# actuday6418/ray-tracer-s8

Hardware: AMD Instinct MI355X
Metric: Mrays/sec @ 4K/8spp 1024-sphere (higher is better)
Workload: dtype f32

## Files before the change

ray_tracer_s8_amd/csrc/rt_api.hip:

```cpp
#include <hip/hip_runtime.h>
#include <dlfcn.h>

#include <algorithm>
#include <chrono>
#include <cmath>
#include <cstdarg>
#include <cstdio>
#include <cstdlib>
#include <cstring>
#include <atomic>
#include <climits>
#include <condition_variable>
#include <mutex>
#include <new>
#include <stdexcept>
#include <string>
#include <thread>
#include <vector>

#include "rt_assign.h"
#include "rt_bvh.h"
#include "rt_kernel.hip.h"
#include "rt_plan.h"
#include "rt_query.hip.h"
#include "rt_scene_host.h"
#include "rt_trace.hip.h"
#include "rt_bounce.hip.h"
#include "rt_direct.hip.h"
#include "rt_nee.hip.h"
#include "rt_aov.hip.h"
#include "rt_camera.hip.h"
#include "rt_denoise.hip.h"
#include "rt_tile.h"
#ifdef RT_DEBUG_HOOKS
#include "rt_unit.hip.h"
#endif

namespace {

thread_local std::string g_err;

int fail(int code, const std::string& msg) {
    g_err = msg;
    return code;
}

void set_err_noexcept(const char* what) noexcept {
    try {
        g_err = what;
    } catch (...) {
    }
}
template <class F>
int guarded(F&& body) noexcept {
    try {
        return body();
    } catch (const std::bad_alloc&) {
        set_err_noexcept("host allocation failed");
        return RT_ERR_OOM;
    } catch (const std::exception& e) {
        set_err_noexcept(e.what());
        return RT_ERR_HIP;
    } catch (...) {
        set_err_noexcept("internal error");
        return RT_ERR_HIP;
    }
}

#define HIPCHK(expr)                                                                                  \
    do {                                                                                              \
        hipError_t _e = (expr);                                                                       \
        if (_e != hipSuccess)                                                                         \
            return fail(RT_ERR_HIP, std::string(#expr) + ": " + hipGetErrorString(_e) + " (" __FILE__ \
                                                                                        ":" +         \
                                        std::to_string(__LINE__) + ")");                              \
    } while (0)

struct DevBuf {
    char* d = nullptr;
    size_t cap = 0;
    int reserve(size_t bytes, const char* what) {
        if (cap >= bytes) return RT_OK;
        release();
        if (hipMalloc(&d, bytes) != hipSuccess) {
            d = nullptr;
            (void)hipGetLastError();
            return fail(RT_ERR_OOM, std::string("hipMalloc(") + what + ") failed");
        }
        cap = bytes;
        return RT_OK;
    }
    void release() {
        (void)hipFree(d);
        d = nullptr;
        cap = 0;
    }
};

struct DeviceCtx {
    int dev = -1;
    hipStream_t stream = nullptr;
    hipStream_t copy_stream = nullptr;
    int n_cu = 0;
    std::mutex mu;
};

enum DebugKnob {
    DBG_LDS_TREE = 0,
    DBG_CULL_WALK,
    DBG_NO_STAGE,
    DBG_SLOTS,
    DBG_FORCE_CAPPED,
    DBG_STACK_LDS,
    DBG_COMPACT,
    DBG_REFILL_EIGHTHS,
    DBG_COMMIT_SLOTS,
    DBG_VERBOSE,
    DBG_REORDER,
    DBG_TAIL_TILES,
    DBG_STRIP_COST,
    DBG_DENOISE_LDS_STEP,
    DBG_N
};
std::atomic<int> g_dbg[DBG_N];
const struct { const char* env; int def; } g_dbg_spec[DBG_N] = {
    {"RT_LDS_TREE", 1}, {"RT_CULL_WALK", -1}, {"RT_NO_STAGE", 0}, {"RT_SLOTS", 0}, {"RT_FORCE_CAPPED", 0},
    {"RT_STACK_LDS", 0}, {"RT_COMPACT", 1}, {"RT_REFILL_EIGHTHS", 0}, {"RT_COMMIT_SLOTS", 0}, {"RT_VERBOSE", 0}, {"RT_REORDER", 1}, {"RT_TAIL_TILES", -1}, {"RT_STRIP_COST", 1},
    {"RT_DENOISE_LDS_STEP", -1}};
std::once_flag g_dbg_once;
void dbg_load_env() {
    std::call_once(g_dbg_once, [] {
        for (int k = 0; k < DBG_N; k++) {
            const char* e = getenv(g_dbg_spec[k].env);
            int v = g_dbg_spec[k].def;
            if (e) v = k == DBG_VERBOSE ? 1 : atoi(e);
            g_dbg[k].store(v, std::memory_order_relaxed);
        }
    });
}
inline int dbg(DebugKnob k) { return g_dbg[k].load(std::memory_order_relaxed); }

std::mutex g_mu;
bool g_init = false;
std::vector<DeviceCtx*> g_ctx;
std::atomic<int> g_live_scenes{0};

rtplan::Knobs plan_knobs() {
    rtplan::Knobs k;
    k.lds_tree = dbg(DBG_LDS_TREE);
    k.cull_walk = dbg(DBG_CULL_WALK);
    k.no_stage = dbg(DBG_NO_STAGE);
    k.slots = dbg(DBG_SLOTS);
    k.commit_slots = dbg(DBG_COMMIT_SLOTS);
    k.force_capped = dbg(DBG_FORCE_CAPPED);
    k.stack_lds = dbg(DBG_STACK_LDS);
    k.compact = dbg(DBG_COMPACT);
    k.refill_eighths = dbg(DBG_REFILL_EIGHTHS);
    k.tail_tiles = dbg(DBG_TAIL_TILES);
    return k;
}

}

struct rt_scene {
    DeviceCtx* ctx = nullptr;
    rtplan::SceneShape shape;
    uint32_t n_lights = 0;
    uint32_t* d_lights = nullptr;
    rtplan::Pose pose;
    bool has_pose = false;
    float4* d_geom = nullptr;
    float4* d_geom_pk = nullptr;
    float4* d_geom_px = nullptr;
    float4* d_mat = nullptr;
    float* d_emis = nullptr;
    float* d_tri = nullptr;
    float4* d_tri_box = nullptr;
    float4* d_bvh = nullptr;
    float4* d_trav = nullptr;
    uint32_t* d_stack_ovf = nullptr;
    size_t stack_ovf_words = 0;
    hipEvent_t ovf_done = nullptr;
    uint4* d_travq = nullptr;
    float4* d_geom_r = nullptr;
    uint32_t* d_big = nullptr;
    uint32_t n_big = 0;
    float tri_k = 0.f, tri_diag = 0.f, tri_es = 0.f, tri_e = 0.f;
    rtbvh::QGrid grid;
    uint32_t* d_leaf_of = nullptr;
    uint32_t* d_world_rank = nullptr;
    bool has_order = false;
    float bvh_build_ms = 0.f;
    unsigned long long* d_counters = nullptr;
    struct Ring {
        float* d = nullptr;
        size_t bytes = 0;
        hipStream_t last = nullptr;
        hipEvent_t done = nullptr;
        uint64_t stamp = 0;
    };
    Ring rings[4];
    uint64_t ring_clock = 0;
    DevBuf d_out, d_outf, d_acc, d_cost, d_aov, d_dn, d_cam;
    DevBuf d_caller;
    std::vector<std::pair<hipEvent_t, hipEvent_t>> pending, free_ev;
    uint64_t primary_rays = 0;
    float h2d_ms = 0.f;
    uint32_t last_engine = 0, last_form = 0;
    std::mutex mu;
};

namespace {

int check_request(const rt_tile_request* rq) {
    if (!rq) return fail(RT_ERR_BAD_ARG, "request is NULL");
    if (rq->width == 0 || rq->height == 0 || rq->divisions == 0 || rq->spp == 0)
        return fail(RT_ERR_BAD_ARG, "width, height, divisions and spp must be non-zero");
    if (rq->division_no >= rq->divisions) return fail(RT_ERR_BAD_ARG, "division_no >= divisions");
    if (rq->height / rq->divisions == 0) return fail(RT_ERR_BAD_ARG, "height / divisions == 0 rows");
    if (rq->max_bounces > RT_MAX_BOUNCES) return fail(RT_ERR_LIMIT, "max_bounces > RT_MAX_BOUNCES");
    if (rq->spp > RT_MAX_SPP) return fail(RT_ERR_LIMIT, "spp > RT_MAX_SPP");
    if (rq->reserved != 0) return fail(RT_ERR_BAD_ARG, "reserved must be 0");
    if ((uint64_t)rq->width * rq->height > 0x7fffffffull) return fail(RT_ERR_LIMIT, "image too large");
    return RT_OK;
}

struct EvPair {
    hipEvent_t a, b;
};

int get_events(rt_scene* sc, EvPair& ev) {
    if (!sc->free_ev.empty()) {
        ev.a = sc->free_ev.back().first;
        ev.b = sc->free_ev.back().second;
        sc->free_ev.pop_back();
        return RT_OK;
    }
    HIPCHK(hipEventCreate(&ev.a));
    HIPCHK(hipEventCreate(&ev.b));
    return RT_OK;
}

constexpr uint32_t QUEUE_SLOTS = 16384;
#ifdef RT_PROFILE_TIME
constexpr uint32_t COUNTER_WORDS = 4 + QUEUE_SLOTS + 16 * 8192;
#else
constexpr uint32_t COUNTER_WORDS = 4 + QUEUE_SLOTS;
#endif

int check_slot(const rt_scene* sc) {
    if (sc->pending.size() >= QUEUE_SLOTS) return fail(RT_ERR_LIMIT, "too many uncollected launches: call rt_scene_collect()");
    return RT_OK;
}

template <class P>
int enqueue(rt_scene* sc, hipStream_t stream, void (*kern)(const P), uint32_t blocks, uint32_t block, size_t lds, const P& p) {
    EvPair ev;
    int rc;
    if ((rc = check_slot(sc)) || (rc = get_events(sc, ev))) return rc;
    HIPCHK(hipEventRecord(ev.a, stream));
    hipLaunchKernelGGL(kern, dim3(blocks), dim3(block), lds, stream, p);
    HIPCHK(hipGetLastError());
    HIPCHK(hipEventRecord(ev.b, stream));
    sc->pending.push_back({ev.a, ev.b});
    return RT_OK;
}

struct Grid {
    uint32_t blocks = 0;
    int per_cu = 0;
};
template <class P>
int persistent_blocks(const rt_scene* sc, void (*kern)(const P), uint32_t block, size_t lds, uint64_t items, Grid& g) {
    HIPCHK(hipOccupancyMaxActiveBlocksPerMultiprocessor(&g.per_cu, kern, (int)block, lds));
    if (g.per_cu < 1) g.per_cu = 1;
    g.blocks = (uint32_t)std::min<uint64_t>((items + block - 1) / block, (uint64_t)sc->ctx->n_cu * (uint32_t)g.per_cu);
    return RT_OK;
}

void scene_refs(const rt_scene* sc, bool full_chain, rtk::SceneRefs& r) {
    r.n_sph = sc->shape.n_sph;
    r.n_tri = sc->shape.n_tri;
    r.root_ref = sc->shape.root_ref;
    r.full_chain = full_chain ? 1u : 0u;
    r.trav = sc->d_trav;
    r.bvh_nodes = sc->d_bvh;
    r.leaf_of = sc->d_leaf_of;
    r.world_rank = sc->has_order ? sc->d_world_rank : nullptr;
    r.geom_r = sc->d_geom_r;
    r.tri = sc->d_tri;
    r.counters = sc->d_counters;
}

bool same_frame(const rt_tile_request& a, const rt_tile_request& b) {
    return a.width == b.width && a.height == b.height && a.divisions == b.divisions && a.spp == b.spp &&
           a.max_bounces == b.max_bounces && a.aperture == b.aperture && a.focus_distance == b.focus_distance &&
           a.fov == b.fov && a.focal_length == b.focal_length && a.t_min == b.t_min && a.t_max == b.t_max &&
           a.flags == b.flags;
}

struct Pass {
    uint32_t begin, end;
    void* const* d_acc;
};
int acquire_stack_ovf(rt_scene* sc, size_t words) {
    if (words > sc->stack_ovf_words) {
        if (sc->d_stack_ovf) {
            if (sc->ovf_done) HIPCHK(hipEventSynchronize(sc->ovf_done));
            (void)hipFree(sc->d_stack_ovf);
            sc->d_stack_ovf = nullptr;
            sc->stack_ovf_words = 0;
        }
        HIPCHK(hipMalloc(&sc->d_stack_ovf, words * sizeof(uint32_t)));
        sc->stack_ovf_words = words;
    }
    return RT_OK;
}

int acquire_ring(rt_scene* sc, hipStream_t stream, size_t bytes, rt_scene::Ring*& rg) {
    rg = nullptr;
    for (auto& r : sc->rings)
        if (r.d && r.last == stream) { rg = &r; break; }
    if (!rg)
        for (auto& r : sc->rings)
            if (!r.d) { rg = &r; break; }
    if (!rg) {
        rg = &sc->rings[0];
        for (auto& r : sc->rings)
            if (r.stamp < rg->stamp) rg = &r;
    }
    if (rg->bytes < bytes) {
        if (rg->d) {
            if (rg->done) HIPCHK(hipEventSynchronize(rg->done));
            (void)hipFree(rg->d);
            rg->d = nullptr;
            rg->bytes = 0;
        }
        HIPCHK(hipMalloc(&rg->d, bytes));
        rg->bytes = bytes;
    }
    if (!rg->done) HIPCHK(hipEventCreateWithFlags(&rg->done, hipEventDisableTiming));
    else if (rg->last != stream) HIPCHK(hipStreamWaitEvent(stream, rg->done, 0));
    rg->last = stream;
    rg->stamp = ++sc->ring_clock;
    return RT_OK;
}

int launch_batch(rt_scene* sc, const rt_tile_request* rqs, uint32_t n, void* const* d_rgb, void* const* d_f32,
                 hipStream_t stream, unsigned long long* d_strip_cost = nullptr, const Pass* pass = nullptr) {
    const rtplan::Knobs kn = plan_knobs();
    const rtplan::SceneShape& sh = sc->shape;
    rtk::KParams p;
    std::memset(&p, 0, sizeof p);
    const rtplan::SampleRange smp = pass ? rtplan::SampleRange{pass->begin, pass->end, true} : rtplan::SampleRange{0u, rqs[0].spp, false};
    rtplan::Plan pl = rtplan::plan_launch(sh, rqs[0], n, smp, kn, p, sc->has_pose ? &sc->pose : nullptr);
    if (pl.status != RT_OK) return fail(pl.status, pl.error);
    p.geom_pk = sc->d_geom_pk;
    p.geom_px = sc->d_geom_px;
    p.geom = sc->d_geom;
    p.mat = sc->d_mat;
    p.emis = sc->d_emis;
    p.tri = sc->d_tri;
    p.tri_box = sc->d_tri_box;
    p.bvh_nodes = sc->d_bvh;
    p.trav = sc->d_trav;
    p.travq = sc->d_travq;
    p.geom_r = sc->d_geom_r;
    for (int i = 0; i < 3; i++) {
        p.q_base[i] = sc->grid.base[i];
        p.q_step[i] = sc->grid.step[i];
        p.q_rstep[i] = 1.0f / sc->grid.step[i];
    }
    p.leaf_of = sc->d_leaf_of;
    p.world_rank = sc->has_order ? sc->d_world_rank : nullptr;
    p.big = sc->d_big;
    p.n_big = sc->n_big;
    p.r_slack = sh.r_slack;
    p.tri_k = sc->tri_k;
    p.tri_diag = sc->tri_diag;
    p.tri_es = sc->tri_es;
    p.tri_e = sc->tri_e;
    for (uint32_t i = 0; i < n; i++) {
        p.strips[i].seed = rqs[i].seed;
        p.strips[i].rgb = (uint8_t*)d_rgb[i];
        p.strips[i].f32 = d_f32 ? (float*)d_f32[i] : nullptr;
        p.strips[i].acc = pass ? (float*)pass->d_acc[i] : nullptr;
        p.strips[i].y0 = p.Hs * rqs[i].division_no;
    }
    int rc = check_slot(sc);
    if (rc) return rc;
    p.counters = sc->d_counters;
    p.queue = sc->d_counters + 4 + sc->pending.size();
    p.strip_cost = dbg(DBG_STRIP_COST) ? d_strip_cost : nullptr;

    const rtk::KernelFn kern = pl.isect < 2 ? rtk::kernel_linear(pl.isect, pl.expanded) : rtk::kernel_traverse(pl.isect, pl.count_steps);
    int per_cu = 0;
    HIPCHK(hipOccupancyMaxActiveBlocksPerMultiprocessor(&per_cu, kern, pl.block, pl.lds));
    if (per_cu < 1) per_cu = 1;
    if (dbg(DBG_VERBOSE))
        fprintf(stderr, "[rt] engine %d%s  lds %zu B  workgroups/CU %d  leaf slots %u  bvh depth %u  leaf density %.3f  prims %u\n",
                pl.engine, pl.capped ? " (capped stack)" : "", pl.lds, per_cu, pl.maxl_l2, sh.bvh_depth, sh.leaf_density, sh.n_sph + sh.n_tri);
    rtplan::plan_queue(pl, (uint32_t)sc->ctx->n_cu * (uint32_t)per_cu, kn, p);
    p.stack_ovf = nullptr;
    if (pl.capped) {
        if ((rc = acquire_stack_ovf(sc, pl.ovf_words))) return rc;
        p.stack_ovf = sc->d_stack_ovf;
    }
    if (dbg(DBG_VERBOSE))
        fprintf(stderr, "[rt] sample-unit ring %zu B: %u units per pixel, %u slots of %u records per wave\n", pl.ring_bytes, p.upp, p.n_slots,
                p.slot_stride);
    rt_scene::Ring* rg = nullptr;
    if ((rc = acquire_ring(sc, stream, pl.ring_bytes, rg))) return rc;
    p.ring = rg->d;
    if (p.stack_ovf) {
        if (sc->ovf_done) HIPCHK(hipStreamWaitEvent(stream, sc->ovf_done, 0));
        else HIPCHK(hipEventCreateWithFlags(&sc->ovf_done, hipEventDisableTiming));
    }
    HIPCHK(hipMemsetAsync(p.queue, 0, sizeof(unsigned long long), stream));
    sc->last_engine = (uint32_t)pl.engine;
    sc->last_form = pl.expanded ? 1u : 0u;
    if ((rc = enqueue(sc, stream, kern, pl.blocks, pl.block, pl.lds, p))) return rc;
    HIPCHK(hipEventRecord(rg->done, stream));
    if (p.stack_ovf) HIPCHK(hipEventRecord(sc->ovf_done, stream));
    sc->primary_rays += (uint64_t)p.Hs * p.W * p.upp * n;
    return RT_OK;
}

int collect_locked(rt_scene* sc, rt_tile_stats* st) {
    float ms = 0.f;
    uint32_t n = 0;
    for (auto& pr : sc->pending) {
        HIPCHK(hipEventSynchronize(pr.second));
        float t = 0.f;
        HIPCHK(hipEventElapsedTime(&t, pr.first, pr.second));
        ms += t;
        n++;
        sc->free_ev.push_back(pr);
    }
    sc->pending.clear();
    unsigned long long c[4] = {0, 0, 0, 0};
    HIPCHK(hipMemcpy(c, sc->d_counters, sizeof c, hipMemcpyDeviceToHost));
    HIPCHK(hipMemset(sc->d_counters, 0, sizeof c));
    if (st) {
        st->ray_segments = c[0];
        st->broad_candidates = c[1];
        st->exact_fallbacks = c[2];
        st->primary_rays = sc->primary_rays;
        st->kernel_ms = ms;
        st->n_launches = n;
        st->h2d_ms = sc->h2d_ms;
        st->d2h_ms = 0.f;
        st->engine = sc->last_engine;
        st->broad_form = sc->last_form;
        st->node_steps = c[3];
    }
    sc->primary_rays = 0;
    sc->h2d_ms = 0.f;
    return RT_OK;
}

struct StagedCall {
    rt_scene* const sc;
    const hipStream_t st;
    const float scene_h2d_ms;
    EvPair up{nullptr, nullptr}, down{nullptr, nullptr};
    bool finished = false;
    explicit StagedCall(rt_scene* s) : sc(s), st(s->ctx->stream), scene_h2d_ms(s->h2d_ms) {}
    StagedCall(const StagedCall&) = delete;
    ~StagedCall() {
        if (!finished) (void)hipStreamSynchronize(st);
        if (up.b) sc->free_ev.push_back({up.a, up.b});
        if (down.b) sc->free_ev.push_back({down.a, down.b});
        sc->h2d_ms = scene_h2d_ms;
    }
    int begin() {
        int rc;
        if ((rc = collect_locked(sc, nullptr)) || (rc = get_events(sc, up)) || (rc = get_events(sc, down))) return rc;
        HIPCHK(hipEventRecord(up.a, st));
        return RT_OK;
    }
    int uploads_done() {
        HIPCHK(hipEventRecord(up.b, st));
        return RT_OK;
    }
    int kernels_done() {
        HIPCHK(hipEventRecord(down.a, st));
        return RT_OK;
    }
    int finish(rt_tile_stats* stats) {
        HIPCHK(hipEventRecord(down.b, st));
        HIPCHK(hipEventSynchronize(down.b));
        finished = true;
        rt_tile_stats s;
        float h2d = 0.f, d2h = 0.f;
        HIPCHK(hipEventElapsedTime(&h2d, up.a, up.b));
        HIPCHK(hipEventElapsedTime(&d2h, down.a, down.b));
        int rc = collect_locked(sc, &s);
        if (rc) return rc;
        s.h2d_ms = h2d;
        s.d2h_ms = d2h;
        if (stats) *stats = s;
        return RT_OK;
    }
};

__attribute__((format(printf, 1, 2))) std::string vtext(const char* fmt, ...) {
    if (!dbg(DBG_VERBOSE)) return {};
    char buf[256];
    va_list ap;
    va_start(ap, fmt);
    vsnprintf(buf, sizeof buf, fmt, ap);
    va_end(ap);
    return buf;
}

template <class P>
void material_refs(const rt_scene* sc, P& p) {
    p.mat = sc->d_mat;
    p.emis = sc->d_emis;
}
template <class P>
void light_refs(const rt_scene* sc, P& p) {
    p.lights = sc->d_lights;
    p.n_lights = sc->n_lights;
}

template <class P>
int launch_rays(rt_scene* sc, const rtplan::QueryPlan& qp, uint32_t block, void (*kern)(const P), const char* what, P& p, uint64_t items,
                const std::string& head, const std::string& tail, uint64_t primary, hipStream_t stream, void* d_zero = nullptr) {
    if (!kern) return fail(RT_ERR_HIP, std::string("no ") + what + " kernel for this plan");
    scene_refs(sc, qp.full_chain, p);
    Grid g;
    int rc = persistent_blocks(sc, kern, block, qp.lds, items, g);
    if (rc || (d_zero && (rc = check_slot(sc)))) return rc;
    if (dbg(DBG_VERBOSE)) fprintf(stderr, "[rt] %s  workgroups/CU %d  %s\n", head.c_str(), g.per_cu, tail.c_str());
    if (d_zero) HIPCHK(hipMemsetAsync(d_zero, 0, sizeof(uint32_t), stream));
    if ((rc = enqueue(sc, stream, kern, g.blocks, block, qp.lds, p))) return rc;
    sc->primary_rays += primary;
    sc->last_engine = (uint32_t)qp.engine;
    sc->last_form = 0;
    return RT_OK;
}

template <class L>
int device_form(rt_scene* sc, void* hip_stream, L&& launch) {
    std::lock_guard<std::mutex> lk(sc->mu);
    HIPCHK(hipSetDevice(sc->ctx->dev));
    return launch(hip_stream ? (hipStream_t)hip_stream : sc->ctx->stream);
}

struct HostForm {
    rt_scene* const sc;
    std::lock_guard<std::mutex> dl, lk;
    explicit HostForm(rt_scene* s) : sc(s), dl(s->ctx->mu), lk(s->mu) {}
    int device() const {
        HIPCHK(hipSetDevice(sc->ctx->dev));
        return RT_OK;
    }
};

struct Staging {
    enum : unsigned { UP = 1, DOWN = 2 };
    struct Entry {
        const void* host;
        size_t bytes;
        unsigned copy;
        size_t off;
    };
    DevBuf& buf;
    std::vector<Entry> e;
    size_t total = 0;
    Staging(rt_scene* sc, std::initializer_list<Entry> entries) : buf(sc->d_caller), e(entries) {
        for (Entry& x : e) {
            x.off = total;
            total += x.bytes;
        }
    }
    int reserve(const char* what) { return buf.reserve(total, what); }
    char* dev(int k) const { return e[k].host ? buf.d + e[k].off : nullptr; }
    int upload(StagedCall& call) const {
        for (int k = 0; k < (int)e.size(); k++)
            if (e[k].host && e[k].bytes && (e[k].copy & UP)) HIPCHK(hipMemcpyAsync(dev(k), e[k].host, e[k].bytes, hipMemcpyHostToDevice, call.st));
        return call.uploads_done();
    }
    int download(StagedCall& call) const {
        int rc = call.kernels_done();
        if (rc) return rc;
        for (int k = 0; k < (int)e.size(); k++)
            if (e[k].host && e[k].bytes && (e[k].copy & DOWN))
                HIPCHK(hipMemcpyAsync(const_cast<void*>(e[k].host), dev(k), e[k].bytes, hipMemcpyDeviceToHost, call.st));
        return RT_OK;
    }
};

int check_active_list(const uint32_t* active, uint32_t n_active, uint32_t n) {
    if (!active) return RT_OK;
    if (n_active > n) return fail(RT_ERR_BAD_ARG, "n_active > n");
    for (uint32_t k = 0; k < n_active; k++)
        if (active[k] >= n) return fail(RT_ERR_BAD_ARG, "active[" + std::to_string(k) + "] >= n");
    return RT_OK;
}

}

extern "C" {

RT_API uint32_t rt_abi_version(void) { return RT_ABI_VERSION; }

RT_API const char* rt_strerror(int status) {
    switch (status) {
        case RT_OK: return "ok";
        case RT_ERR_BAD_ARG: return "bad argument";
        case RT_ERR_NOT_INITIALIZED: return "rt_init() has not succeeded";
        case RT_ERR_NO_DEVICE: return "no HIP device (this library has no CPU fallback)";
        case RT_ERR_BAD_DEVICE: return "device ordinal out of range";
        case RT_ERR_BUFFER_TOO_SMALL: return "output buffer smaller than (height/divisions)*width*3";
        case RT_ERR_FRAME_SIZE: return "height is not a multiple of divisions";
        case RT_ERR_HIP: return "HIP runtime error";
        case RT_ERR_LIMIT: return "limit exceeded";
        case RT_ERR_OOM: return "out of memory";
        default: return "unknown status";
    }
}

RT_API const char* rt_last_error(void) { return g_err.c_str(); }

RT_API void rt_tile_request_defaults(rt_tile_request* rq) {
    if (!rq) return;
    std::memset(rq, 0, sizeof *rq);
    rq->width = 1920;
    rq->height = 1080;
    rq->divisions = 20;
    rq->division_no = 0;
    rq->spp = 100;
    rq->max_bounces = 10;
    rq->aperture = 0.1f;
    rq->focus_distance = 1.0f;
    rq->fov = 3.14159265358979323846f / 2.0f;
    rq->focal_length = 1.0f;
    rq->t_min = 0.001f;
    rq->t_max = 1000.0f;
    rq->seed = 0;
    rq->flags = RT_FLAG_NONE;
}

RT_API size_t rt_tile_bytes(const rt_tile_request* rq) {
    if (!rq || rq->divisions == 0) return 0;
    return (size_t)(rq->height / rq->divisions) * rq->width * 3;
}

static int rt_init_impl(int* n_devices) {
    dbg_load_env();
    std::lock_guard<std::mutex> lk(g_mu);
    if (g_init) {
        if (n_devices) *n_devices = (int)g_ctx.size();
        return RT_OK;
    }
    int n = 0;
    hipError_t e = hipGetDeviceCount(&n);
    if (e != hipSuccess || n <= 0) {
        if (n_devices) *n_devices = 0;
        return fail(RT_ERR_NO_DEVICE, std::string("hipGetDeviceCount: ") +
                                          (e != hipSuccess ? hipGetErrorString(e) : "0 devices"));
    }
    for (int d = 0; d < n; d++) {
        DeviceCtx* c = new DeviceCtx;
        c->dev = d;
        g_ctx.push_back(c);
    }
    g_init = true;
    if (n_devices) *n_devices = n;
    return RT_OK;
}

static int ensure_ctx(DeviceCtx* c) {
    std::lock_guard<std::mutex> lk(c->mu);
    if (c->stream) return RT_OK;
    HIPCHK(hipSetDevice(c->dev));
    HIPCHK(hipDeviceGetAttribute(&c->n_cu, hipDeviceAttributeMultiprocessorCount, c->dev));
    for (int isect = 0; isect < rtplan::N_ISECT; isect++)
        for (int alt = 0; alt < 2; alt++)
            HIPCHK(hipFuncSetAttribute((const void*)(isect < 2 ? rtk::kernel_linear(isect, alt != 0) : rtk::kernel_traverse(isect, alt != 0)),
                                       hipFuncAttributeMaxDynamicSharedMemorySize, (int)rtplan::LDS_LIMIT));
    hipStream_t st = nullptr, cs = nullptr;
    HIPCHK(hipStreamCreateWithFlags(&st, hipStreamNonBlocking));
    HIPCHK(hipStreamCreateWithFlags(&cs, hipStreamNonBlocking));
    c->copy_stream = cs;
    c->stream = st;
    return RT_OK;
}

static int rt_shutdown_impl(void) {
    std::lock_guard<std::mutex> lk(g_mu);
    if (g_live_scenes.load() > 0)
        return fail(RT_ERR_BAD_ARG, "rt_shutdown() refused: destroy every rt_scene first (their device contexts stay valid)");
    for (DeviceCtx* c : g_ctx) {
        (void)hipSetDevice(c->dev);
        if (c->stream) (void)hipStreamDestroy(c->stream);
        if (c->copy_stream) (void)hipStreamDestroy(c->copy_stream);
        delete c;
    }
    g_ctx.clear();
    g_init = false;
    return RT_OK;
}

static int rt_scene_destroy_impl(rt_scene* sc);

using rtscene::HostScene;
static_assert(sizeof(rtscene::F4) == sizeof(float4) && alignof(rtscene::F4) == alignof(float4), "HostScene's records are the device's float4");

static int check_world(const rt_sphere* sp, uint32_t ns, const rt_triangle* tr, uint32_t nt, const uint32_t* world_index) {
    if ((ns && !sp) || (nt && !tr)) return fail(RT_ERR_BAD_ARG, "primitive pointer is NULL");
    if ((uint64_t)ns + nt > RT_MAX_PRIMITIVES) return fail(RT_ERR_LIMIT, "too many primitives (RT_MAX_PRIMITIVES)");
    if (world_index && !rtscene::world_is_permutation(world_index, ns + nt))
        return fail(RT_ERR_BAD_ARG, "world_index is not a permutation of 0 .. n_spheres + n_triangles - 1");
    return RT_OK;
}

static int upload_scene(int device, const HostScene& hs, rt_scene** out) {
    const auto t_create0 = std::chrono::steady_clock::now();
    if (!g_init) return fail(RT_ERR_NOT_INITIALIZED, "call rt_init() first");
    if (device < 0 || device >= (int)g_ctx.size()) return fail(RT_ERR_BAD_DEVICE, "bad device ordinal");
    DeviceCtx* ctx = g_ctx[device];
    {
        int rc0 = ensure_ctx(ctx);
        if (rc0) return rc0;
    }
    HIPCHK(hipSetDevice(ctx->dev));
    rt_scene* sc = new (std::nothrow) rt_scene;
    if (!sc) return fail(RT_ERR_OOM, "host allocation failed");
    g_live_scenes.fetch_add(1);
    struct SceneGuard {
        rt_scene* sc;
        ~SceneGuard() {
            if (sc) rt_scene_destroy_impl(sc);
        }
    } guard{sc};
    const rtbvh::FlatBVH& bvh = hs.bvh;
    sc->ctx = ctx;
    sc->shape = hs.shape;
    sc->bvh_build_ms = hs.bvh_build_ms;
    sc->grid = bvh.grid;
    hipEvent_t e0, e1;
    if (hipEventCreate(&e0) != hipSuccess) return fail(RT_ERR_HIP, "hipEventCreate failed");
    if (hipEventCreate(&e1) != hipSuccess) {
        (void)hipEventDestroy(e0);
        return fail(RT_ERR_HIP, "hipEventCreate failed");
    }
#define SC_CHK(expr)                                                                      \
    do {                                                                                  \
        hipError_t _e = (expr);                                                           \
        if (_e != hipSuccess) {                                                           \
            (void)hipEventDestroy(e0);                                                    \
            (void)hipEventDestroy(e1);                                                    \
            return fail(_e == hipErrorOutOfMemory ? RT_ERR_OOM : RT_ERR_HIP,              \
                        std::string(#expr) + ": " + hipGetErrorString(_e));               \
        }                                                                                 \
    } while (0)
#define SC_UP(dst, vec)                                                                                       \
    do {                                                                                                      \
        SC_CHK(hipMalloc(&sc->dst, (vec).size() * sizeof((vec)[0])));                                         \
        SC_CHK(hipMemcpyAsync(sc->dst, (vec).data(), (vec).size() * sizeof((vec)[0]), hipMemcpyHostToDevice,  \
                              ctx->stream));                                                                  \
    } while (0)
    SC_CHK(hipEventRecord(e0, ctx->stream));
    SC_UP(d_geom, hs.geom);
    SC_UP(d_geom_pk, hs.geom_pk);
    SC_UP(d_geom_px, hs.geom_px);
    SC_UP(d_mat, hs.mat);
    SC_UP(d_emis, hs.emis);
    SC_UP(d_tri, hs.tri);
    SC_UP(d_tri_box, hs.tri_box);
    SC_UP(d_bvh, bvh.nodes);
    SC_UP(d_leaf_of, bvh.leaf_of);
    SC_UP(d_world_rank, hs.world_rank);
    sc->has_order = hs.has_order;
    SC_UP(d_trav, bvh.trav);
    SC_UP(d_travq, bvh.travq);
    SC_UP(d_geom_r, hs.geom_r);
    SC_UP(d_big, hs.big);
    SC_UP(d_lights, hs.lights);
    sc->n_lights = hs.n_lights;
    sc->n_big = hs.n_big;
    sc->tri_k = hs.tri_k;
    sc->tri_diag = hs.tri_diag;
    sc->tri_es = hs.tri_es;
    sc->tri_e = hs.tri_e;
    SC_CHK(hipMalloc(&sc->d_counters, COUNTER_WORDS * sizeof(unsigned long long)));
    SC_CHK(hipMemsetAsync(sc->d_counters, 0, COUNTER_WORDS * sizeof(unsigned long long), ctx->stream));
    SC_CHK(hipEventRecord(e1, ctx->stream));
    SC_CHK(hipEventSynchronize(e1));
    SC_CHK(hipEventElapsedTime(&sc->h2d_ms, e0, e1));
#undef SC_UP
#undef SC_CHK
    (void)hipEventDestroy(e0);
    (void)hipEventDestroy(e1);
    if (dbg(DBG_VERBOSE))
        fprintf(stderr, "[rt] scene: %u prims  culled walk: %u big spheres, slack radius %g, box density %.3f -> %s  bvh build %.2f ms (host)  uploads %.2f ms  upload total %.2f ms\n",
                hs.shape.n_sph + hs.shape.n_tri, hs.n_big, hs.shape.r_slack, hs.shape.cull_density, hs.shape.cull_pays ? "default" : "off", sc->bvh_build_ms, sc->h2d_ms,
                std::chrono::duration<float, std::milli>(std::chrono::steady_clock::now() - t_create0).count());
    guard.sc = nullptr;
    *out = sc;
    return RT_OK;
}

static int rt_scene_create_impl(int device, const rt_sphere* sp, uint32_t ns, const rt_triangle* tr, uint32_t nt,
                                const uint32_t* world_index, rt_scene** out) {
    if (!out) return fail(RT_ERR_BAD_ARG, "out_scene is NULL");
    *out = nullptr;
    int rc = check_world(sp, ns, tr, nt, world_index);
    if (rc) return rc;
    if (!g_init) return fail(RT_ERR_NOT_INITIALIZED, "call rt_init() first");
    if (device < 0 || device >= (int)g_ctx.size()) return fail(RT_ERR_BAD_DEVICE, "bad device ordinal");
    HostScene hs;
    rtscene::build_host_scene(sp, ns, tr, nt, world_index, dbg(DBG_REORDER) != 0, hs);
    return upload_scene(device, hs, out);
}

static int rt_scene_destroy_impl(rt_scene* sc) {
    if (!sc) return RT_OK;
    if (sc->ctx) (void)hipSetDevice(sc->ctx->dev);
    for (auto& pr : sc->pending) {
        (void)hipEventSynchronize(pr.second);
        (void)hipEventDestroy(pr.first);
        (void)hipEventDestroy(pr.second);
    }
    for (auto& pr : sc->free_ev) {
        (void)hipEventDestroy(pr.first);
        (void)hipEventDestroy(pr.second);
    }
    (void)hipFree(sc->d_geom);
    (void)hipFree(sc->d_geom_pk);
    (void)hipFree(sc->d_geom_px);
    (void)hipFree(sc->d_mat);
    (void)hipFree(sc->d_emis);
    (void)hipFree(sc->d_tri);
    (void)hipFree(sc->d_tri_box);
    (void)hipFree(sc->d_bvh);
    (void)hipFree(sc->d_trav);
    (void)hipFree(sc->d_travq);
    (void)hipFree(sc->d_stack_ovf);
    if (sc->ovf_done) (void)hipEventDestroy(sc->ovf_done);
    for (auto& r : sc->rings) {
        (void)hipFree(r.d);
        if (r.done) (void)hipEventDestroy(r.done);
    }
    (void)hipFree(sc->d_geom_r);
    (void)hipFree(sc->d_big);
    (void)hipFree(sc->d_lights);
    (void)hipFree(sc->d_leaf_of);
    (void)hipFree(sc->d_world_rank);
    (void)hipFree(sc->d_counters);
    for (DevBuf* b : {&sc->d_out, &sc->d_outf, &sc->d_acc, &sc->d_cost, &sc->d_aov, &sc->d_dn, &sc->d_cam, &sc->d_caller}) b->release();
    delete sc;
    g_live_scenes.fetch_sub(1);
    return RT_OK;
}

static int check_batch(const rt_tile_request* rqs, uint32_t n) {
    if (!rqs || n == 0) return fail(RT_ERR_BAD_ARG, "empty request batch");
    for (uint32_t i = 0; i < n; i++) {
        int rc = check_request(&rqs[i]);
        if (rc) return rc;
        if (!same_frame(rqs[0], rqs[i]))
            return fail(RT_ERR_BAD_ARG, "batched requests must agree on every field but division_no and seed");
    }
    return RT_OK;
}

static int check_samples(uint32_t begin, uint32_t end, uint32_t spp) {
    if (begin >= end) return fail(RT_ERR_BAD_ARG, "sample_begin >= sample_end");
    if (end > spp) return fail(RT_ERR_BAD_ARG, "sample_end > spp");
    return RT_OK;
}

static int check_array(const void* const* a, uint32_t n, const char* what) {
    if (!a) return fail(RT_ERR_BAD_ARG, std::string(what) + " is NULL");
    for (uint32_t i = 0; i < n; i++)
        if (!a[i]) return fail(RT_ERR_BAD_ARG, std::string(what) + "[i] is NULL");
    return RT_OK;
}

static int check_pass(const rt_tile_request* rqs, uint32_t n, const Pass& pass) {
    int rc = check_samples(pass.begin, pass.end, rqs[0].spp);
    return rc ? rc : check_array(pass.d_acc, n, "accum");
}

static int rt_scene_render_tiles_device_impl(rt_scene* sc, const rt_tile_request* rqs, uint32_t n,
                                        void* const* d_out_rgb, size_t out_len_each, void* const* d_out_f32,
                                        void* hip_stream, const Pass* pass = nullptr) {
    if (!sc) return fail(RT_ERR_BAD_ARG, "scene is NULL");
    int rc = check_batch(rqs, n);
    if (rc) return rc;
    if ((rc = check_array(d_out_rgb, n, "d_out_rgb"))) return rc;
    if (out_len_each < rt_tile_bytes(&rqs[0])) return fail(RT_ERR_BUFFER_TOO_SMALL, "out_len < (H/div)*W*3");
    if (pass && (rc = check_pass(rqs, n, *pass))) return rc;
    std::lock_guard<std::mutex> lk(sc->mu);
    HIPCHK(hipSetDevice(sc->ctx->dev));
    hipStream_t st = hip_stream ? (hipStream_t)hip_stream : sc->ctx->stream;
    for (uint32_t i0 = 0; i0 < n; i0 += rtk::MAX_BATCH) {
        uint32_t m = std::min<uint32_t>(rtk::MAX_BATCH, n - i0);
        Pass part = {};
        if (pass) part = {pass->begin, pass->end, pass->d_acc + i0};
        rc = launch_batch(sc, rqs + i0, m, d_out_rgb + i0, d_out_f32 ? d_out_f32 + i0 : nullptr, st, nullptr, pass ? &part : nullptr);
        if (rc) return rc;
    }
    return RT_OK;
}

static int rt_scene_render_tile_device_impl(rt_scene* sc, const rt_tile_request* rq, void* d_out_rgb, size_t out_len,
                                       void* d_out_f32, void* hip_stream) {
    void* rgb[1] = {d_out_rgb};
    void* f32[1] = {d_out_f32};
    return rt_scene_render_tiles_device_impl(sc, rq, 1, rgb, out_len, d_out_f32 ? f32 : nullptr, hip_stream);
}

static int rt_scene_collect_impl(rt_scene* sc, rt_tile_stats* st) {
    if (!sc) return fail(RT_ERR_BAD_ARG, "scene is NULL");
    std::lock_guard<std::mutex> lk(sc->mu);
    HIPCHK(hipSetDevice(sc->ctx->dev));
    return collect_locked(sc, st);
}

static int rt_scene_render_tiles_impl(rt_scene* sc, const rt_tile_request* rqs, uint32_t n, uint8_t* const* out_rgb,
                                 size_t out_len_each, float* const* out_f32, rt_tile_stats* stats,
                                 unsigned long long* strip_cost_out = nullptr, const Pass* pass = nullptr) {
    if (!sc) return fail(RT_ERR_BAD_ARG, "scene is NULL");
    int rc = check_batch(rqs, n);
    if (rc) return rc;
    if ((rc = check_array((const void* const*)out_rgb, n, "out_rgb"))) return rc;
    const size_t need = rt_tile_bytes(&rqs[0]);
    if (out_len_each < need) return fail(RT_ERR_BUFFER_TOO_SMALL, "out_len < (H/div)*W*3");
    if (pass && (rc = check_pass(rqs, n, *pass))) return rc;
    bool want_f32 = false;
    if (out_f32)
        for (uint32_t i = 0; i < n; i++) want_f32 |= out_f32[i] != nullptr;
    std::lock_guard<std::mutex> dl(sc->ctx->mu);
    std::lock_guard<std::mutex> lk(sc->mu);
    HIPCHK(hipSetDevice(sc->ctx->dev));
    hipStream_t st = sc->ctx->stream;
    if ((rc = sc->d_out.reserve(need * n, "strips")) || (want_f32 && (rc = sc->d_outf.reserve(need * n * sizeof(float), "strips f32"))) ||
        (pass && (rc = sc->d_acc.reserve(need * n * sizeof(float), "running sums"))))
        return rc;
    constexpr size_t COST_BLOCK = (size_t)rtk::COST_COPIES * rtk::MAX_BATCH;
    const size_t cost_blocks = strip_cost_out ? (n + rtk::MAX_BATCH - 1) / rtk::MAX_BATCH + 1 : 0;
    unsigned long long* d_cost = nullptr;
    if (strip_cost_out) {
        const size_t cost_b = cost_blocks * COST_BLOCK * sizeof(unsigned long long);
        if ((rc = sc->d_cost.reserve(cost_b, "strip costs"))) return rc;
        d_cost = (unsigned long long*)sc->d_cost.d;
        HIPCHK(hipMemsetAsync(d_cost, 0, cost_b, st));
    }
    rt_tile_stats prev;
    rc = collect_locked(sc, &prev);
    if (rc) return rc;
    sc->h2d_ms = prev.h2d_ms;
    std::vector<void*> drgb(n), df32(n), dacc(pass ? n : 0);
    for (uint32_t i = 0; i < n; i++) {
        drgb[i] = sc->d_out.d + need * i;
        df32[i] = (want_f32 && out_f32[i]) ? sc->d_outf.d + need * i * sizeof(float) : nullptr;
        if (pass) dacc[i] = sc->d_acc.d + need * i * sizeof(float);
    }
    std::vector<std::pair<uint32_t, uint32_t>> groups;
    {
        const uint32_t tail = (n >= 4 && (uint64_t)need * n > (64ull << 20)) ? std::max<uint32_t>(1, n / 4) : 0;
        for (uint32_t i0 = 0; i0 < n - tail; i0 += rtk::MAX_BATCH)
            groups.emplace_back(i0, std::min<uint32_t>(rtk::MAX_BATCH, n - tail - i0));
        for (uint32_t i0 = n - tail; i0 < n; i0 += rtk::MAX_BATCH)
            groups.emplace_back(i0, std::min<uint32_t>(rtk::MAX_BATCH, n - i0));
    }
    hipStream_t cs = sc->ctx->copy_stream;
    std::vector<EvPair> gev;
    gev.reserve(groups.size());
    struct EvReturn {
        rt_scene* sc;
        std::vector<EvPair>& v;
        hipStream_t a, b;
        bool ok = false;
        ~EvReturn() {
            if (!ok) {
                (void)hipStreamSynchronize(a);
                (void)hipStreamSynchronize(b);
            }
            for (auto& e : v) sc->free_ev.push_back({e.a, e.b});
        }
// ... 1538 lines not shown
```

ray_tracer_s8_amd/csrc/rt_consts.h:

```cpp
#pragma once
#include <stdint.h>

#if defined(__HIPCC__)
#define RT_HOST_DEVICE __host__ __device__ inline
#else
#define RT_HOST_DEVICE inline
#endif

#ifndef RT_MAXC
#define RT_MAXC 16
#endif
#ifndef RT_MAXL
#define RT_MAXL 8
#endif
#ifndef RT_MINL
#define RT_MINL 4
#endif
#ifndef RT_MAXL_LTREE
#define RT_MAXL_LTREE 12
#endif

namespace rtk {

constexpr int BLOCK = 256;
constexpr int LTREE_BLOCK = 1024;
constexpr int UNROLL = 8;
constexpr int MAXC = RT_MAXC;
constexpr int CHUNK = 2048;
constexpr int MAX_BATCH = 64;
constexpr int TRAV_STACK = 64;
constexpr int MAXL = RT_MAXL;
constexpr int MINL = RT_MINL;
constexpr int MAXL_EXACT = 7;
constexpr int LNODE_DW = 19;
RT_HOST_DEVICE uint32_t lt_r0(uint32_t n_internal) { return 0x8000u - (n_internal + 1u) * (uint32_t)LNODE_DW; }
constexpr int MAXL_LTREE = RT_MAXL_LTREE;
constexpr int MAXL_LTREE_MAX = 16;
constexpr uint32_t LEAF_BIT = 0x80000000u;
constexpr uint32_t STAGE_TILE_BYTES = 192;
constexpr uint32_t STAGE_TILES = 3;
constexpr uint32_t SLOTS_MAX = 32;
constexpr uint32_t COST_COPIES = 16;

}
```

ray_tracer_s8_amd/csrc/rt_kernel.hip.h:

```cpp
#pragma once
#include <hip/hip_runtime.h>
#include <type_traits>
#include <stdint.h>

#include "rt_consts.h"
#include "rt_cull.h"

namespace rtk {

#ifndef RT_MINWAVES
#define RT_MINWAVES 4
#endif
#ifndef RT_MINWAVES_TRAV
#define RT_MINWAVES_TRAV 4
#endif
#ifndef RT_MINWAVES_LTREE
#define RT_MINWAVES_LTREE 4
#endif
#ifndef RT_MINWAVES_CULL
#define RT_MINWAVES_CULL 5
#endif
#ifndef RT_STEPS_PER_CHECK_X
#define RT_STEPS_PER_CHECK_X 16
#endif
#ifndef RT_QUEUE_TAKE_MIN
#define RT_QUEUE_TAKE_MIN 4
#endif
#ifndef RT_BF2
#define RT_BF2 1
#endif
#ifndef RT_CULL_FLUSH_MIN
#define RT_CULL_FLUSH_MIN 1
#endif
#ifndef RT_MINWAVES_QTRAV
#define RT_MINWAVES_QTRAV 5
#endif
#ifndef RT_STEPS_PER_CHECK
#define RT_STEPS_PER_CHECK 8
#endif
#ifndef RT_STEPS_PER_CHECK_LTREE
#define RT_STEPS_PER_CHECK_LTREE 8
#endif
#ifndef RT_STEPS_PER_CHECK_Q
#define RT_STEPS_PER_CHECK_Q 16
#endif
#ifndef RT_LT_PARTIAL
#define RT_LT_PARTIAL 40
#endif
#ifndef RT_LT_EAGER
#define RT_LT_EAGER 12
#endif

constexpr uint32_t SLOT_FREE = 0x80000000u;
struct WaveQ {
    uint32_t cnt[SLOTS_MAX];
    uint32_t cost_acc[2];
    uint32_t cost_strip[2];
};
static_assert(sizeof(WaveQ) == 144, "WaveQ layout (rt_plan.h: LDS_LIMIT leaves 3 KiB of static LDS)");
constexpr uint32_t SLOT_UNIT_BITS = 13;
struct WaveStage {
    int left[STAGE_TILES + 1];
    uint32_t dst_lo[STAGE_TILES + 1], dst_hi[STAGE_TILES + 1];
};

struct StripDesc {
    uint64_t seed;
    uint8_t* rgb;
    float* f32;
    float* acc;
    uint32_t y0;
    uint32_t pad;
};

struct KParams {
    uint32_t W, H, Hs;
    uint32_t upp, depth;
    uint32_t spp_all, s_begin, gap;
    uint32_t acc_out;
    uint32_t n_sph, n_sph_pad;
    uint32_t n_tri;
    uint32_t chunk;
    uint32_t n_chunks;
    uint32_t flags;
    uint32_t path32;
    uint32_t lds_cand_off;
    uint32_t lds_path_off;
    uint32_t lds_rr_off;
    uint32_t lds_stack_off;
    uint32_t lds_cmp_off;
    uint32_t lds_stage_off;
    uint32_t n_strips;
    uint32_t tiles_x, tiles_per_strip;
    uint32_t tiles_total;
    uint32_t tiles_big;
    uint32_t sub_shift;
    uint32_t n_tiles;
    uint32_t n_slots;
    uint32_t grp;
    uint32_t grp_magic;
    uint32_t slot_stride;
    uint32_t commit_slots;
    uint32_t spp_magic;
    uint32_t slotu_magic;
    float* ring;
    float org[3], llc[3], hor[3], ver[3];
    float lens_radius, focus_distance;
    float lens_u[3], lens_v[3];
    float u_den, v_den;
    float t_min, t_max;
    float spp_f;
    float spp_rcp;
    const float4* geom_pk;
    const float4* geom_px;
    const float4* geom;
    const float4* mat;
    const float* emis;
    const float* tri;
    const float4* tri_box;
    const float4* trav;
    const uint4* travq;
    const float4* geom_r;
    float q_base[3], q_step[3], q_rstep[3];
    uint32_t root_ref;
    uint32_t maxl;
    uint32_t list16;
    uint32_t stack_lds;
    uint32_t ovf_stride;
    uint32_t* stack_ovf;
    const uint32_t* big;
    uint32_t n_big;
    float r_slack;
    float tri_k, tri_diag, tri_es, tri_e;
    uint32_t refill_eighths;
    uint32_t n_internal;
    uint32_t lds_node_off;
    const float4* bvh_nodes;
    const uint32_t* leaf_of;
    const uint32_t* world_rank;
    unsigned long long* strip_cost;
    unsigned long long* counters;
    unsigned long long* queue;
    StripDesc strips[MAX_BATCH];
};

struct V3 {
    float x, y, z;
};
__device__ __forceinline__ V3 mk(float x, float y, float z) { return V3{x, y, z}; }
__device__ __forceinline__ V3 operator+(V3 a, V3 b) { return {a.x + b.x, a.y + b.y, a.z + b.z}; }
__device__ __forceinline__ V3 operator-(V3 a, V3 b) { return {a.x - b.x, a.y - b.y, a.z - b.z}; }
__device__ __forceinline__ V3 operator*(float s, V3 a) { return {s * a.x, s * a.y, s * a.z}; }
__device__ __forceinline__ V3 operator*(V3 a, float s) { return {a.x * s, a.y * s, a.z * s}; }
template <class P>
__device__ __forceinline__ V3 lens_offset(const P& p, float x1, float x2) {
    return mk(x1 * p.lens_u[0] + x2 * p.lens_v[0], x1 * p.lens_u[1] + x2 * p.lens_v[1], x1 * p.lens_u[2] + x2 * p.lens_v[2]);
}
template <bool NEG_OK = false>
__device__ __forceinline__ float sqrt_rn(float x) {
#ifdef RT_IEEE_SQRT_PLAIN
    return __builtin_sqrtf(x);
#else
    const float r = __builtin_amdgcn_rsqf(x);
    float g = x * r, h = 0.5f * r;
    const float e = __builtin_fmaf(-h, g, 0.5f);
    g = __builtin_fmaf(g, e, g);
    h = __builtin_fmaf(h, e, h);
    const float dd = __builtin_fmaf(-g, g, x);
    float y = __builtin_fmaf(dd, h, g);
    const bool odd = ((__float_as_uint(x) & (NEG_OK ? 0x7fffffffu : 0xffffffffu)) - 0x0f800000u) >= (0x7f800000u - 0x0f800000u);
    if (__ballot(odd)) {
        if (odd) {
            asm volatile("" : "+v"(x));
            y = __builtin_sqrtf(x);
        }
    }
    return y;
#endif
}
#define RT_SQRT(x_) sqrt_rn(x_)
#define RT_SQRT_NEG_OK(x_) sqrt_rn<true>(x_)
#define RT_DIV(a_, b_) ((a_) / (b_))
#define RT_HOOK_LT_STEP_LOADS(nd_, ni_, lnodes_)
#define RT_HOOK_LT_STEP_ALU(p0_, p1_, p2_, p3_, oy_)
#define RT_HOOK_LT_STEP_END
#define RT_HOOK_Q_GATHER(t_ref_, cl_, travq_, n_internal_)
#ifdef RT_PROBES
#include "rt_probes.h"
#endif
__device__ __forceinline__ V3 operator/(V3 a, float s) { return {RT_DIV(a.x, s), RT_DIV(a.y, s), RT_DIV(a.z, s)}; }
__device__ __forceinline__ float dot(V3 a, V3 b) { return (a.x * b.x + a.y * b.y) + a.z * b.z; }
__device__ __forceinline__ float vlength(V3 a) { return RT_SQRT(dot(a, a)); }
__device__ __forceinline__ V3 normalize(V3 a) { return a / vlength(a); }
__device__ __forceinline__ bool try_normalize(V3 a, V3& out) {
    float rcp = RT_DIV(1.0f, RT_SQRT(dot(a, a)));
    if (rcp > 0.0f && rcp < __builtin_inff()) {
        out = a * rcp;
        return true;
    }
    return false;
}
__device__ __forceinline__ V3 normalize_or_zero(V3 a) {
    V3 r;
    return try_normalize(a, r) ? r : mk(0.f, 0.f, 0.f);
}
__device__ __forceinline__ V3 cross(V3 a, V3 b) {
    return {a.y * b.z - a.z * b.y, a.z * b.x - a.x * b.z, a.x * b.y - a.y * b.x};
}

struct Rng {
    uint64_t s0, s1, s2, s3;
};
__device__ __forceinline__ uint64_t rotl64(uint64_t x, int k) { return (x << k) | (x >> (64 - k)); }
__device__ __forceinline__ uint32_t next_u32(Rng& r) {
    uint64_t result = rotl64(r.s0 + r.s3, 23) + r.s0;
    uint64_t t = r.s1 << 17;
    r.s2 ^= r.s0;
    r.s3 ^= r.s1;
    r.s1 ^= r.s2;
    r.s0 ^= r.s3;
    r.s2 ^= t;
    r.s3 = rotl64(r.s3, 45);
    return (uint32_t)(result >> 32);
}
__device__ __forceinline__ uint64_t splitmix_mix(uint64_t z) {
    z = (z ^ (z >> 30)) * 0xbf58476d1ce4e5b9ull;
    z = (z ^ (z >> 27)) * 0x94d049bb133111ebull;
    return z ^ (z >> 31);
}
constexpr uint64_t PHI = 0x9e3779b97f4a7c15ull;
__device__ __forceinline__ Rng seed_state(uint64_t st) {
    Rng r;
    st += PHI; r.s0 = splitmix_mix(st);
    st += PHI; r.s1 = splitmix_mix(st);
    st += PHI; r.s2 = splitmix_mix(st);
    st += PHI; r.s3 = splitmix_mix(st);
    return r;
}
__device__ __forceinline__ float u01(Rng& r) {
    return __uint_as_float((next_u32(r) >> 9) | 0x3f800000u) - 1.0f;
}
__device__ __forceinline__ float gen_range_01(Rng& r) { return u01(r) * 1.0f + 0.0f; }
__device__ __forceinline__ float uniform_m1_1(Rng& r) { return u01(r) * 2.0f + -1.0f; }

__device__ __forceinline__ bool exact_sphere(V3 o, V3 td, V3 cen, float rr, float t_min, float t_max,
                                             float& t_out) {
    const V3 oc = o - cen;
    const float b = dot(td, oc);
    const float len = RT_SQRT(dot(oc, oc));
    const float c = len * len - rr;
    const float disc = b * b - 4.0f * c;
    const float sq = RT_SQRT_NEG_OK(disc);
    const bool bneg = b < 0.0f;
    const float same_sign = bneg ? -b + sq : -b - sq;
    const float diff_sign = bneg ? -b - sq : -b + sq;
    const float a0x2 = 2.0f * c;
    const bool big_s = __builtin_fabsf(same_sign) > 2.0f, big_d = __builtin_fabsf(diff_sign) > 2.0f;
    const float q1 = RT_DIV(a0x2, same_sign), q2 = RT_DIV(a0x2, diff_sign), hs = same_sign / 2.0f, hd = diff_sign / 2.0f;
    const float x1 = big_s ? q1 : hd;
    const float x2 = big_s ? (big_d ? q2 : hs) : hs;
    const bool one = disc == 0.0f;
    const float r1 = -b / 2.0f;
    const float x = one ? r1 : (x1 < x2 ? x1 : x2);
    const float y = one ? r1 : (x1 < x2 ? x2 : x1);
    const bool xin = (x >= t_min) && (x < t_max);
    const bool yin = (y >= t_min) && (y < t_max);
    t_out = (xin && yin) ? (x < y ? x : y) : (xin ? x : y);
    return !(disc < 0.0f) && (xin || yin);
}

__device__ __forceinline__ bool exact_triangle(V3 o, V3 d, const float* __restrict__ tv, float t_min, float t_max,
                                               float& t_out) {
    const float EPSILON = 0.00001f;
    V3 A = mk(tv[0], tv[1], tv[2]), B = mk(tv[3], tv[4], tv[5]), C = mk(tv[6], tv[7], tv[8]);
    V3 a_to_b = B - A;
    V3 a_to_c = C - A;
    V3 u_vec = cross(d, a_to_c);
    float det = dot(a_to_b, u_vec);
    if (det < EPSILON && det > -EPSILON) return false;
    float inv_det = 1.0f / det;
    V3 a_to_origin = o - A;
    float u = dot(a_to_origin, u_vec) * inv_det;
    if (!(u >= 0.0f && u <= 1.0f)) return false;
    V3 v_vec = cross(a_to_origin, a_to_b);
    float v = dot(d, v_vec) * inv_det;
    if (v < 0.0f || u + v > 1.0f) return false;
    float dist = dot(a_to_c, v_vec) * inv_det;
    if (!(dist > EPSILON)) return false;
    t_out = dist;
    return (dist >= t_min) && (dist < t_max);
}

struct RayAux {
    V3 inv;
    bool sx, sy, sz;
    bool full_chain;
    bool finite;
};
__device__ __forceinline__ RayAux ray_aux(V3 d, bool full_chain) {
    RayAux a;
    a.full_chain = full_chain;
    a.inv = mk(RT_DIV(1.0f, d.x), RT_DIV(1.0f, d.y), RT_DIV(1.0f, d.z));
    a.sx = d.x < 0.0f;
    a.sy = d.y < 0.0f;
    a.sz = d.z < 0.0f;
    const float big = __builtin_inff();
    a.finite = !full_chain && __builtin_fabsf(a.inv.x) < big && __builtin_fabsf(a.inv.y) < big &&
               __builtin_fabsf(a.inv.z) < big;
    return a;
}
__device__ __forceinline__ float rmin(float x, float y) { return x < y ? x : y; }
__device__ __forceinline__ float rmax(float x, float y) { return x > y ? x : y; }
__device__ __forceinline__ bool intersects_aabb(V3 o, const RayAux& a, float4 lo, float4 hi) {
    float ray_min = ((a.sx ? hi.x : lo.x) - o.x) * a.inv.x;
    float ray_max = ((a.sx ? lo.x : hi.x) - o.x) * a.inv.x;
    float y_min = ((a.sy ? hi.y : lo.y) - o.y) * a.inv.y;
    float y_max = ((a.sy ? lo.y : hi.y) - o.y) * a.inv.y;
    ray_min = rmax(ray_min, y_min);
    ray_max = rmin(ray_max, y_max);
    float z_min = ((a.sz ? hi.z : lo.z) - o.z) * a.inv.z;
    float z_max = ((a.sz ? lo.z : hi.z) - o.z) * a.inv.z;
    ray_min = rmax(ray_min, z_min);
    ray_max = rmin(ray_max, z_max);
    return rmax(ray_min, 0.0f) <= ray_max;
}
__device__ __forceinline__ bool intersects_aabb_finite(V3 o, const RayAux& a, float4 lo, float4 hi) {
    const float x0 = (lo.x - o.x) * a.inv.x, x1 = (hi.x - o.x) * a.inv.x;
    const float y0 = (lo.y - o.y) * a.inv.y, y1 = (hi.y - o.y) * a.inv.y;
    const float z0 = (lo.z - o.z) * a.inv.z, z1 = (hi.z - o.z) * a.inv.z;
    const float ray_min = __builtin_fmaxf(__builtin_fmaxf(__builtin_fminf(x0, x1), __builtin_fminf(y0, y1)),
                                          __builtin_fminf(z0, z1));
    const float ray_max = __builtin_fminf(__builtin_fminf(__builtin_fmaxf(x0, x1), __builtin_fmaxf(y0, y1)),
                                          __builtin_fmaxf(z0, z1));
    return __builtin_fmaxf(ray_min, 0.0f) <= ray_max;
}
__device__ __forceinline__ void slabs_finite(V3 o, const RayAux& a, float4 lo, float4 hi, float& ray_min, float& ray_max) {
    const float x0 = (lo.x - o.x) * a.inv.x, x1 = (hi.x - o.x) * a.inv.x;
    const float y0 = (lo.y - o.y) * a.inv.y, y1 = (hi.y - o.y) * a.inv.y;
    const float z0 = (lo.z - o.z) * a.inv.z, z1 = (hi.z - o.z) * a.inv.z;
    ray_min = __builtin_fmaxf(__builtin_fmaxf(__builtin_fminf(x0, x1), __builtin_fminf(y0, y1)), __builtin_fminf(z0, z1));
    ray_max = __builtin_fminf(__builtin_fminf(__builtin_fmaxf(x0, x1), __builtin_fmaxf(y0, y1)), __builtin_fmaxf(z0, z1));
}
__device__ __forceinline__ bool bvh_reaches(const float4* __restrict__ nodes, uint32_t node, V3 o, const RayAux& a) {
    const bool finite_inv = a.finite;
    for (;;) {
        const float4 lo = nodes[2 * (size_t)node];
        const uint32_t parent = __float_as_uint(lo.w);
        if (parent == 0xffffffffu) return true;
        const float4 hi = nodes[2 * (size_t)node + 1];
        if (!intersects_aabb(o, a, lo, hi)) return false;
        if (finite_inv) return true;
        node = parent;
    }
}

struct Hit {
    int idx;
    float dist;
    float t;
};
template <int MODE>
__device__ __forceinline__ void consider(Hit& h, int idx, V3 o, V3 d, float t, const RayAux& a,
                                         const float4* __restrict__ nodes, const uint32_t* __restrict__ leaf_of) {
    V3 p = o + t * d;
    float dist = vlength(p - o);
    const bool better = h.idx < 0 || h.dist > dist;
    const bool tie = h.idx >= 0 && h.dist == dist;
    if (!(better || tie)) return;
    if (MODE == 0) {
        if (!better) return;
    } else if (MODE == 1) {
        if (!better && leaf_of[idx] > leaf_of[h.idx]) return;
    } else {
        const uint32_t rank = leaf_of[idx];
        if (!better && rank > leaf_of[h.idx]) return;
        if (!bvh_reaches(nodes, rank, o, a)) return;
    }
    h.idx = idx;
    h.dist = dist;
    h.t = t;
}

template <bool RANKED = false, class Pred>
__device__ __forceinline__ void consider_if(Hit& h, int idx, V3 o, V3 d, float t, Pred admitted, const uint32_t* __restrict__ leaf_of = nullptr) {
    V3 p = o + t * d;
    float dist = vlength(p - o);
    if (!(h.idx < 0 || h.dist > dist)) {
        if (!(RANKED && h.dist == dist && leaf_of[idx] < leaf_of[h.idx])) return;
    }
    if (!admitted()) return;
    h.idx = idx;
    h.dist = dist;
    h.t = t;
}

__device__ __forceinline__ unsigned long long wave_sum(unsigned long long v) {
    for (int off = 32; off > 0; off >>= 1) v += __shfl_xor(v, off, 64);
    return v;
}

__device__ __forceinline__ uint8_t f32_as_u8(float v) {
    if (!(v == v)) return 0;
    if (v <= 0.0f) return 0;
    if (v >= 255.0f) return 255;
    return (uint8_t)(int)v;
}

#ifdef RT_PROFILE_PHASES
#define WCOUNT(slot)                                                                         \
    do {                                                                                     \
        unsigned long long _m = __ballot(1);                                                 \
        if ((int)(threadIdx.x & 63) == (int)__builtin_ctzll(_m)) atomicAdd(&p.counters[4 + 8192 + (slot)], 1ull); \
    } while (0)
#define LCOUNT(slot)                                                                         \
    do {                                                                                     \
        unsigned long long _m = __ballot(1);                                                 \
        if ((int)(threadIdx.x & 63) == (int)__builtin_ctzll(_m)) {                           \
            atomicAdd(&p.counters[4 + 8192 + 32 + (slot)], (unsigned long long)__builtin_popcountll(_m)); \
            atomicAdd(&p.counters[4 + 8192 + 64 + (slot)], 1ull);                            \
        }                                                                                    \
    } while (0)
#else
#define WCOUNT(slot) do { } while (0)
#define LCOUNT(slot) do { } while (0)
#endif
#ifdef RT_PROFILE_TIME
#define TDECL unsigned long long _tacc[8] = {0, 0, 0, 0, 0, 0, 0, 0}; unsigned long long _tlast = __builtin_amdgcn_s_memtime(); const unsigned long long _t0 = __builtin_amdgcn_s_memrealtime(); unsigned long long _tq = 0, _nq = 0
#define TDRAINED do { _tq = __builtin_amdgcn_s_memrealtime(); } while (0)
#define TROUND do { if (_tq) { const uint32_t _w = blockIdx.x * (blockDim.x >> 6) + (threadIdx.x >> 6); const unsigned long long _lv = __builtin_popcountll(__ballot(have_unit)); \
    if ((threadIdx.x & 63) == 0 && _w % 20u == 0u && _w / 20u < 215u && _nq < 16ull) p.counters[4 + 8192 + 4400 + (_w / 20u) * 16u + _nq] = (__builtin_amdgcn_s_memrealtime() & 0xfffffffull) | (_lv << 28); \
    _nq++; } } while (0)
#define TSTAMP(ph) do { const unsigned long long _n = __builtin_amdgcn_s_memtime(); _tacc[ph] += _n - _tlast; _tlast = _n; } while (0)
#define TFLUSH do { if ((threadIdx.x & 63) == 0) { const uint32_t _w = blockIdx.x * (blockDim.x >> 6) + (threadIdx.x >> 6); \
    if (_w < 8192u) { unsigned long long* _b = p.counters + 4 + 16384 + 16u * _w; for (int _i = 0; _i < 8; _i++) _b[_i] = _tacc[_i]; \
    _b[8] = __builtin_amdgcn_s_memrealtime(); _b[9] = _t0; _b[10] = _tq; _b[11] = _nq; } } } while (0)
#else
#define TDECL do { } while (0)
#define TDRAINED do { } while (0)
#define TROUND do { } while (0)
#define TSTAMP(ph) do { } while (0)
#define TFLUSH do { } while (0)
#endif

#ifndef RT_GEOM_RR
#define RT_SPHERE_REC(p_, prim_) ([&]() { const float4 r_ = at32((p_).geom_r, (prim_)); return make_float4(r_.x, r_.y, r_.z, r_.w * r_.w); }())
#else
#define RT_SPHERE_REC(p_, prim_) at32((p_).geom, (prim_))
#endif

typedef float v2f __attribute__((ext_vector_type(2)));
__device__ __forceinline__ v2f pk_fma(v2f a, v2f b, v2f c) { return __builtin_elementwise_fma(a, b, c); }

template <class T>
__device__ __forceinline__ const T& at32(const T* __restrict__ base, uint32_t i) {
    return *reinterpret_cast<const T*>(reinterpret_cast<const char*>(base) + i * (uint32_t)sizeof(T));
}

template <bool ON>
__device__ __forceinline__ int cold(int v) {
    if (ON) asm volatile("" : "+v"(v));
    return v;
}
#ifndef RT_COMMIT_BATCH
#define RT_COMMIT_BATCH 8
#endif
#ifndef RT_COMMIT_AGENT_LOADS
#define RT_COMMIT_AGENT_LOADS 0
#endif
template <class T>
__device__ __forceinline__ T ring_load(const T* q) {
#if RT_COMMIT_AGENT_LOADS
    return __hip_atomic_load(q, __ATOMIC_RELAXED, __HIP_MEMORY_SCOPE_AGENT);
#else
    return *q;
#endif
}
__device__ __forceinline__ uint32_t uni(uint32_t v) { return (uint32_t)__builtin_amdgcn_readfirstlane((int)v); }

__device__ __forceinline__ void qslabs(const uint4 qa, const uint4 qb, V3 ig, V3 cq, float& lmin, float& lmax, float& rmin_, float& rmax_) {
#define RT_Q(word, hi16) ((float)((hi16) ? ((word) >> 16) : ((word) & 0xffffu)))
    const float ax = __builtin_fabsf(ig.x), ay = __builtin_fabsf(ig.y), az = __builtin_fabsf(ig.z);
    const float lcx = __builtin_fmaf(RT_Q(qa.x, 0), ig.x, cq.x), lcy = __builtin_fmaf(RT_Q(qa.x, 1), ig.y, cq.y), lcz = __builtin_fmaf(RT_Q(qa.y, 0), ig.z, cq.z);
    const float lhx = RT_Q(qa.y, 1), lhy = RT_Q(qa.z, 0), lhz = RT_Q(qa.z, 1);
    const float rcx = __builtin_fmaf(RT_Q(qa.w, 0), ig.x, cq.x), rcy = __builtin_fmaf(RT_Q(qa.w, 1), ig.y, cq.y), rcz = __builtin_fmaf(RT_Q(qb.x, 0), ig.z, cq.z);
    const float rhx = RT_Q(qb.x, 1), rhy = RT_Q(qb.y, 0), rhz = RT_Q(qb.y, 1);
#undef RT_Q
    lmin = __builtin_fmaxf(__builtin_fmaxf(__builtin_fmaf(-lhx, ax, lcx), __builtin_fmaf(-lhy, ay, lcy)), __builtin_fmaf(-lhz, az, lcz));
    lmax = __builtin_fminf(__builtin_fminf(__builtin_fmaf(lhx, ax, lcx), __builtin_fmaf(lhy, ay, lcy)), __builtin_fmaf(lhz, az, lcz));
    rmin_ = __builtin_fmaxf(__builtin_fmaxf(__builtin_fmaf(-rhx, ax, rcx), __builtin_fmaf(-rhy, ay, rcy)), __builtin_fmaf(-rhz, az, rcz));
    rmax_ = __builtin_fminf(__builtin_fminf(__builtin_fmaf(rhx, ax, rcx), __builtin_fmaf(rhy, ay, rcy)), __builtin_fmaf(rhz, az, rcz));
}

__device__ __forceinline__ float cull_bound(float best, V3 o, float r_slack) { return cull_bound(best, o.x, o.y, o.z, r_slack); }
__device__ __forceinline__ float cull_bound_tri(float best, V3 o, float k, float diag, float es, float e) {
    return cull_bound_tri(best, o.x, o.y, o.z, k, diag, es, e);
}

template <int ISECT, bool EXPANDED, int BS = BLOCK, bool STATS = false>
__global__ __launch_bounds__(BS, (ISECT == 5 || ISECT == 6) ? RT_MINWAVES_LTREE : ISECT == 9 ? RT_MINWAVES_TRAV : ISECT >= 7 ? RT_MINWAVES_CULL : ISECT >= 3 ? RT_MINWAVES_QTRAV : ISECT == 2 ? RT_MINWAVES_TRAV : RT_MINWAVES) void rt_tile_kernel(const KParams p) {
    constexpr int BLOCK = BS;
    constexpr bool STREAMED = (ISECT == 1);
    constexpr bool TRAVERSE = (ISECT >= 2);
    constexpr bool QNODES = (ISECT == 3 || ISECT == 4 || ISECT == 7 || ISECT == 8);
    constexpr bool CULL = (ISECT == 6 || ISECT == 7 || ISECT == 8 || ISECT == 9);
    constexpr bool XNODES = (ISECT == 2 || ISECT == 9);
    constexpr bool CAPPED = (ISECT == 4 || ISECT == 8);
    constexpr bool LTREE = (ISECT == 5 || ISECT == 6);
    constexpr uint32_t LB = LTREE ? 0x8000u : LEAF_BIT;
    constexpr bool BFSTEP = LTREE;
    const uint32_t ML = QNODES ? p.maxl : (uint32_t)MAXL_EXACT;
    extern __shared__ __attribute__((aligned(16))) unsigned char lds_raw[];
    __shared__ unsigned long long wg_tiles;
    __shared__ unsigned int wg_lock, wg_drained;
    __shared__ WaveQ wave_q[BS / 64];
    constexpr bool CAN_STAGE = (ISECT >= 1 && ISECT <= 4) || ISECT >= 7;
    __shared__ WaveStage wave_st[CAN_STAGE ? BS / 64 : 1];
    {
        uint32_t* z = reinterpret_cast<uint32_t*>(&wave_q[threadIdx.x >> 6]);
        if ((threadIdx.x & 63u) < SLOTS_MAX) wave_q[threadIdx.x >> 6].cnt[threadIdx.x & 63u] = SLOT_FREE;
        if ((threadIdx.x & 63u) == 0u) {
            wave_q[threadIdx.x >> 6].cost_acc[0] = wave_q[threadIdx.x >> 6].cost_acc[1] = 0u;
            wave_q[threadIdx.x >> 6].cost_strip[0] = wave_q[threadIdx.x >> 6].cost_strip[1] = 0xffffffffu;
        }
        (void)z;
        if (CAN_STAGE && (threadIdx.x & 63u) <= STAGE_TILES) wave_st[threadIdx.x >> 6].left[threadIdx.x & 63u] = -1;
    }
    if (threadIdx.x == 0) {
        wg_tiles = 0ull;
        wg_lock = 0u;
        wg_drained = 0u;
    }
    __syncthreads();
    float4* lgeom = reinterpret_cast<float4*>(lds_raw);
    const float* lgeomf = reinterpret_cast<const float*>(lds_raw);
    float* lrr = reinterpret_cast<float*>(lds_raw + p.lds_rr_off);
    const float4* __restrict__ gsrc = EXPANDED ? p.geom_px : p.geom_pk;
    uint16_t* lcand = reinterpret_cast<uint16_t*>(lds_raw + p.lds_cand_off);
    unsigned char* lpath = lds_raw + p.lds_path_off;

    const int tid = threadIdx.x;
    const int lane = tid & 63;
    const int tid16 = (tid & ~63) | ((tid & 31) << 1) | ((tid >> 5) & 1);

    if (ISECT == 0) {
        for (uint32_t i = tid; i < p.n_sph_pad; i += BLOCK) lgeom[i] = gsrc[i];
        if (EXPANDED)
            for (uint32_t i = tid; i < p.n_sph_pad; i += BLOCK) lrr[i] = p.geom[i].w;
        __syncthreads();
    }

    if (LTREE) {
        float* ln = reinterpret_cast<float*>(lds_raw + p.lds_node_off);
        const uint32_t r0 = lt_r0(p.n_internal);
        for (uint32_t n = tid; n <= p.n_internal; n += BLOCK) {
            float* q = ln + LNODE_DW * n;
            if (n < p.n_internal) {
                const float4 a0 = p.trav[4u * n], a1 = p.trav[4u * n + 1], a2 = p.trav[4u * n + 2], a3 = p.trav[4u * n + 3];
                auto ref16 = [r0](uint32_t r) { return (r & LEAF_BIT) ? (0x8000u | (r & 0x7fffu)) : r0 + r * (uint32_t)LNODE_DW; };
                q[0] = a0.x; q[1] = a1.x; q[2] = a0.x;   q[3] = a2.x; q[4] = a3.x; q[5] = a2.x;
                q[6] = a0.y; q[7] = a1.y; q[8] = a0.y;   q[9] = a2.y; q[10] = a3.y; q[11] = a2.y;
                q[12] = a0.z; q[13] = a1.z; q[14] = a0.z; q[15] = a2.z; q[16] = a3.z; q[17] = a2.z;
                q[18] = __uint_as_float(ref16(__float_as_uint(a0.w)) | (ref16(__float_as_uint(a1.w)) << 16));
            } else {
                const float qn = __builtin_nanf(""), inf = __builtin_inff();
                for (int i = 0; i < 18; i++) q[i] = qn;
                for (int a = 0; a < 3; a++) { q[6 * a] = -inf; q[6 * a + 1] = inf; q[6 * a + 2] = -inf; }
                q[18] = __uint_as_float((r0 + p.n_internal * (uint32_t)LNODE_DW) * 0x10001u);
            }
        }
        float* nanf_ = ln + LNODE_DW * (p.n_internal + 1u);
        for (uint32_t i = tid; i < p.n_sph + p.n_tri + (uint32_t)LNODE_DW; i += BLOCK) nanf_[i] = __builtin_nanf("");
        __syncthreads();
    }
    const float* const lnodes = reinterpret_cast<const float*>(lds_raw + p.lds_node_off) - (LTREE ? (int)lt_r0(p.n_internal) : 0);
    const V3 corg = mk(p.org[0], p.org[1], p.org[2]);
    const V3 llc = mk(p.llc[0], p.llc[1], p.llc[2]);
    const V3 hor = mk(p.hor[0], p.hor[1], p.hor[2]);
    const V3 ver = mk(p.ver[0], p.ver[1], p.ver[2]);
    const bool exact_scan = (p.flags & 1u) != 0;
    const bool use_bvh = (p.flags & 2u) == 0;
    const float KMf = 1.0f - 0x1p-17f;
    const v2f NKM = {-KMf, -KMf};

    const uint32_t wave = (uint32_t)tid >> 6;
#define wq wave_q[wave]
#define wst wave_st[CAN_STAGE ? wave : 0u]
    float* const ring = p.ring + (size_t)(blockIdx.x * (uint32_t)(BLOCK / 64) + wave) * ((size_t)p.n_slots * p.slot_stride * 3u);
    const uint32_t all_free = p.n_slots >= 32u ? 0xffffffffu : (1u << p.n_slots) - 1u;
    uint32_t freem = all_free;
    uint32_t cur_slot = 0;
    uint32_t tile_u = 0, tile_units = 0;
    uint32_t tile_x0 = 0, tile_row = 0, tile_yg = 0;
    uint32_t tile_meta = STAGE_TILES << 16;
    uint64_t tile_seed = 0;
    bool q_drained = false;
    bool have_unit = false, need_ray = false;
    uint32_t useq = 0;
    Rng rng = {0, 0, 0, 0};
    uint32_t depth_left = 0, k = 0;
    V3 o = mk(0, 0, 0), d = mk(0, 0, 0);
    bool bounce = false;
    V3 bn = mk(0, 0, 0);
    float brough = 0.f;
    using Cnt = typename std::conditional<(ISECT >= 2), uint32_t, unsigned long long>::type;
    Cnt n_seg = 0, n_cand = 0, n_fall = 0;
    Cnt n_int = 0;
    Hit h;
    h.idx = -1;
    h.dist = 0.f;
    h.t = 0.f;
    RayAux aux = ray_aux(mk(1.f, 1.f, 1.f), false);
    auto AUX = [&]() -> RayAux { return QNODES ? ray_aux(d, (p.flags & 8u) != 0) : aux; };
    auto far_bound = [&](float best) -> float {
        float b = cull_bound(best, o, p.r_slack);
        if ((ISECT == 9 || ISECT == 6) && p.n_tri) b = __builtin_fmaxf(b, cull_bound_tri(best, o, p.tri_k, p.tri_diag, p.tri_es, p.tri_e));
        return b;
    };
    V3 td = mk(0, 0, 0);
    bool in_trav = false;
    uint32_t t_ref = 0, t_sp = 0, t_cnt = 0;
    uint32_t t_head = 0;
    V3 ig = mk(0, 0, 0), cq = mk(0, 0, 0);
    bool qfin = false;
    float t_far = __builtin_inff();
    uint32_t* lc32 = reinterpret_cast<uint32_t*>(lds_raw + p.lds_cand_off);
    uint32_t* lstack = reinterpret_cast<uint32_t*>(lds_raw + p.lds_stack_off);
    uint32_t sgx = 0, sgy = 0, sgz = 0;
    uint16_t* lc16 = reinterpret_cast<uint16_t*>(lds_raw + p.lds_cand_off);
    uint16_t* lstack16 = reinterpret_cast<uint16_t*>(lds_raw + p.lds_stack_off);

    if (BFSTEP) lstack16[tid16] = (uint16_t)(lt_r0(p.n_internal) + p.n_internal * (uint32_t)LNODE_DW);

    auto drain_counters = [&]() {
        const unsigned long long ws = wave_sum(n_seg), wc = wave_sum(n_cand), wf = wave_sum(n_fall);
        const unsigned long long wi = STATS ? wave_sum(n_int) : 0ull;
        if (lane == (int)__builtin_ctzll(__ballot(true))) {
            atomicAdd(&p.counters[0], ws);
            atomicAdd(&p.counters[1], wc);
            atomicAdd(&p.counters[2], wf);
            if (STATS) atomicAdd(&p.counters[3], wi);
        }
        n_seg = n_cand = n_fall = 0;
        n_int = 0;
    };
    const bool staging = CAN_STAGE && p.lds_stage_off != 0xffffffffu;
    unsigned char* const stage_base = lds_raw + (staging ? p.lds_stage_off + wave * (STAGE_TILES * STAGE_TILE_BYTES) : 0u);
    auto decode_tile = [&](uint32_t t, uint32_t& st, uint32_t& x0, uint32_t& row) {
        st = t / p.tiles_per_strip;
        const uint32_t rem = t - st * p.tiles_per_strip;
        row = rem / p.tiles_x;
        x0 = (rem - row * p.tiles_x) << 6;
    };
    auto div_spp = [&](uint32_t q) -> uint32_t { return p.spp_magic ? __umulhi(q, p.spp_magic) : q; };

    TDECL;
    for (;;) {
        WCOUNT(0);
        TSTAMP(5);
        TROUND;
        uint32_t px = 0, pyg = 0;
        if (freem != all_free) {
            __builtin_amdgcn_fence(__ATOMIC_ACQ_REL, "wavefront");
            const bool slot_done = (uint32_t)lane < SLOTS_MAX && (wq.cnt[cold<QNODES>(lane) & (int)(SLOTS_MAX - 1u)] & (SLOT_FREE | ((1u << SLOT_UNIT_BITS) - 1u))) == 0u;
            const uint32_t complete = (uint32_t)__ballot(slot_done);
            const uint32_t n_complete = (uint32_t)__builtin_popcount(complete);
            const bool issue_over = q_drained && tile_u == tile_units;
            if (n_complete >= p.commit_slots || (n_complete != 0u && ((uint32_t)__builtin_popcount(freem) < 2u || issue_over))) {
                WCOUNT(14);
                asm volatile("s_waitcnt vmcnt(0)" ::: "memory");
                const uint32_t n_lanes = p.n_slots * p.grp;
                for (uint32_t l0 = 0; l0 < n_lanes; l0 += 64u) {
                    const uint32_t L = l0 + (uint32_t)lane;
                    const uint32_t slot = p.grp == 1u ? L : __umulhi(L, p.grp_magic), g = L - slot * p.grp;
                    const bool mine = slot < p.n_slots && ((complete >> (slot & 31u)) & 1u) != 0u;
                    if (__ballot(mine) == 0ull) continue;
                    uint32_t stg = STAGE_TILES, cstrip = 0;
                    bool fin = false;
                    uint32_t pin = 0;
                    if (mine) {
                        const float* sb = ring + __umul24(slot, p.slot_stride) * 3u;
                        const uint32_t hx = ring_load(reinterpret_cast<const uint32_t*>(sb) + 0);
                        const uint32_t hrow = ring_load(reinterpret_cast<const uint32_t*>(sb) + 1);
                        const uint32_t hmeta = ring_load(reinterpret_cast<const uint32_t*>(sb) + 2);
                        const float* r = sb + 3u + g * p.upp * 3u;
                        float sum_r = 0.f, sum_g = 0.f, sum_b = 0.f;
                        cstrip = hmeta & 0xffu;
                        if (p.s_begin != 0u && g < ((hmeta >> 8) & 0xffu)) {
                            const float* a = p.strips[cstrip].acc + ((size_t)hrow * p.W + hx + g) * 3;
                            sum_r = a[0];
                            sum_g = a[1];
                            sum_b = a[2];
                        }
                        {
                            uint32_t i = 0;
                            auto batch = [&](auto cb_tag) {
                                constexpr int CB = decltype(cb_tag)::value;
#pragma clang loop unroll(disable)
                                for (; i + (uint32_t)CB <= p.upp; i += (uint32_t)CB) {
                                    LCOUNT(12);
                                    float c[3 * CB];
#pragma unroll
                                    for (int e = 0; e < 3 * CB; e++) c[e] = ring_load(r + e);
#pragma unroll
                                    for (int e = 0; e < CB; e++) {
                                        sum_r = sum_r + c[3 * e + 0];
                                        sum_g = sum_g + c[3 * e + 1];
                                        sum_b = sum_b + c[3 * e + 2];
                                    }
                                    r += 3 * CB;
                                }
                            };
                            if (RT_COMMIT_BATCH > 4 && !QNODES) batch(std::integral_constant<int, RT_COMMIT_BATCH>{});
                            batch(std::integral_constant<int, 4>{});
#pragma clang loop unroll(disable)
                            for (; i < p.upp; i++) {
                                LCOUNT(12);
                                const float cr = ring_load(r + 0);
                                const float cg = ring_load(r + 1);
                                const float cb = ring_load(r + 2);
                                sum_r = sum_r + cr;
                                sum_g = sum_g + cg;
                                sum_b = sum_b + cb;
                                r += 3;
                            }
                        }
                        if (g < ((hmeta >> 8) & 0xffu)) {
                            float cr_, cg_, cb_;
                            if (p.spp_rcp != 0.0f) {
                                cr_ = __builtin_sqrtf(sum_r * p.spp_rcp);
                                cg_ = __builtin_sqrtf(sum_g * p.spp_rcp);
                                cb_ = __builtin_sqrtf(sum_b * p.spp_rcp);
                            } else {
                                cr_ = __builtin_sqrtf(sum_r / p.spp_f);
                                cg_ = __builtin_sqrtf(sum_g / p.spp_f);
                                cb_ = __builtin_sqrtf(sum_b / p.spp_f);
                            }
                            const uint32_t sidx = hmeta & 0xffu;
                            stg = (hmeta >> 16) & 0xffu;
                            const size_t oidx = ((size_t)hrow * p.W + hx + g) * 3;
                            if (p.acc_out) {
                                float* a = p.strips[sidx].acc;
                                a[oidx + 0] = sum_r;
                                a[oidx + 1] = sum_g;
                                a[oidx + 2] = sum_b;
                            }
                            if (!CAN_STAGE || stg == STAGE_TILES) {
                                uint8_t* orgb = p.strips[sidx].rgb;
                                orgb[oidx + 0] = f32_as_u8(cr_ * 255.999f);
                                orgb[oidx + 1] = f32_as_u8(cg_ * 255.999f);
                                orgb[oidx + 2] = f32_as_u8(cb_ * 255.999f);
                            } else {
                                uint8_t* sd = stage_base + stg * STAGE_TILE_BYTES + ((hx + g) & 63u) * 3u;
                                sd[0] = f32_as_u8(cr_ * 255.999f);
                                sd[1] = f32_as_u8(cg_ * 255.999f);
                                sd[2] = f32_as_u8(cb_ * 255.999f);
                                fin = true;
                            }
                            float* of = p.strips[sidx].f32;
                            if (of) {
                                of[oidx + 0] = cr_;
                                of[oidx + 1] = cg_;
                                of[oidx + 2] = cb_;
                            }
                            (void)pin;
                        }
                    }
                    if (p.strip_cost && mine && g == 0u) {
                        const uint32_t sg = wq.cnt[slot & (SLOTS_MAX - 1u)] >> SLOT_UNIT_BITS;
                        if (cstrip == wq.cost_strip[0]) (void)__hip_atomic_fetch_add(&wq.cost_acc[0], sg, __ATOMIC_RELAXED, __HIP_MEMORY_SCOPE_WAVEFRONT);
                        else if (cstrip == wq.cost_strip[1]) (void)__hip_atomic_fetch_add(&wq.cost_acc[1], sg, __ATOMIC_RELAXED, __HIP_MEMORY_SCOPE_WAVEFRONT);
                        else if (sg) atomicAdd(&p.strip_cost[(blockIdx.x % COST_COPIES) * MAX_BATCH + cstrip], (unsigned long long)sg);
                    }
                    if (CAN_STAGE && __ballot(fin)) {
                        __builtin_amdgcn_fence(__ATOMIC_ACQ_REL, "wavefront");
#pragma unroll
                        for (uint32_t k = 0; k < STAGE_TILES; k++) {
                            const unsigned long long mk = __ballot(fin && stg == k);
                            if (mk == 0ull) continue;
                            const int left = (int)uni((uint32_t)wst.left[k]) - (int)__builtin_popcountll(mk);
                            if (left == 0) {
                                if (lane < (int)(STAGE_TILE_BYTES / 4)) {
                                    uint32_t* d32 = reinterpret_cast<uint32_t*>(((uintptr_t)uni(wst.dst_hi[k]) << 32) | uni(wst.dst_lo[k]));
                                    d32[lane] = reinterpret_cast<const uint32_t*>(stage_base + k * STAGE_TILE_BYTES)[lane];
                                }
                            }
                            if (lane == 0) wst.left[k] = left == 0 ? -1 : left;
                        }
                        __builtin_amdgcn_fence(__ATOMIC_ACQ_REL, "wavefront");
                    }
                }
                if (slot_done) wq.cnt[cold<QNODES>(lane)] = SLOT_FREE;
                freem = uni(freem | complete);
                __builtin_amdgcn_fence(__ATOMIC_ACQ_REL, "wavefront");
            }
        }
        TSTAMP(6);
        if (TRAVERSE && __ballot(((n_seg | n_cand | n_fall | n_int) & 0x80000000u) != 0)) drain_counters();
        {
            bool need = !have_unit;
            for (;;) {
                if (__ballot(need) == 0ull) break;
                if (tile_u == tile_units) {
                    if (q_drained) break;
                    uint32_t t = 0xffffffffu;
                    if (lane == 0) {
                        constexpr uint32_t WGC = (uint32_t)(BLOCK / 64) < (uint32_t)RT_QUEUE_TAKE_MIN ? (uint32_t)RT_QUEUE_TAKE_MIN : (uint32_t)(BLOCK / 64);
                        for (;;) {
                            const unsigned long long old = __hip_atomic_fetch_add(&wg_tiles, 1ull, __ATOMIC_RELAXED, __HIP_MEMORY_SCOPE_WORKGROUP);
                            if ((uint32_t)old < (uint32_t)(old >> 32)) {
                                t = (uint32_t)old;
                                break;
                            }
                            if (__hip_atomic_load(&wg_drained, __ATOMIC_RELAXED, __HIP_MEMORY_SCOPE_WORKGROUP)) break;
                            if (__hip_atomic_exchange(&wg_lock, 1u, __ATOMIC_ACQUIRE, __HIP_MEMORY_SCOPE_WORKGROUP) == 0u) {
                                const unsigned long long cur = __hip_atomic_load(&wg_tiles, __ATOMIC_RELAXED, __HIP_MEMORY_SCOPE_WORKGROUP);
                                bool done = false;
                                if ((uint32_t)cur >= (uint32_t)(cur >> 32)) {
                                    const uint32_t g = (uint32_t)atomicAdd(p.queue, (unsigned long long)WGC);
                                    if (g >= p.n_tiles) {
                                        __hip_atomic_store(&wg_drained, 1u, __ATOMIC_RELAXED, __HIP_MEMORY_SCOPE_WORKGROUP);
                                    } else {
                                        t = g;
                                        const uint32_t ge = min(g + WGC, p.n_tiles);
                                        __hip_atomic_store(&wg_tiles, (unsigned long long)(g + 1u) | ((unsigned long long)ge << 32),
                                                           __ATOMIC_RELAXED, __HIP_MEMORY_SCOPE_WORKGROUP);
                                    }
                                    done = true;
                                }
                                __hip_atomic_store(&wg_lock, 0u, __ATOMIC_RELEASE, __HIP_MEMORY_SCOPE_WORKGROUP);
                                if (done) break;
                            } else {
                                __builtin_amdgcn_s_sleep(2);
                            }
                        }
                    }
                    t = (uint32_t)__builtin_amdgcn_readfirstlane((int)t);
                    if (t == 0xffffffffu) {
                        q_drained = true;
                        TDRAINED;
                        break;
                    }
                    uint32_t sub = 0u, tw = 64u;
                    if (t >= p.tiles_big) {
                        const uint32_t e = t - p.tiles_big;
                        t = p.tiles_big + (e >> p.sub_shift);
                        tw = 64u >> p.sub_shift;
                        sub = (e & ((1u << p.sub_shift) - 1u)) * tw;
                    }
#ifndef RT_TILES_TOP_DOWN
                    t = p.tiles_total - 1u - t;
#endif
                    uint32_t tstrip;
                    decode_tile(t, tstrip, tile_x0, tile_row);
                    if (p.strip_cost && lane == 0 && (wq.cost_strip[0] != tstrip || wq.cost_acc[0] >= 0x80000000u)) {
                        if (wq.cost_acc[1]) atomicAdd(&p.strip_cost[(blockIdx.x % COST_COPIES) * MAX_BATCH + wq.cost_strip[1]], (unsigned long long)wq.cost_acc[1]);
                        wq.cost_acc[1] = wq.cost_acc[0];
                        wq.cost_strip[1] = wq.cost_strip[0];
                        wq.cost_acc[0] = 0u;
                        wq.cost_strip[0] = tstrip;
                    }
                    tile_x0 = uni(tile_x0 + sub);
                    tile_row = uni(tile_row);
                    if (tile_x0 >= p.W) continue;
                    tile_yg = uni(p.strips[tstrip].y0 + tile_row);
                    tile_seed = p.strips[tstrip].seed + (((uint64_t)tile_yg * p.W + tile_x0) * p.spp_all + p.s_begin) * (4ull * PHI);
                    tile_seed = (uint64_t)uni((uint32_t)tile_seed) | ((uint64_t)uni((uint32_t)(tile_seed >> 32)) << 32);
                    const uint32_t npix = min(tw, p.W - tile_x0);
                    tile_units = uni(npix * p.upp);
                    tile_u = 0u;
                    uint32_t tstage = STAGE_TILES;
                    if (staging && npix == 64u) {
                        uint8_t* dst = p.strips[tstrip].rgb + ((size_t)tile_row * p.W + tile_x0) * 3;
                        if ((reinterpret_cast<uintptr_t>(dst) & 3u) == 0) {
                            __builtin_amdgcn_fence(__ATOMIC_ACQ_REL, "wavefront");
                            for (uint32_t k = 0; k < STAGE_TILES; k++)
                                if ((int)uni((uint32_t)wst.left[k]) < 0) {
                                    tstage = k;
                                    break;
                                }
                            if (tstage < STAGE_TILES && lane == 0) {
                                wst.left[tstage] = 64;
                                wst.dst_lo[tstage] = (uint32_t)reinterpret_cast<uintptr_t>(dst);
                                wst.dst_hi[tstage] = (uint32_t)(reinterpret_cast<uintptr_t>(dst) >> 32);
                            }
                            __builtin_amdgcn_fence(__ATOMIC_ACQ_REL, "wavefront");
                        }
                    }
                    tile_meta = uni(tstrip | (tstage << 16));
                }
                bool got = false;
                uint32_t tv = 0;
                bool stall = false;
                {
                    const unsigned long long mask = __ballot(need);
                    const uint32_t want = (uint32_t)__builtin_popcountll(mask);
                    const uint32_t U = p.slot_stride - 1u;
                    const uint32_t k_open = __umulhi(tile_u + U - 1u, p.slotu_magic);
                    const uint32_t n_free = (uint32_t)__builtin_popcount(freem);
                    const uint32_t slot_room = (k_open + n_free) * U - tile_u;
                    const uint32_t take = min(want, min(tile_units - tile_u, slot_room));
                    stall = take < want && take == slot_room;
                    const uint32_t n_new = __umulhi(tile_u + take + U - 1u, p.slotu_magic) - k_open;
                    const uint32_t rank = __builtin_amdgcn_mbcnt_hi((uint32_t)(mask >> 32), __builtin_amdgcn_mbcnt_lo((uint32_t)mask, 0u));
                    got = need && rank < take;
                    tv = tile_u + rank;
                    const uint32_t k = __umulhi(tv, p.slotu_magic);
                    const uint32_t unit = tv - __umul24(k, U);
                    uint32_t m = freem;
                    for (uint32_t i = 0; i + 1u < n_new; i++) m = k > k_open + i ? (m & (m - 1u)) : m;
                    const uint32_t slot = k >= k_open ? (uint32_t)__builtin_ctz(m | 0x80000000u) : cur_slot;
                    if (got) {
                        useq = (slot << 24) | unit;
                        if (unit == 0u) {
                            const uint32_t un = min(U, tile_units - tv);
                            wq.cnt[slot] = un;
                            uint32_t* hdr = reinterpret_cast<uint32_t*>(ring + __umul24(slot, p.slot_stride) * 3u);
                            hdr[0] = tile_x0 + __umul24(k, p.grp);
                            hdr[1] = tile_row;
                            hdr[2] = (tile_meta & 0xffu) | (div_spp(un) << 8) | (tile_meta & 0xff0000u);
                        }
                    }
                    tile_u = uni(tile_u + take);
                    if (n_new) {
                        uint32_t fm = freem;
                        for (uint32_t i = 0; i + 1u < n_new; i++) fm &= fm - 1u;
                        cur_slot = uni((uint32_t)__builtin_ctz(fm));
                        freem = uni(fm & (fm - 1u));
                    }
                }
                TSTAMP(7);
                if (got) {
                    WCOUNT(1);
                    LCOUNT(0);
                    const uint32_t j = div_spp(tv);
                    px = tile_x0 + j;
                    pyg = tile_yg;
                    rng = seed_state(tile_seed + (uint64_t)(tv + __umul24(j, p.gap)) * (4ull * PHI));
                    have_unit = true;
                    need_ray = true;
                    bounce = false;
                    need = false;
                }
                if (stall) { LCOUNT(14); break; }
            }
        }
        const bool active = have_unit;
        if (!active) { LCOUNT(13); }
        TSTAMP(0);
        if (active && need_ray) {
            float x1, x2, sm;
            WCOUNT(2);
            for (;;) {
                WCOUNT(3);
                LCOUNT(1);
                x1 = uniform_m1_1(rng);
                x2 = uniform_m1_1(rng);
                sm = x1 * x1 + x2 * x2;
                if (bounce ? !(sm >= 1.0f) : (sm <= 1.0f)) break;
            }
            V3 xdir, pre, fallback;
            LCOUNT(2);
            if (bounce) {
                LCOUNT(3);
                const float factor = 2.0f * RT_SQRT(1.0f - sm);
                const V3 us = mk(x1 * factor, x2 * factor, 1.0f - 2.0f * sm);
                const V3 diffuse_dir = us + bn;
                const V3 glossy_dir = d - (2.0f * dot(d, bn)) * bn;
                pre = diffuse_dir + brough * (glossy_dir - diffuse_dir);
                fallback = bn;
            } else {
                LCOUNT(4);
                const V3 offset = lens_offset(p, x1, x2);
                const float u = ((float)px + gen_range_01(rng)) / p.u_den;
                const float v = ((float)(p.H - pyg - 1) + gen_range_01(rng)) / p.v_den;
                const V3 dir0 = normalize_or_zero(llc + u * hor + v * ver - corg);
                const V3 d1 = normalize(dir0);
                const V3 focal_point = corg + p.focus_distance * d1;
                o = corg + offset;
                pre = focal_point - o;
                fallback = mk(0.f, 0.f, 0.f);
                depth_left = p.depth;
                k = 0;
            }
            if (!try_normalize(pre, xdir)) xdir = fallback;
            d = normalize(xdir);
            need_ray = false;
            bounce = false;
        }
        TSTAMP(1);
        const bool wave_busy = __ballot(active) != 0ull || freem != all_free || !q_drained || tile_u != tile_units;
        if (STREAMED) {
            if (!__syncthreads_or(wave_busy ? 1 : 0)) break;
        } else {
            if (!wave_busy) break;
        }

        if (active && !in_trav) {
            h.idx = -1;
            aux = ray_aux(d, (p.flags & 8u) != 0);
            if (!TRAVERSE) td = 2.0f * d;
            n_seg++;
            if (QNODES) {
                const V3 og = mk((o.x - p.q_base[0]) * p.q_rstep[0], (o.y - p.q_base[1]) * p.q_rstep[1], (o.z - p.q_base[2]) * p.q_rstep[2]);
                ig = mk(p.q_step[0] * aux.inv.x, p.q_step[1] * aux.inv.y, p.q_step[2] * aux.inv.z);
                cq = mk(-(og.x * ig.x), -(og.y * ig.y), -(og.z * ig.z));
                const float big = 0x1p100f, tiny = 0x1p-60f;
                const float ax = __builtin_fabsf(ig.x), ay = __builtin_fabsf(ig.y), az = __builtin_fabsf(ig.z);
                qfin = aux.finite && ax < big && ay < big && az < big && ax > tiny && ay > tiny && az > tiny &&
                       __builtin_fabsf(og.x) < 0x1p18f && __builtin_fabsf(og.y) < 0x1p18f && __builtin_fabsf(og.z) < 0x1p18f;
            }
            if (LTREE) {
                aux.finite = aux.finite && __builtin_fabsf(o.x) < __builtin_inff() && __builtin_fabsf(o.y) < __builtin_inff() &&
                             __builtin_fabsf(o.z) < __builtin_inff();
                sgx = aux.sx ? 1u : 0u;
                sgy = aux.sy ? 1u : 0u;
                sgz = aux.sz ? 1u : 0u;
            }
            if (CULL) {
                t_far = __builtin_inff();
                for (uint32_t j = 0; j < p.n_big; j++) {
                    const uint32_t prim = p.big[j];
                    float t;
                    bool hit;
                    if (prim < p.n_sph) {
                        const float4 g = RT_SPHERE_REC(p, prim);
                        hit = exact_sphere(o, 2.0f * d, mk(g.x, g.y, g.z), g.w, p.t_min, p.t_max, t);
                    } else {
                        hit = exact_triangle(o, d, p.tri + 9 * (size_t)(prim - p.n_sph), p.t_min, p.t_max, t);
                    }
                    if (hit)
                        consider_if<true>(h, (int)prim, o, d, t, [&]() { return bvh_reaches(p.bvh_nodes, p.leaf_of[prim], o, AUX()); }, p.leaf_of);
                }
                if (h.idx >= 0) t_far = far_bound(h.dist);
            }
            if (TRAVERSE) {
                t_ref = p.root_ref;
                t_sp = BFSTEP ? 1u : 0u;
                t_cnt = 0;
                in_trav = (p.n_sph + p.n_tri) > 0;
            }
        }
        if constexpr (TRAVERSE) {
            auto root_test = [&](uint32_t i) {
                    LCOUNT(6);
                    const uint32_t prim = LTREE ? (uint32_t)lc16[i * BLOCK + tid16] & 0x7fffu
                                          : p.list16 ? (uint32_t)lc16[i * BLOCK + tid16] : lc32[i * BLOCK + tid];
                    float t;
                    if (prim < p.n_sph) {
                        const float4 g = RT_SPHERE_REC(p, prim);
                        if (exact_sphere(o, 2.0f * d, mk(g.x, g.y, g.z), g.w, p.t_min, p.t_max, t)) {
                            if (QNODES)
                                consider_if<CULL>(h, (int)prim, o, d, t, [&]() {
                                    if (!qfin || (p.n_sph + p.n_tri) == 1) return true;
                                    const float4 s = at32(p.geom_r, prim);
                                    return intersects_aabb_finite(o, AUX(), make_float4(s.x - s.w, s.y - s.w, s.z - s.w, 0.f),
                                                                  make_float4(s.x + s.w, s.y + s.w, s.z + s.w, 0.f));
                                }, p.leaf_of);
                            else if (CULL)
                                consider<1>(h, (int)prim, o, d, t, aux, p.bvh_nodes, p.leaf_of);
                            else
                                consider<0>(h, (int)prim, o, d, t, aux, p.bvh_nodes, p.leaf_of);
                        }
                    } else {
                        if (exact_triangle(o, d, p.tri + 9 * (size_t)(prim - p.n_sph), p.t_min, p.t_max, t)) {
                            if (QNODES)
                                consider_if(h, (int)prim, o, d, t,
                                            [&]() { return !qfin || bvh_reaches(p.bvh_nodes, p.leaf_of[prim], o, AUX()); });
                            else if (CULL)
                                consider<1>(h, (int)prim, o, d, t, aux, p.bvh_nodes, p.leaf_of);
                            else
                                consider<0>(h, (int)prim, o, d, t, aux, p.bvh_nodes, p.leaf_of);
                        }
                    }
            };
            auto flush = [&]() {
                if (BFSTEP) n_cand += t_cnt - t_head;
#pragma clang loop unroll(disable)
                for (uint32_t i = BFSTEP ? t_head : 0u; i < t_cnt; i++) root_test(i);
                t_cnt = 0;
                if (BFSTEP) t_head = 0;
                if (CULL && h.idx >= 0) t_far = far_bound(h.dist);
            };
            auto flush_one = [&]() {
                n_cand++;
                root_test(t_head);
                t_head++;
                if (t_head == t_cnt) t_head = t_cnt = 0;
                if (CULL && h.idx >= 0) t_far = far_bound(h.dist);
            };

            constexpr bool COMPACT = XNODES;
            auto flush_c = [&](bool want) {
                const uint32_t cnt = want ? t_cnt : 0u;
                uint32_t excl = 0, total = 0;
#pragma unroll
                for (int b = 0; b < 4; b++) {
                    const unsigned long long m = __ballot(((cnt >> b) & 1u) != 0);
                    excl += (uint32_t)__builtin_amdgcn_mbcnt_hi((uint32_t)(m >> 32), __builtin_amdgcn_mbcnt_lo((uint32_t)m, 0u)) << b;
                    total += (uint32_t)__builtin_popcountll(m) << b;
                }
                const unsigned long long act = __ballot(true);
                const uint32_t n_act = (uint32_t)__builtin_popcountll(act);
                const uint32_t rank = (uint32_t)__builtin_amdgcn_mbcnt_hi((uint32_t)(act >> 32), __builtin_amdgcn_mbcnt_lo((uint32_t)act, 0u));
                uint32_t* const w_pref = reinterpret_cast<uint32_t*>(lds_raw + p.lds_cmp_off) + (tid >> 6) * 256;
                float* const w_dist = reinterpret_cast<float*>(w_pref + 64);
                float* const w_root = reinterpret_cast<float*>(w_pref + 128);
                uint32_t* const w_hit = w_pref + 192;
                w_pref[rank] = excl | ((uint32_t)lane << 16);
                __builtin_amdgcn_fence(__ATOMIC_ACQ_REL, "wavefront");
                int best_k = -1;
                float best_t = 0.f;
                auto own_prim = [&](uint32_t k) -> uint32_t {
                    return p.list16 ? (uint32_t)lc16[k * BLOCK + tid16] : lc32[k * BLOCK + tid];
                };
                for (uint32_t base = 0; base < total; base += n_act) {
                    const uint32_t j = base + rank;
                    const bool valid = j < total;
                    uint32_t R = 0, ent = w_pref[0];
                    if (valid) {
#pragma unroll
                        for (uint32_t stp = 32; stp > 0; stp >>= 1) {
                            const uint32_t c = R + stp;
                            if (c < n_act) {
                                const uint32_t e = w_pref[c];
                                if ((e & 0xffffu) <= j) { R = c; ent = e; }
                            }
                        }
                    }
                    const uint32_t L = ent >> 16, slot = j - (ent & 0xffffu);
                    const V3 ro = mk(__shfl(o.x, (int)L, 64), __shfl(o.y, (int)L, 64), __shfl(o.z, (int)L, 64));
                    const V3 rd = mk(__shfl(d.x, (int)L, 64), __shfl(d.y, (int)L, 64), __shfl(d.z, (int)L, 64));
                    bool hit = false;
                    float t = 0.f, dist = 0.f;
                    if (valid) {
                        LCOUNT(6);
                        const uint32_t ot = ((uint32_t)tid & ~63u) | L;
                        const uint32_t ot16 = (ot & ~63u) | ((ot & 31u) << 1) | ((ot >> 5) & 1u);
                        const uint32_t prim = p.list16 ? (uint32_t)lc16[slot * BLOCK + ot16] : lc32[slot * BLOCK + ot];
                        if (prim < p.n_sph) {
                            const float4 g = RT_SPHERE_REC(p, prim);
                            hit = exact_sphere(ro, 2.0f * rd, mk(g.x, g.y, g.z), g.w, p.t_min, p.t_max, t);
                        } else {
                            hit = exact_triangle(ro, rd, p.tri + 9 * (size_t)(prim - p.n_sph), p.t_min, p.t_max, t);
                        }
                        if (hit) {
                            const V3 pp = ro + t * rd;
                            dist = vlength(pp - ro);
                        }
                    }
                    w_dist[rank] = dist;
                    w_root[rank] = t;
                    w_hit[rank] = hit ? 1u : 0u;
                    __builtin_amdgcn_fence(__ATOMIC_ACQ_REL, "wavefront");
                    if (cnt) {
                        const uint32_t k0 = excl > base ? excl : base, k1 = min(excl + cnt, base + n_act);
#pragma clang loop unroll(disable)
                        for (uint32_t k = k0; k < k1; k++) {
                            if (!w_hit[k - base]) continue;
                            const float dk = w_dist[k - base];
                            bool take = best_k < 0 ? (h.idx < 0 || h.dist > dk) : (h.dist > dk);
                            if (CULL && !take && h.dist == dk && (best_k >= 0 || h.idx >= 0)) {
                                const uint32_t cur = best_k >= 0 ? own_prim((uint32_t)best_k) : (uint32_t)h.idx;
                                take = p.leaf_of[own_prim(k - excl)] < p.leaf_of[cur];
                            }
                            if (take) {
                                h.dist = dk;
                                best_k = (int)(k - excl);
                                best_t = w_root[k - base];
                            }
                        }
                    }
                    __builtin_amdgcn_fence(__ATOMIC_ACQ_REL, "wavefront");
                }
                if (best_k >= 0) {
                    h.idx = (int)own_prim((uint32_t)best_k);
                    h.t = best_t;
                }
                if (want) t_cnt = 0;
                if (CULL && want && h.idx >= 0) t_far = far_bound(h.dist);
            };
            auto push = [&](uint32_t v) {
                if (LTREE) lstack16[t_sp * BLOCK + tid16] = (uint16_t)v;
                else if (!CAPPED || t_sp < p.stack_lds) lstack[t_sp * BLOCK + tid] = v;
                else p.stack_ovf[(size_t)(t_sp - p.stack_lds) * p.ovf_stride + (blockIdx.x * BLOCK + tid)] = v;
                t_sp++;
            };
            auto pop = [&]() -> uint32_t {
                --t_sp;
                if (LTREE) return (uint32_t)lstack16[t_sp * BLOCK + tid16];
                if (!CAPPED || t_sp < p.stack_lds) return lstack[t_sp * BLOCK + tid];
                return p.stack_ovf[(size_t)(t_sp - p.stack_lds) * p.ovf_stride + (blockIdx.x * BLOCK + tid)];
            };
            if constexpr (BFSTEP) {
            const uint32_t DONE = lt_r0(p.n_internal) + p.n_internal * (uint32_t)LNODE_DW;
            constexpr int STEPS = RT_STEPS_PER_CHECK_LTREE;
            static_assert(MAXL_LTREE > STEPS, "the leaf list must take a block of appends");
            constexpr uint32_t SLOT = (uint32_t)BLOCK * 2u;
            typedef __attribute__((address_space(3))) unsigned char lds_byte;
            typedef __attribute__((address_space(3))) uint16_t lds_u16;
            const uint32_t lds0 = (uint32_t)(uintptr_t)(lds_byte*)lds_raw;
            const uint32_t stack0_a = lds0 + p.lds_stack_off + (uint32_t)tid16 * 2u;
            const uint32_t list0_m = lds0 + p.lds_cand_off + (uint32_t)tid16 * 2u - SLOT;
            uint32_t top_a = 0, cnt_m = 0;
            auto lds16 = [&](uint32_t a) -> lds_u16& { return *(lds_u16*)(uintptr_t)a; };
            auto step = [&](auto slow_tag) {
                constexpr bool SLOW = decltype(slow_tag)::value;
                static_assert(SLOT == 0x800u, "leaf flag 0x8000 >> 4 must be one slot");
                const uint32_t leaf_slot = (t_ref >> 4) & SLOT;
                const uint32_t ni = t_ref;
                if (STATS) n_int += (ni < DONE) ? 1u : 0u;
                const uint32_t top = (uint32_t)lds16(top_a);
                WCOUNT(5);
                LCOUNT(5);
                lds16(cnt_m + SLOT) = (uint16_t)t_ref;
                const float* __restrict__ nd = lnodes + ni;
                const float* __restrict__ fx = nd + sgx;
                const float* __restrict__ fy = nd + 6 + sgy;
                const float* __restrict__ fz = nd + 12 + sgz;
                const float p0 = fx[0], p1 = fx[1], p2 = fx[3], p3 = fx[4], p4 = fy[0], p5 = fy[1], p6 = fy[3], p7 = fy[4];
                const float p8 = fz[0], p9 = fz[1], p10 = fz[3], p11 = fz[4];
                const uint32_t refs = __float_as_uint(nd[18]);
                RT_HOOK_LT_STEP_LOADS(nd, ni, lnodes);
                __builtin_amdgcn_sched_barrier(0);
                RT_HOOK_LT_STEP_ALU(p0, p1, p2, p3, o.y);
                const float lxn = (p0 - o.x) * aux.inv.x, lxf = (p1 - o.x) * aux.inv.x;
                const float rxn = (p2 - o.x) * aux.inv.x, rxf = (p3 - o.x) * aux.inv.x;
                const float lyn = (p4 - o.y) * aux.inv.y, lyf = (p5 - o.y) * aux.inv.y;
                const float ryn = (p6 - o.y) * aux.inv.y, ryf = (p7 - o.y) * aux.inv.y;
                const float lzn = (p8 - o.z) * aux.inv.z, lzf = (p9 - o.z) * aux.inv.z;
                const float rzn = (p10 - o.z) * aux.inv.z, rzf = (p11 - o.z) * aux.inv.z;
                bool hl, hr;
                float le, re;
                if (SLOW) {
                    le = rmax(rmax(rmax(lxn, lyn), lzn), 0.0f);
                    re = rmax(rmax(rmax(rxn, ryn), rzn), 0.0f);
                    hl = le <= rmin(rmin(lxf, lyf), lzf);
                    hr = re <= rmin(rmin(rxf, ryf), rzf);
                } else {
                    le = __builtin_fmaxf(__builtin_fmaxf(__builtin_fmaxf(lxn, lyn), lzn), 0.0f);
                    re = __builtin_fmaxf(__builtin_fmaxf(__builtin_fmaxf(rxn, ryn), rzn), 0.0f);
                    hl = le <= __builtin_fminf(__builtin_fminf(lxf, lyf), lzf);
                    hr = re <= __builtin_fminf(__builtin_fminf(rxf, ryf), rzf);
                }
                uint32_t cl = refs & 0xffffu, cr = refs >> 16;
                if (CULL) {
                    hl = hl && le <= t_far;
                    hr = hr && re <= t_far;
                    const bool swp = hl && hr && re < le;
                    const uint32_t c0 = cl;
                    cl = swp ? cr : cl;
                    cr = swp ? c0 : cr;
                }
                lds16(top_a + SLOT) = (uint16_t)cr;
                const bool any = hl || hr;
                t_ref = any ? (hl ? cl : cr) : top;
                uint32_t delta = any ? 0u : 0u - SLOT;
                delta = (hl && hr) ? SLOT : delta;
                asm volatile("" : "+v"(delta));
                top_a += delta;
                if (SLOW) top_a = max(top_a, stack0_a);
                cnt_m += leaf_slot;
                RT_HOOK_LT_STEP_END;
            };
            for (;;) {
                const uint32_t walking = (uint32_t)__builtin_popcountll(__ballot(in_trav));
                const uint32_t live = (uint32_t)__builtin_popcountll(__ballot(active));
                if (walking == 0 || (walking * 8 <= live * p.refill_eighths && walking < live)) break;
                if (in_trav && t_cnt > p.maxl - (uint32_t)STEPS) flush();
                if (RT_LT_PARTIAL < 64) {
                    const bool pend = t_cnt > t_head;
                    if ((int)__builtin_popcountll(__ballot(pend)) >= RT_LT_PARTIAL ||
                        (CULL && (int)__builtin_popcountll(__ballot(pend && h.idx < 0)) >= RT_LT_EAGER)) {
                        if (pend) flush_one();
                    }
                }
                const bool slow = __ballot(in_trav && !aux.finite) != 0;
                if (in_trav) {
                    top_a = stack0_a + (t_sp - 1u) * SLOT;
                    cnt_m = list0_m + t_cnt * SLOT;
                    if (slow) {
#pragma unroll
                        for (int rep = 0; rep < STEPS; rep++) step(std::true_type{});
                    } else {
#pragma unroll
                        for (int rep = 0; rep < STEPS; rep++) step(std::false_type{});
                    }
                    t_sp = (top_a + SLOT - stack0_a) / SLOT;
                    t_cnt = (cnt_m - list0_m) / SLOT;
                    in_trav = t_ref != DONE;
                }
            }
            } else {
            for (;;) {
                const uint32_t walking = (uint32_t)__builtin_popcountll(__ballot(in_trav));
                const uint32_t live = (uint32_t)__builtin_popcountll(__ballot(active));
                if (walking == 0 || (walking * 8 <= live * p.refill_eighths && walking < live)) break;
#ifndef RT_FLUSH_INLINE
                if (COMPACT && p.lds_cmp_off != 0xffffffffu) {
                    const bool want = in_trav && (t_cnt == ML || (CULL && t_cnt >= (uint32_t)RT_CULL_FLUSH_MIN && h.idx < 0));
                    if (__ballot(want)) flush_c(want);
                } else
                if (in_trav && (t_cnt == ML || (CULL && t_cnt >= (uint32_t)RT_CULL_FLUSH_MIN && h.idx < 0))) flush();
#endif
                constexpr bool BF2 = (RT_BF2 != 0) && (XNODES || QNODES);
                if (BF2 && !__ballot(in_trav && !(QNODES ? qfin : aux.finite))) {
#pragma unroll
                    for (int rep = 0; rep < (QNODES ? RT_STEPS_PER_CHECK_Q : RT_STEPS_PER_CHECK_X); rep++)
                    if (in_trav) {
                        WCOUNT(5);
                        LCOUNT(5);
                        const bool is_leaf = (t_ref & LEAF_BIT) != 0;
                        if (STATS) n_int += is_leaf ? 0u : 1u;
                        const uint32_t tsl = t_sp - (t_sp ? 1u : 0u);
                        uint32_t top = lstack[(CAPPED ? min(tsl, p.stack_lds - 1u) : tsl) * BLOCK + tid];
                        bool hl, hr;
                        float le = 0.f, re = 0.f;
                        uint32_t c0, c1;
                        if constexpr (QNODES) {
                        const uint4* __restrict__ nq = reinterpret_cast<const uint4*>(reinterpret_cast<const char*>(p.travq) + ((is_leaf ? 0u : t_ref) << 5));
                        uint4 qa = nq[0], qb = nq[1];
                        asm volatile("" : "+v"(qb.x), "+v"(qb.y), "+v"(qb.z), "+v"(qb.w));
                        float lmin, lmax, rmin_, rmax_;
                        qslabs(qa, qb, ig, cq, lmin, lmax, rmin_, rmax_);
                        le = __builtin_fmaxf(lmin, 0.0f);
                        re = __builtin_fmaxf(rmin_, 0.0f);
                        hl = le <= (CULL ? __builtin_fminf(lmax, t_far) : lmax);
                        hr = re <= (CULL ? __builtin_fminf(rmax_, t_far) : rmax_);
                        c0 = qb.z;
                        c1 = qb.w;
                        } else {
                        const float4* __restrict__ nd = reinterpret_cast<const float4*>(reinterpret_cast<const char*>(p.trav) + ((is_leaf ? 0u : t_ref) << 6));
                        const float4 n0 = nd[0], n1 = nd[1], n2 = nd[2], n3 = nd[3];
                        if (CULL) {
                            float lmin, lmax, rmin_, rmax_;
                            slabs_finite(o, aux, n0, n1, lmin, lmax);
                            slabs_finite(o, aux, n2, n3, rmin_, rmax_);
                            le = __builtin_fmaxf(lmin, 0.0f);
                            re = __builtin_fmaxf(rmin_, 0.0f);
                            hl = le <= lmax && le <= t_far;
                            hr = re <= rmax_ && re <= t_far;
                        } else {
                            hl = intersects_aabb_finite(o, aux, n0, n1);
                            hr = intersects_aabb_finite(o, aux, n2, n3);
                        }
                        c0 = __float_as_uint(n0.w);
                        c1 = __float_as_uint(n1.w);
                        }
                        hl = hl && !is_leaf;
                        hr = hr && !is_leaf;
                        const bool both = hl && hr, any = hl || hr;
                        const bool swp = CULL && both && re < le;
                        const uint32_t cl = swp ? c1 : c0, cr = swp ? c0 : c1;
                        if (!CAPPED || t_sp < p.stack_lds) lstack[t_sp * BLOCK + tid] = cr;
                        else if (both) p.stack_ovf[(size_t)(t_sp - p.stack_lds) * p.ovf_stride + (blockIdx.x * BLOCK + tid)] = cr;
                        const bool can = t_cnt < ML, app = is_leaf && can, stall = is_leaf && !can;
                        if (app) {
                            if (p.list16) lc16[t_cnt * BLOCK + tid16] = (uint16_t)t_ref;
                            else lc32[t_cnt * BLOCK + tid] = t_ref & ~LEAF_BIT;
                        }
                        t_cnt += app ? 1u : 0u;
                        n_cand += app ? 1u : 0u;
                        const bool pop_ = !any && !stall, empty = t_sp == 0;
                        if (CAPPED && pop_ && t_sp > p.stack_lds)
                            top = p.stack_ovf[(size_t)(t_sp - 1u - p.stack_lds) * p.ovf_stride + (blockIdx.x * BLOCK + tid)];
                        t_ref = stall ? t_ref : any ? (hl ? cl : cr) : top;
                        in_trav = !(pop_ && empty);
                        t_sp = t_sp + (both ? 1u : 0u) - ((pop_ && !empty) ? 1u : 0u);
                    }
                } else
#if defined(RT_ROLL_STEPS) || RT_BF2
#pragma clang loop unroll(disable)
#else
#pragma unroll
#endif
                for (int rep = 0; rep < (QNODES ? RT_STEPS_PER_CHECK_Q : RT_STEPS_PER_CHECK); rep++)
                if (in_trav) {
                    WCOUNT(5);
                    LCOUNT(5);
                    if (t_ref & LB) {
#ifdef RT_FLUSH_INLINE
                        if (t_cnt == ML) flush();
#else
                        if (t_cnt == ML) continue;
#endif
                        if (p.list16) lc16[t_cnt * BLOCK + tid16] = (uint16_t)t_ref;
                        else lc32[t_cnt * BLOCK + tid] = t_ref & ~LEAF_BIT;
                        t_cnt++;
                        n_cand++;
                        if (t_sp == 0) {
                            in_trav = false;
                        } else {
                            t_ref = pop();
                        }
                    } else {
                        bool hl, hr;
                        uint32_t cl, cr;
                        if (STATS) n_int++;
                        if (QNODES) {
                            const uint4* __restrict__ nq = reinterpret_cast<const uint4*>(reinterpret_cast<const char*>(p.travq) + (t_ref << 5));
                            uint4 qa = nq[0], qb = nq[1];
                            asm volatile("" : "+v"(qb.x), "+v"(qb.y), "+v"(qb.z), "+v"(qb.w));
                            cl = qb.z;
                            cr = qb.w;
                            RT_HOOK_Q_GATHER(t_ref, cl, p.travq, p.n_internal);
                            if (qfin) {
                                float lmin, lmax, rmin_, rmax_;
                                qslabs(qa, qb, ig, cq, lmin, lmax, rmin_, rmax_);
                                if (CULL) {
                                    const float le = __builtin_fmaxf(lmin, 0.0f), re = __builtin_fmaxf(rmin_, 0.0f);
                                    hl = le <= __builtin_fminf(lmax, t_far);
                                    hr = re <= __builtin_fminf(rmax_, t_far);
                                    if (hl && hr && re < le) {
                                        const uint32_t t = cl;
                                        cl = cr;
                                        cr = t;
                                    }
                                } else {
                                    hl = __builtin_fmaxf(lmin, 0.0f) <= lmax;
                                    hr = __builtin_fmaxf(rmin_, 0.0f) <= rmax_;
                                }
                            } else {
                                const float4* __restrict__ nd = reinterpret_cast<const float4*>(reinterpret_cast<const char*>(p.trav) + (t_ref << 6));
                                const RayAux ax = AUX();
                                hl = intersects_aabb(o, ax, nd[0], nd[1]);
                                hr = intersects_aabb(o, ax, nd[2], nd[3]);
                            }
                        } else {
                            const float4* __restrict__ nd = reinterpret_cast<const float4*>(reinterpret_cast<const char*>(p.trav) + (t_ref << 6));
                            const float4 n0 = nd[0], n1 = nd[1], n2 = nd[2], n3 = nd[3];
                            if (aux.finite) {
                                hl = intersects_aabb_finite(o, aux, n0, n1);
                                hr = intersects_aabb_finite(o, aux, n2, n3);
                            } else {
                                hl = intersects_aabb(o, aux, n0, n1);
                                hr = intersects_aabb(o, aux, n2, n3);
                            }
                            cl = __float_as_uint(n0.w);
                            cr = __float_as_uint(n1.w);
                        }
                        if (hl) {
                            if (hr) push(cr);
                            t_ref = cl;
                        } else if (hr) {
                            t_ref = cr;
                        } else if (t_sp == 0) {
                            in_trav = false;
                        } else {
                            t_ref = pop();
                        }
                    }
                }
            }
            }
            TSTAMP(2);
            if (COMPACT && p.lds_cmp_off != 0xffffffffu) {
                const bool want = active && !in_trav && t_cnt > 0;
                if (__ballot(want)) flush_c(want);
            } else
            if (active && !in_trav) flush();
            TSTAMP(3);
        } else {
            bool seg_active = active;
            bool inline_chain = false;
            for (;;) {
                if (seg_active) h.idx = -1;
                for (uint32_t ch = 0; ch < p.n_chunks; ch++) {
                    const uint32_t base = ch * p.chunk;
                    const uint32_t cn = min(p.chunk, p.n_sph_pad - base);
                    if (STREAMED) {
                        __syncthreads();
                        for (uint32_t i = tid; i < cn; i += BLOCK) lgeom[i] = gsrc[base + i];
                        if (EXPANDED)
                            for (uint32_t i = tid; i < cn; i += BLOCK) lrr[i] = p.geom[base + i].w;
                        __syncthreads();
                    }
                    if (seg_active) {
                        uint32_t cnt = 0;
                        if (!exact_scan) {
                            uint32_t ncand_it = 0;
                            v2f k0x, k0y, k0z, k1x, k1y, k1z, kA, kB;
                            if (EXPANDED) {
                                const float A = __builtin_fmaf(d.z, o.z, __builtin_fmaf(d.y, o.y, d.x * o.x));
                                const float oo =
                                    __builtin_fmaf(o.z, o.z, __builtin_fmaf(o.y, o.y, o.x * o.x)) * (1.0f - 0x1p-16f);
                                k0x = v2f{-d.x, -d.x}; k0y = v2f{-d.y, -d.y}; k0z = v2f{-d.z, -d.z};
                                k1x = v2f{-2.0f * o.x, -2.0f * o.x}; k1y = v2f{-2.0f * o.y, -2.0f * o.y};
                                k1z = v2f{-2.0f * o.z, -2.0f * o.z};
                                kA = v2f{A, A};
                                kB = v2f{oo, oo};
                            } else {
                                k0x = v2f{o.x, o.x}; k0y = v2f{o.y, o.y}; k0z = v2f{o.z, o.z};
                                k1x = v2f{d.x, d.x}; k1y = v2f{d.y, d.y}; k1z = v2f{d.z, d.z};
                                kA = NKM;
                                kB = NKM;
                            }
                            for (uint32_t j = 0; j < cn; j += UNROLL) {
                                float t[UNROLL];
    #pragma unroll
                                for (int q = 0; q < UNROLL / 2; q++) {
                                    const float4 A4 = lgeom[j + 2 * q];
                                    const float4 B4 = lgeom[j + 2 * q + 1];
                                    const v2f cx = {A4.x, A4.y}, cy = {A4.z, A4.w}, cz = {B4.x, B4.y}, cw = {B4.z, B4.w};
                                    v2f tt;
                                    if (EXPANDED) {
                                        const v2f bb = pk_fma(k0x, cx, pk_fma(k0y, cy, pk_fma(k0z, cz, kA)));
                                        const v2f qq = pk_fma(k1x, cx, pk_fma(k1y, cy, pk_fma(k1z, cz, cw + kB)));
                                        tt = pk_fma(bb, bb, -qq);
                                    } else {
                                        const v2f ocx = k0x - cx, ocy = k0y - cy, ocz = k0z - cz;
                                        const v2f bb = pk_fma(k1z, ocz, pk_fma(k1y, ocy, k1x * ocx));
                                        const v2f l2 = pk_fma(ocz, ocz, pk_fma(ocy, ocy, ocx * ocx));
                                        tt = pk_fma(l2, kA, pk_fma(bb, bb, cw));
                                    }
                                    t[2 * q] = tt.x;
                                    t[2 * q + 1] = tt.y;
                                }
                                const float m = __builtin_fmaxf(
                                    __builtin_fmaxf(__builtin_fmaxf(t[0], t[1]), __builtin_fmaxf(t[2], t[3])),
                                    __builtin_fmaxf(__builtin_fmaxf(t[4], t[5]), __builtin_fmaxf(t[6], t[7])));
                                if (!(m < 0.0f)) {
                                    WCOUNT(4);
                                    uint32_t neg = 0;
    #pragma unroll
                                    for (int q = 0; q < UNROLL; q++) neg |= (__float_as_uint(t[q]) >> 31) << q;
                                    const uint32_t pass8 = ~neg & 0xffu;
                                    if (cnt < (uint32_t)MAXC) lcand[cnt * BLOCK + tid] = (uint16_t)(((j >> 3) << 8) | pass8);
                                    cnt++;
                                    ncand_it += (uint32_t)__builtin_popcount(pass8);
                                }
                            }
                            if (!inline_chain) n_cand += ncand_it;
                        }
                        const bool direct = exact_scan || cnt > (uint32_t)MAXC;
                        if (!exact_scan && direct && !inline_chain) n_fall++;
                        const uint32_t n_ent = direct ? (cn >> 3) : cnt;
                        uint32_t ei = 0, grp = 0, bits = 0;
                        for (;;) {
                            if (bits == 0) {
                                if (ei == n_ent) break;
                                if (direct) {
                                    grp = ei;
                                    bits = 0xffu;
                                } else {
                                    const uint32_t e = lcand[ei * BLOCK + tid];
                                    grp = e >> 8;
                                    bits = e & 0xffu;
                                }
                                ei++;
                                if (bits == 0) continue;
                            }
                            WCOUNT(5);
                            const uint32_t j = grp * 8 + (uint32_t)__builtin_ctz(bits);
                            bits &= bits - 1;
                            const uint32_t fo = (j >> 1) * 8 + (j & 1);
                            const V3 cen = mk(lgeomf[fo], lgeomf[fo + 2], lgeomf[fo + 4]);
                            const float rr = EXPANDED ? lrr[j] : lgeomf[fo + 6];
                            float t;
                            if (exact_sphere(o, td, cen, rr, p.t_min, p.t_max, t)) {
                                WCOUNT(6);
                                if (!use_bvh) {
                                    if (p.world_rank) consider<1>(h, (int)(base + j), o, d, t, aux, p.bvh_nodes, p.world_rank);
                                    else consider<0>(h, (int)(base + j), o, d, t, aux, p.bvh_nodes, p.leaf_of);
                                } else if (inline_chain)
                                    consider<2>(h, (int)(base + j), o, d, t, aux, p.bvh_nodes, p.leaf_of);
                                else
                                    consider<1>(h, (int)(base + j), o, d, t, aux, p.bvh_nodes, p.leaf_of);
                            }
                        }
                    }
                }
                if (seg_active) {
                    for (uint32_t j = 0; j < p.n_tri; j++) {
                        if (use_bvh && p.n_sph + p.n_tri > 1 &&
                            !intersects_aabb(o, aux, p.tri_box[2 * (size_t)j], p.tri_box[2 * (size_t)j + 1]))
                            continue;
                        float t;
                        if (exact_triangle(o, d, p.tri + 9 * (size_t)j, p.t_min, p.t_max, t)) {
                            if (!use_bvh) {
                                if (p.world_rank) consider<1>(h, (int)(p.n_sph + j), o, d, t, aux, p.bvh_nodes, p.world_rank);
                                else consider<0>(h, (int)(p.n_sph + j), o, d, t, aux, p.bvh_nodes, p.leaf_of);
                            } else if (inline_chain)
                                consider<2>(h, (int)(p.n_sph + j), o, d, t, aux, p.bvh_nodes, p.leaf_of);
                            else
                                consider<1>(h, (int)(p.n_sph + j), o, d, t, aux, p.bvh_nodes, p.leaf_of);
                        }
                    }
                }
                bool redo = false;
                if (seg_active && use_bvh && !inline_chain && h.idx >= 0) {
                    WCOUNT(7);
                    redo = !bvh_reaches(p.bvh_nodes, p.leaf_of[h.idx], o, aux);
                }
                if (STREAMED) {
                    if (!__syncthreads_or(redo ? 1 : 0)) break;
                } else {
                    if (!redo) break;
                }
                seg_active = redo;
                inline_chain = true;
            }
        }
        if (active && !in_trav) {
            float term_r, term_g, term_b;
            bool finished;
            LCOUNT(7);
            const bool hit = h.idx >= 0;
            float em = 0.f;
            float4 m = make_float4(0.f, 0.f, 0.f, 0.f);
            V3 hp = o, nv = d;
            if (hit) {
                WCOUNT(8);
                LCOUNT(8);
                em = at32(p.emis, (uint32_t)h.idx);
                m = at32(p.mat, (uint32_t)h.idx);
                if (!(em > 0.0f)) {
                    hp = o + h.t * d;
                    if ((uint32_t)h.idx < p.n_sph) {
                        float4 g = TRAVERSE ? RT_SPHERE_REC(p, (uint32_t)h.idx) : at32(p.geom, (uint32_t)h.idx);
                        nv = hp - mk(g.x, g.y, g.z);
                    } else {
                        const float* tv = p.tri + 9 * (size_t)(h.idx - p.n_sph);
                        V3 A = mk(tv[0], tv[1], tv[2]), B = mk(tv[3], tv[4], tv[5]), C = mk(tv[6], tv[7], tv[8]);
                        nv = cross(A - B, A - C);
                    }
                }
            }
            const V3 nn = normalize_or_zero(nv);
            if (hit) {
                if (em > 0.0f) {
                    term_r = m.x * em;
                    term_g = m.y * em;
                    term_b = m.z * em;
                    finished = true;
                } else {
                    const V3 n = nn;
                    if (p.path32)
                        reinterpret_cast<uint32_t*>(lpath)[k * BLOCK + cold<QNODES>(tid)] = (uint32_t)h.idx;
                    else
                        reinterpret_cast<uint16_t*>(lpath)[k * BLOCK + cold<QNODES>(tid16)] = (uint16_t)h.idx;
                    k++;
                    depth_left--;
                    if (depth_left == 0) {
                        WCOUNT(9);
                        for (;;) {
                            WCOUNT(10);
                            const float y1 = uniform_m1_1(rng);
                            const float y2 = uniform_m1_1(rng);
                            if (!(y1 * y1 + y2 * y2 >= 1.0f)) break;
                        }
                    } else {
                        o = hp;
                        bn = n;
                        brough = m.w;
                        bounce = true;
                        need_ray = true;
                    }
                    finished = (depth_left == 0);
                    term_r = term_g = term_b = 0.0f;
                }
            } else {
                WCOUNT(11);
                LCOUNT(9);
                float t = nn.y * 0.5f + 1.0f;
                float omt = 1.0f - t;
                term_r = 1.0f * t + 0.3f * omt;
                term_g = 1.0f * t + 0.3f * omt;
                term_b = 1.0f * t + 0.8f * omt;
                finished = true;
            }
            if (finished) {
                WCOUNT(12);
                LCOUNT(10);
                {
                    auto path_idx = [&](uint32_t i) -> uint32_t {
                        return p.path32 ? reinterpret_cast<uint32_t*>(lpath)[i * BLOCK + cold<QNODES>(tid)]
                                        : (uint32_t) reinterpret_cast<uint16_t*>(lpath)[i * BLOCK + cold<QNODES>(tid16)];
                    };
                    uint32_t i = k;
#pragma clang loop unroll(disable)
                    while (i >= 2) {
                        WCOUNT(13);
                        LCOUNT(11);
                        const float4 ma = at32(p.mat, path_idx(i - 1)), mb = at32(p.mat, path_idx(i - 2));
                        term_r = mb.x * (ma.x * term_r);
                        term_g = mb.y * (ma.y * term_g);
                        term_b = mb.z * (ma.z * term_b);
                        i -= 2;
                    }
                    if (i) {
                        WCOUNT(13);
                        LCOUNT(11);
                        const float4 ma = at32(p.mat, path_idx(0));
                        term_r = ma.x * term_r;
                        term_g = ma.y * term_g;
                        term_b = ma.z * term_b;
                    }
                }
                {
                    const uint32_t slot = useq >> 24;
                    float* r = ring + (__umul24(slot, p.slot_stride) + 1u + (useq & 0xffffffu)) * 3u;
                    r[0] = term_r;
                    r[1] = term_g;
                    r[2] = term_b;
                    const uint32_t usegs = k + ((hit && !(em > 0.0f)) ? 0u : 1u);
                    (void)__hip_atomic_fetch_add(&wq.cnt[slot], (usegs << SLOT_UNIT_BITS) - 1u, __ATOMIC_RELAXED, __HIP_MEMORY_SCOPE_WAVEFRONT);
                    have_unit = false;
                }
            }
        }
        TSTAMP(4);
    }

    if (p.strip_cost && lane < 2 && wq.cost_acc[lane])
        atomicAdd(&p.strip_cost[(blockIdx.x % COST_COPIES) * MAX_BATCH + wq.cost_strip[lane]], (unsigned long long)wq.cost_acc[lane]);
    drain_counters();
    TFLUSH;
#undef wq
#undef wst
}

using KernelFn = void (*)(const KParams);
KernelFn kernel_linear(int isect, bool expanded);
KernelFn kernel_traverse(int isect, bool stats);
void sqrt_selftest_launch(uint32_t from, unsigned long long n, unsigned long long* d_bad, hipStream_t st);

}
```

ray_tracer_s8_amd/csrc/rt_kernels_trav.hip:

```cpp
#include "rt_kernel.hip.h"

namespace rtk {
template <bool STATS>
KernelFn traverse_kernel(int isect) {
    switch (isect) {
        case 5: return rt_tile_kernel<5, false, LTREE_BLOCK, STATS>;
        case 6: return rt_tile_kernel<6, false, LTREE_BLOCK, STATS>;
        case 7: return rt_tile_kernel<7, false, BLOCK, STATS>;
        case 8: return rt_tile_kernel<8, false, BLOCK, STATS>;
        case 9: return rt_tile_kernel<9, false, BLOCK, STATS>;
        case 3: return rt_tile_kernel<3, false, BLOCK, STATS>;
        case 2: return rt_tile_kernel<2, false, BLOCK, STATS>;
        case 4: return rt_tile_kernel<4, false, BLOCK, STATS>;
        default: return nullptr;
    }
}
KernelFn kernel_traverse(int isect, bool stats) { return stats ? traverse_kernel<true>(isect) : traverse_kernel<false>(isect); }

__global__ void sqrt_selftest_kernel(uint32_t from, unsigned long long n, unsigned long long* bad) {
    unsigned long long mine = 0;
    for (unsigned long long i = blockIdx.x * (unsigned long long)blockDim.x + threadIdx.x; i < n; i += (unsigned long long)gridDim.x * blockDim.x) {
        float x = __uint_as_float(from + (uint32_t)i);
        asm volatile("" : "+v"(x));
        const float ref = __builtin_sqrtf(x);
        const float a = sqrt_rn(x), b = sqrt_rn<true>(x);
        const bool both_nan_a = (a != a) && (ref != ref), both_nan_b = (b != b) && (ref != ref);
        if (__float_as_uint(a) != __float_as_uint(ref) && !both_nan_a) mine++;
        if (__float_as_uint(b) != __float_as_uint(ref) && !both_nan_b) mine++;
    }
    if (mine) atomicAdd(bad, mine);
}
void sqrt_selftest_launch(uint32_t from, unsigned long long n, unsigned long long* d_bad, hipStream_t st) {
    hipLaunchKernelGGL(sqrt_selftest_kernel, dim3(4096), dim3(256), 0, st, from, n, d_bad);
}
}

#ifdef RT_DEBUG_HOOKS
#define RT_UNIT_ID 1
#include "rt_unit.hip.h"
#endif
```

ray_tracer_s8_amd/csrc/rt_plan.h:

```cpp
#pragma once
#include <algorithm>
#include <cmath>
#include <cstddef>
#include <cstdint>

#include "rt_consts.h"
#include "rt_tile.h"

namespace rtplan {

constexpr size_t LDS_LIMIT = 160 * 1024 - 3072;
constexpr uint32_t RESIDENT_MAX = rtk::CHUNK;
constexpr uint32_t STREAM_CHUNK = 2048;
constexpr uint32_t STACK_LDS_MAX = 12;
constexpr uint32_t RT_QNODES_MIN_PRIMS = 4096;
constexpr uint32_t DENSE_SCAN_MAX_PRIMS = 192;
constexpr float DENSE_SCAN_MIN_DENSITY = 3.0f;
constexpr float DENSE_MID_MIN_DENSITY = 2.5f;
constexpr uint32_t DENSE_MID_MIN_PRIMS = 512;
constexpr float FIELD_MID_MIN_DENSITY = 0.15f;
constexpr float LT_CULL_MIN_DENSITY = 2.2f;
constexpr uint32_t TRAVERSE_MIN_PRIMS = 2;

struct SceneShape {
    uint32_t n_sph = 0, n_sph_pad = 0, n_tri = 0;
    uint32_t bvh_depth = 0, n_internal = 0;
    uint32_t root_ref = 0;
    float cull_density = 0.f;
    bool cull_pays = false;
    bool xcull_pays = false;
    bool quant_ok = false;
    bool tri_ok = false;
    float r_slack = 0.f;
    bool inverted_boxes = false;
    bool expanded = false;
    float leaf_density = 0.f;
};

struct Knobs {
    int lds_tree = 1;
    int cull_walk = -1;
    int no_stage = 0;
    int slots = 0;
    int commit_slots = 0;
    int force_capped = 0;
    int stack_lds = 0;
    int compact = 1;
    int refill_eighths = 0;
    int tail_tiles = -1;
};

struct Engine {
    int isect, isect_capped, block;
};
constexpr Engine ENGINES[8] = {
    {0, -1, rtk::BLOCK},
    {1, -1, rtk::BLOCK},
    {2, -1, rtk::BLOCK},
    {3, 4, rtk::BLOCK},
    {5, -1, rtk::LTREE_BLOCK},
    {7, 8, rtk::BLOCK},
    {9, -1, rtk::BLOCK},
    {6, -1, rtk::LTREE_BLOCK},
};
constexpr int N_ISECT = 10;

struct SampleRange {
    uint32_t begin, end;
    bool pass;
};

struct Plan {
    int status = RT_OK;
    const char* error = nullptr;
    int engine = 0;
    bool capped = false;
    int isect = 0;
    int block = rtk::BLOCK;
    bool expanded = false;
    bool count_steps = false;
    size_t lds = 0;
    uint32_t maxl_l2 = 0;
    uint32_t ovf_entries = 0;
    uint32_t blocks = 0;
    size_t ring_bytes = 0;
    size_t ovf_words = 0;
};

inline bool cull_wanted(uint32_t flags, int knob, bool rule) {
    return (flags & RT_FLAG_NO_CULL_WALK) ? false : (flags & RT_FLAG_CULL_WALK) ? true : knob >= 0 ? knob != 0 : rule;
}

struct Pose {
    float origin[3];
    float u[3], v[3], w[3];
};

inline float length3(const float a[3]) { return std::sqrt((a[0] * a[0] + a[1] * a[1]) + a[2] * a[2]); }
inline void cross3(const float a[3], const float b[3], float out[3]) {
    out[0] = a[1] * b[2] - a[2] * b[1];
    out[1] = a[2] * b[0] - a[0] * b[2];
    out[2] = a[0] * b[1] - a[1] * b[0];
}

inline bool make_pose(const rt_camera& c, Pose& ps) {
    if (c.flags != 0 || c.reserved != 0) return false;
    for (int i = 0; i < 3; i++)
        if (!std::isfinite(c.origin[i]) || !std::isfinite(c.target[i]) || !std::isfinite(c.up[i])) return false;
    Pose r;
    float d[3], x[3];
    for (int i = 0; i < 3; i++) d[i] = c.origin[i] - c.target[i];
    const float ld = length3(d);
    if (!(ld > 0.0f) || !std::isfinite(ld)) return false;
    for (int i = 0; i < 3; i++) r.w[i] = d[i] / ld;
    cross3(c.up, r.w, x);
    const float lx = length3(x);
    if (!(lx > 0.0f) || !std::isfinite(lx)) return false;
    for (int i = 0; i < 3; i++) r.u[i] = x[i] / lx;
    cross3(r.w, r.u, r.v);
    for (int i = 0; i < 3; i++) r.origin[i] = c.origin[i];
    ps = r;
    return true;
}

template <class KP>
auto set_lens(KP& p, const float lu[3], const float lv[3], int) -> decltype((void)p.lens_u[0]) {
    for (int i = 0; i < 3; i++) {
        p.lens_u[i] = lu[i];
        p.lens_v[i] = lv[i];
    }
}
template <class KP>
void set_lens(KP&, const float*, const float*, long) {}

template <class KP>
void fill_camera(const rt_tile_request& rq, KP& p) {
    const float origin[3] = {0.f, 0.f, 0.f};
    const float aspect_ratio = (float)rq.width / (float)rq.height;
    const float image_height = (float)rq.height;
    const float vh = 2.0f * std::tan(rq.fov / 2.0f);
    const float vw = aspect_ratio * vh;
    const float hor[3] = {vw, 0.f, 0.f}, ver[3] = {0.f, vh, 0.f};
    const float foc[3] = {0.f, 0.f, rq.focal_length};
    for (int i = 0; i < 3; i++) {
        p.org[i] = origin[i];
        p.hor[i] = hor[i];
        p.ver[i] = ver[i];
        float v = origin[i] - hor[i] / 2.0f;
        v = v - ver[i] / 2.0f;
        v = v - foc[i];
        p.llc[i] = v;
    }
    p.lens_radius = rq.aperture / 2.0f;
    const float lens_u[3] = {p.lens_radius, 0.f, 0.f}, lens_v[3] = {0.f, p.lens_radius, 0.f};
    set_lens(p, lens_u, lens_v, 0);
    p.focus_distance = rq.focus_distance;
    p.u_den = aspect_ratio * image_height - 1.0f;
    p.v_den = image_height - 1.0f;
}

template <class KP>
void fill_camera(const rt_tile_request& rq, const Pose& ps, KP& p) {
    const float aspect_ratio = (float)rq.width / (float)rq.height;
    const float image_height = (float)rq.height;
    const float vh = 2.0f * std::tan(rq.fov / 2.0f);
    const float vw = aspect_ratio * vh;
    p.lens_radius = rq.aperture / 2.0f;
    float lens_u[3], lens_v[3];
    for (int i = 0; i < 3; i++) {
        const float hor = vw * ps.u[i], ver = vh * ps.v[i], foc = rq.focal_length * ps.w[i];
        p.org[i] = ps.origin[i];
        p.hor[i] = hor;
        p.ver[i] = ver;
        float v = ps.origin[i] - hor / 2.0f;
        v = v - ver / 2.0f;
        v = v - foc;
        p.llc[i] = v;
        lens_u[i] = p.lens_radius * ps.u[i];
        lens_v[i] = p.lens_radius * ps.v[i];
    }
    set_lens(p, lens_u, lens_v, 0);
    p.focus_distance = rq.focus_distance;
    p.u_den = aspect_ratio * image_height - 1.0f;
    p.v_den = image_height - 1.0f;
}

template <class KP>
void fill_camera(const rt_tile_request& rq, const Pose* pose, KP& p) {
    if (pose) fill_camera(rq, *pose, p);
    else fill_camera(rq, p);
}

template <class KP>
Plan plan_launch(const SceneShape& sh, const rt_tile_request& rq, uint32_t n_strips, const SampleRange& smp, const Knobs& kn, KP& p,
                 const Pose* pose = nullptr) {
    using namespace rtk;
    Plan pl;
    p.W = rq.width;
    p.H = rq.height;
    p.Hs = rq.height / rq.divisions;
    const uint32_t s_begin = smp.begin, s_end = smp.end;
    p.upp = s_end - s_begin;
    p.spp_all = rq.spp;
    p.s_begin = s_begin;
    p.gap = rq.spp - p.upp;
    p.acc_out = smp.pass ? 1u : 0u;
    p.depth = rq.max_bounces + 1;
    p.n_sph = sh.n_sph;
    p.n_sph_pad = sh.n_sph_pad;
    p.n_tri = sh.n_tri;
    p.flags = rq.flags;
    if (sh.inverted_boxes) p.flags |= RT_FLAG_FULL_CHAIN;
    const uint32_t fl = rq.flags;
    const uint32_t n_prims = sh.n_sph + sh.n_tri;
    const bool trav_ok = !(fl & (RT_FLAG_EXACT_SCAN | RT_FLAG_NO_BVH_CULL | RT_FLAG_LINEAR_SCAN)) &&
                         sh.bvh_depth < (uint32_t)TRAV_STACK && n_prims > 0;
    const bool dense_pile = sh.n_tri == 0 && n_prims <= DENSE_SCAN_MAX_PRIMS && sh.cull_density >= DENSE_SCAN_MIN_DENSITY;
    const bool traverse = trav_ok && ((fl & RT_FLAG_BVH_TRAVERSE) || (n_prims >= TRAVERSE_MIN_PRIMS && !dense_pile));
    bool ltree_fits = false;
    const size_t lt_lane = ((size_t)MAXL_LTREE + (size_t)(rq.max_bounces + 1) + (size_t)(sh.bvh_depth + 2)) * sizeof(uint16_t);
    if (traverse && kn.lds_tree != 0 && !(fl & RT_FLAG_NO_LDS_TREE) && sh.n_internal > 0 && n_prims <= 0x7fffu &&
        ((size_t)sh.n_internal + 2) * LNODE_DW < 0x8000u) {
        const size_t fixed = (((size_t)sh.n_internal + 2) * LNODE_DW + n_prims) * 4 + 16 + lt_lane * LTREE_BLOCK;
        ltree_fits = fixed <= LDS_LIMIT;
    }
    const bool dense_mid = sh.cull_pays && !(fl & RT_FLAG_NO_CULL_WALK) && !ltree_fits && sh.cull_density >= DENSE_MID_MIN_DENSITY &&
                           n_prims >= DENSE_MID_MIN_PRIMS;
    const bool field_mid = !ltree_fits && sh.n_tri == 0 && n_prims < RT_QNODES_MIN_PRIMS && sh.cull_density >= FIELD_MID_MIN_DENSITY;
    const bool qnodes = traverse && sh.quant_ok && !(fl & RT_FLAG_EXACT_NODES) &&
                        ((fl & RT_FLAG_QUANT_NODES) || (n_prims >= RT_QNODES_MIN_PRIMS && sh.n_tri <= sh.n_sph) || dense_mid ||
                         field_mid);
    const bool ltree = ltree_fits && !qnodes;
    const bool cull = qnodes && cull_wanted(fl, kn.cull_walk, sh.cull_pays) && sh.n_tri == 0 && std::isfinite(sh.r_slack);
    const bool xcull = traverse && !qnodes && !ltree && cull_wanted(fl, kn.cull_walk, sh.xcull_pays) && sh.n_tri > 0 && sh.tri_ok &&
                       std::isfinite(sh.r_slack) && !sh.inverted_boxes;
    const bool lt_cull_ok = ltree && !sh.inverted_boxes && std::isfinite(sh.r_slack) && (sh.n_tri == 0 || sh.tri_ok);
    const bool ltcull = lt_cull_ok && cull_wanted(fl, kn.cull_walk, sh.cull_density >= LT_CULL_MIN_DENSITY);
    const bool streamed = !traverse && sh.n_sph_pad > RESIDENT_MAX;
    pl.engine = traverse ? (ltree ? (ltcull ? 7 : 4) : qnodes ? (cull ? 5 : 3) : xcull ? 6 : 2) : (streamed ? 1 : 0);
    const int bs = ENGINES[pl.engine].block;
    p.chunk = traverse ? 0 : (streamed ? STREAM_CHUNK : sh.n_sph_pad);
    p.n_chunks = p.chunk ? (sh.n_sph_pad + p.chunk - 1) / p.chunk : 0;
    p.path32 = (sh.n_sph + sh.n_tri) > 65536u ? 1u : 0u;
    size_t geom_bytes = traverse ? 0 : (size_t)(p.chunk ? p.chunk : 1) * 4 * sizeof(float);
    p.lds_cand_off = (uint32_t)geom_bytes;
    size_t path_bytes = (size_t)p.depth * BLOCK * (p.path32 ? 4 : 2);
    const bool want_stage = kn.no_stage == 0 && ((traverse && !ltree) || streamed);
    const bool list16 = traverse && !ltree && n_prims <= 65536u;
    const size_t stage_bytes_wg = (size_t)STAGE_TILES * STAGE_TILE_BYTES * (bs / 64);
    const uint32_t stack_capped = sh.bvh_depth + 1;
    const uint32_t stack_need = sh.bvh_depth + (ltree ? 2u : 1u);
    uint32_t maxl = qnodes ? (uint32_t)MAXL : (uint32_t)MAXL_EXACT, stack_lds = stack_need;
    if (traverse && qnodes) {
        const size_t per_wg = (160u * 1024u - 4096u) / 5u - 512u;
        const size_t slot = (size_t)BLOCK * (list16 ? sizeof(uint16_t) : sizeof(uint32_t));
        const size_t fixed = path_bytes + (size_t)stack_need * BLOCK * sizeof(uint32_t) + (want_stage ? stage_bytes_wg : 0);
        if (kn.force_capped == 0 && fixed + (size_t)MINL * slot <= per_wg) {
            maxl = (uint32_t)std::min<size_t>((size_t)MAXL, (per_wg - fixed) / slot);
        } else {
            const uint32_t cap = kn.stack_lds > 0 ? (uint32_t)kn.stack_lds : STACK_LDS_MAX;
            pl.capped = stack_capped > cap;
            stack_lds = pl.capped ? cap : stack_need;
        }
    }
    p.maxl = maxl;
    p.stack_lds = stack_lds;
    p.list16 = list16 ? 1u : 0u;
    size_t cand_bytes = traverse ? (size_t)maxl * BLOCK * (list16 ? sizeof(uint16_t) : sizeof(uint32_t))
                                 : (size_t)MAXC * BLOCK * sizeof(uint16_t);
    p.lds_path_off = (uint32_t)(geom_bytes + cand_bytes);
    const bool expanded = !traverse && sh.expanded && !(fl & RT_FLAG_OC_BROAD_PHASE);
    p.lds_rr_off = (uint32_t)(geom_bytes + cand_bytes + path_bytes);
    size_t rr_bytes = expanded ? (size_t)(p.chunk ? p.chunk : 1) * sizeof(float) : 0;
    p.lds_stack_off = (uint32_t)(geom_bytes + cand_bytes + path_bytes + rr_bytes);
    size_t stack_bytes = traverse ? (size_t)stack_lds * BLOCK * sizeof(uint32_t) : 0;
    size_t lds = geom_bytes + cand_bytes + path_bytes + rr_bytes + stack_bytes;
    p.n_internal = sh.n_internal;
    p.lds_node_off = 0;
    if (ltree) {
        size_t off = ((((size_t)sh.n_internal + 2) * LNODE_DW + n_prims) * 4 + 15) & ~(size_t)15;
        p.lds_cand_off = (uint32_t)off;
        uint32_t lt_maxl = MAXL_LTREE;
        while (lt_maxl < (uint32_t)MAXL_LTREE_MAX &&
               off + ((size_t)(lt_maxl + 1) + p.depth + stack_need) * bs * sizeof(uint16_t) <= LDS_LIMIT) lt_maxl++;
        p.maxl = lt_maxl;
        off += (size_t)lt_maxl * bs * sizeof(uint16_t);
        p.lds_path_off = (uint32_t)off;
        off += (size_t)p.depth * bs * sizeof(uint16_t);
        p.lds_stack_off = (uint32_t)off;
        off += (size_t)stack_need * bs * sizeof(uint16_t);
        lds = off;
    }
    p.lds_cmp_off = 0xffffffffu;
    if (traverse && !qnodes && !ltree && kn.compact != 0 && lds + 1024u * (BLOCK / 64) + 16 <= LDS_LIMIT) {
        lds = (lds + 15) & ~(size_t)15;
        p.lds_cmp_off = (uint32_t)lds;
        lds += 1024u * (BLOCK / 64);
    }
    p.lds_stage_off = 0xffffffffu;
    if (want_stage && lds + stage_bytes_wg <= LDS_LIMIT) {
        lds = (lds + 15) & ~(size_t)15;
        p.lds_stage_off = (uint32_t)lds;
        lds += stage_bytes_wg;
    }
    pl.lds = lds;
    if (lds > LDS_LIMIT) {
        pl.status = RT_ERR_LIMIT;
        pl.error = "LDS budget exceeded (scene chunk + path stack)";
        return pl;
    }
    pl.isect = pl.capped ? ENGINES[pl.engine].isect_capped : ENGINES[pl.engine].isect;
    pl.block = bs;
    pl.expanded = expanded;
    pl.count_steps = traverse && (fl & RT_FLAG_COUNT_STEPS);
    pl.maxl_l2 = maxl;
    pl.ovf_entries = pl.capped ? stack_capped - stack_lds : 0u;
    fill_camera(rq, pose, p);
    p.t_min = rq.t_min;
    p.t_max = rq.t_max;
    p.spp_f = (float)s_end;
    p.spp_rcp = (s_end & (s_end - 1u)) == 0u ? 1.0f / (float)s_end : 0.0f;
    p.root_ref = sh.root_ref;
    if (ltree) p.root_ref = (p.root_ref & LEAF_BIT) ? (0x8000u | (p.root_ref & 0x7fffu)) : lt_r0(sh.n_internal) + p.root_ref * (uint32_t)LNODE_DW;
    p.refill_eighths = kn.refill_eighths > 0 ? (uint32_t)kn.refill_eighths : (n_prims >= RT_QNODES_MIN_PRIMS ? 4u : 2u);
    p.n_strips = n_strips;
    p.tiles_x = (p.W + 63u) / 64u;
    p.tiles_per_strip = p.tiles_x * p.Hs;
    {
        p.grp = p.upp >= 8u ? 1u : (8u + p.upp - 1u) / p.upp;
        const uint64_t slot_units = (uint64_t)p.grp * p.upp;
        p.grp_magic = p.grp > 1u ? (uint32_t)((1ull << 32) / p.grp) + 1u : 0u;
        p.slot_stride = 1u + (uint32_t)slot_units;
        const uint64_t fewest = slot_units <= 256u ? 16u : slot_units <= 1024u ? 8u : 4u;
        p.n_slots = kn.slots > 0 ? std::min<uint32_t>((uint32_t)kn.slots, SLOTS_MAX)
                                 : (uint32_t)std::min<uint64_t>(SLOTS_MAX, std::max<uint64_t>(fewest, 384u / slot_units));
        const uint32_t cs = kn.commit_slots > 0 ? (uint32_t)kn.commit_slots : std::max<uint32_t>(1u, p.n_slots / 4u);
        p.commit_slots = std::min<uint32_t>(cs, p.n_slots);
        p.spp_magic = p.upp > 1u ? (uint32_t)((1ull << 32) / p.upp) + 1u : 0u;
        p.slotu_magic = (uint32_t)((1ull << 32) / slot_units) + 1u;
    }
    const uint64_t n_tiles = (uint64_t)p.tiles_per_strip * n_strips;
    if (n_tiles > 0x1fffffffull) {
        pl.status = RT_ERR_LIMIT;
        pl.error = "too many tiles in one launch";
        return pl;
    }
    p.tiles_total = (uint32_t)n_tiles;
    p.n_tiles = (uint32_t)n_tiles;
    p.tiles_big = (uint32_t)n_tiles;
    return pl;
}

template <class KP>
void plan_queue(Plan& pl, uint32_t blocks, const Knobs& kn, KP& p) {
    const uint32_t waves_per_wg = (uint32_t)pl.block / 64u;
    const uint32_t useful = (p.n_tiles + waves_per_wg - 1) / waves_per_wg;
    if (blocks > useful) blocks = useful ? useful : 1;
    pl.blocks = blocks;
    const uint64_t waves = (uint64_t)blocks * waves_per_wg;
    const bool all_parts = p.tiles_total < 16ull * waves || p.upp > 16u;
    const uint64_t conv = std::min<uint64_t>(p.tiles_total, kn.tail_tiles >= 0 ? (uint64_t)kn.tail_tiles : all_parts ? (uint64_t)p.tiles_total : 2ull * waves);
    p.sub_shift = p.upp > 32u ? 4u : 2u;
    if ((((uint64_t)p.tiles_total - conv) + (conv << p.sub_shift)) > 0x7fffffffull) p.sub_shift = 2u;
    p.tiles_big = p.tiles_total - (uint32_t)conv;
    p.n_tiles = p.tiles_big + ((uint32_t)conv << p.sub_shift);
    p.ovf_stride = blocks * (uint32_t)pl.block;
    pl.ovf_words = (size_t)pl.ovf_entries * p.ovf_stride;
    pl.ring_bytes = (size_t)blocks * waves_per_wg * p.n_slots * p.slot_stride * 12u;
}

constexpr int QUERY_BLOCK = 256;

struct QueryPlan {
    int engine = 2;
    int scan_mode = 2;
    bool full_chain = false;
    size_t lds = 0;
};

inline QueryPlan plan_query(const SceneShape& sh, uint32_t flags) {
    QueryPlan q;
    const uint32_t n_prims = sh.n_sph + sh.n_tri;
    const bool no_cull = (flags & RT_FLAG_NO_BVH_CULL) != 0;
    const bool walk = !no_cull && !(flags & (RT_FLAG_EXACT_SCAN | RT_FLAG_LINEAR_SCAN)) && n_prims > 0 &&
                      sh.bvh_depth < (uint32_t)rtk::TRAV_STACK;
    q.engine = walk ? 2 : 1;
    q.scan_mode = no_cull ? 0 : 2;
    q.full_chain = (flags & RT_FLAG_FULL_CHAIN) != 0 || sh.inverted_boxes;
    q.lds = walk ? ((size_t)sh.bvh_depth + 1) * QUERY_BLOCK * sizeof(uint32_t) : 0;
    return q;
}

constexpr uint32_t DIRECT_MAX_LIGHTS = 1u << 23;

struct DirectPlan {
    QueryPlan query;
    bool too_many = false;
};

inline DirectPlan plan_direct(const SceneShape& sh, uint32_t n_lights, uint32_t flags) {
    DirectPlan d;
    d.query = plan_query(sh, flags);
    d.too_many = n_lights > DIRECT_MAX_LIGHTS;
    return d;
}

using NeePlan = DirectPlan;

inline NeePlan plan_nee(const SceneShape& sh, uint32_t n_lights, uint32_t flags) { return plan_direct(sh, n_lights, flags); }

constexpr uint32_t TRACE_LDS_CU = 160 * 1024;
constexpr uint32_t TRACE_BLOCKS[] = {256, 128, 64};

struct TracePlan {
    int engine = 2;
    int scan_mode = 2;
    bool full_chain = false;
    uint32_t block = 256;
    bool path32 = false;
    size_t lds_path_off = 0;
    size_t lds = 0;
};

inline TracePlan plan_trace(const SceneShape& sh, uint32_t flags, uint32_t max_bounces) {
    const QueryPlan q = plan_query(sh, flags);
    TracePlan t;
    t.engine = q.engine;
    t.scan_mode = q.scan_mode;
    t.full_chain = q.full_chain;
    t.path32 = (sh.n_sph + sh.n_tri) > 65536u;
    const size_t stack_lane = q.engine == 2 ? ((size_t)sh.bvh_depth + 1) * sizeof(uint32_t) : 0;
    const size_t path_lane = ((size_t)max_bounces + 1) * (t.path32 ? 4 : 2);
    for (uint32_t b : TRACE_BLOCKS) {
        t.block = b;
        if (2 * (stack_lane + path_lane) * b <= TRACE_LDS_CU) break;
    }
    t.lds_path_off = stack_lane * t.block;
    t.lds = (stack_lane + path_lane) * t.block;
    return t;
}

constexpr uint32_t DN_TILE_X = 64, DN_TILE_Y = 4, DN_BLOCK = DN_TILE_X * DN_TILE_Y;
constexpr uint32_t DN_MAX_ITER = 8;
constexpr uint32_t DN_LDS_MAX_STEP = 2;
constexpr size_t DN_LDS_CU = 160 * 1024;
constexpr uint32_t DN_WG_PER_CU_MAX = 8;
constexpr size_t DN_REC = 16;
constexpr size_t DN_ALIGN = 256;

struct DenoisePlan {
    uint64_t npix = 0;
    uint32_t tiles_x = 0;
    size_t off_guide = 0;
    size_t off_color[2] = {0, 0};
    size_t scratch_bytes = 0;
    uint32_t step[DN_MAX_ITER] = {};
    size_t lds[DN_MAX_ITER] = {};
    uint32_t wg_per_cu[DN_MAX_ITER] = {};
};

inline size_t dn_align(size_t b) { return (b + DN_ALIGN - 1) / DN_ALIGN * DN_ALIGN; }

inline size_t dn_window_bytes(uint32_t s, bool guided) {
    return (size_t)(DN_TILE_X + 4 * s) * (DN_TILE_Y + 4 * s) * DN_REC * (guided ? 2 : 1);
}

inline DenoisePlan plan_denoise(uint32_t W, uint32_t R, uint32_t iterations, bool guided, uint32_t lds_max_step = DN_LDS_MAX_STEP) {
    DenoisePlan p;
    p.npix = (uint64_t)W * R;
    p.tiles_x = (W + DN_TILE_X - 1) / DN_TILE_X;
    const size_t buf = dn_align((size_t)p.npix * DN_REC);
    p.off_guide = 0;
    p.off_color[0] = buf;
    p.off_color[1] = 2 * buf;
    p.scratch_bytes = 3 * buf;
    for (uint32_t i = 0; i < iterations && i < DN_MAX_ITER; i++) {
        const uint32_t s = 1u << i;
        p.step[i] = s;
        const size_t b = dn_window_bytes(s, guided);
        if (s <= lds_max_step && b <= DN_LDS_CU) {
            p.lds[i] = b;
            p.wg_per_cu[i] = (uint32_t)std::min<size_t>(DN_WG_PER_CU_MAX, DN_LDS_CU / b);
        } else {
            p.wg_per_cu[i] = DN_WG_PER_CU_MAX;
        }
    }
    return p;
}

}
```

Before: 15760.

## Split LDS-tree kernel into walker and shading waves with LDS handoff ring

Adds a specialised form of the LDS-tree traversal kernel (engine 4). Within each workgroup, some waves only walk the BVH and the rest only shade. Walkers post hit results into LDS mailboxes and a lock-free ring, so traversal and shading run concurrently instead of diverging within the same wave. The LDS layout is re-planned with a narrower per-walker stack and leaf list. A timeout and give-up counter void the launch if the handoff deadlocks, at the cost of extra synchronisation, LDS and fewer waves doing traversal.

```diff
diff --git a/ray_tracer_s8_amd/csrc/rt_api.hip b/ray_tracer_s8_amd/csrc/rt_api.hip
--- a/ray_tracer_s8_amd/csrc/rt_api.hip
+++ b/ray_tracer_s8_amd/csrc/rt_api.hip
@@ -120,13 +120,14 @@
     DBG_TAIL_TILES,
     DBG_STRIP_COST,
     DBG_DENOISE_LDS_STEP,
+    DBG_LT_SPLIT,
     DBG_N
 };
 std::atomic<int> g_dbg[DBG_N];
 const struct { const char* env; int def; } g_dbg_spec[DBG_N] = {
     {"RT_LDS_TREE", 1}, {"RT_CULL_WALK", -1}, {"RT_NO_STAGE", 0}, {"RT_SLOTS", 0}, {"RT_FORCE_CAPPED", 0},
     {"RT_STACK_LDS", 0}, {"RT_COMPACT", 1}, {"RT_REFILL_EIGHTHS", 0}, {"RT_COMMIT_SLOTS", 0}, {"RT_VERBOSE", 0}, {"RT_REORDER", 1}, {"RT_TAIL_TILES", -1}, {"RT_STRIP_COST", 1},
-    {"RT_DENOISE_LDS_STEP", -1}};
+    {"RT_DENOISE_LDS_STEP", -1}, {"RT_LT_SPLIT", -1}};
 std::once_flag g_dbg_once;
 void dbg_load_env() {
     std::call_once(g_dbg_once, [] {
@@ -157,6 +158,7 @@
     k.compact = dbg(DBG_COMPACT);
     k.refill_eighths = dbg(DBG_REFILL_EIGHTHS);
     k.tail_tiles = dbg(DBG_TAIL_TILES);
+    k.lt_split = dbg(DBG_LT_SPLIT);
     return k;
 }
 
@@ -192,6 +194,7 @@
     bool has_order = false;
     float bvh_build_ms = 0.f;
     unsigned long long* d_counters = nullptr;
+    bool split_pending = false;
     struct Ring {
         float* d = nullptr;
         size_t bytes = 0;
@@ -243,10 +246,11 @@
 
 constexpr uint32_t QUEUE_SLOTS = 16384;
 #ifdef RT_PROFILE_TIME
-constexpr uint32_t COUNTER_WORDS = 4 + QUEUE_SLOTS + 16 * 8192;
+constexpr uint32_t COUNTER_WORDS = 4 + QUEUE_SLOTS + 16 * 8192 + 1;
 #else
-constexpr uint32_t COUNTER_WORDS = 4 + QUEUE_SLOTS;
+constexpr uint32_t COUNTER_WORDS = 4 + QUEUE_SLOTS + 1;
 #endif
+constexpr uint32_t GIVEUP_WORD = COUNTER_WORDS - 1;
 
 int check_slot(const rt_scene* sc) {
     if (sc->pending.size() >= QUEUE_SLOTS) return fail(RT_ERR_LIMIT, "too many uncollected launches: call rt_scene_collect()");
@@ -393,7 +397,19 @@
     p.queue = sc->d_counters + 4 + sc->pending.size();
     p.strip_cost = dbg(DBG_STRIP_COST) ? d_strip_cost : nullptr;
 
-    const rtk::KernelFn kern = pl.isect < 2 ? rtk::kernel_linear(pl.isect, pl.expanded) : rtk::kernel_traverse(pl.isect, pl.count_steps);
+    rtk::KernelFn kern = pl.isect < 2 ? rtk::kernel_linear(pl.isect, pl.expanded) : rtk::kernel_traverse(pl.isect, pl.count_steps);
+    bool split = false;
+    p.giveup = sc->d_counters + GIVEUP_WORD;
+    if (rtplan::split_wanted(pl, sh, kn)) {
+        const rtplan::SplitPlan sp = rtplan::plan_split(sh, (uint32_t)rtk::LT_SPLIT_W, (uint32_t)rtk::LT_SPLIT_STEPS, p);
+        if (sp.ok) {
+            split = true;
+            kern = rtk::kernel_ltree_split(pl.count_steps);
+            pl.lds = sp.lds;
+            if (dbg(DBG_VERBOSE))
+                fprintf(stderr, "[rt] split form: %u walker + %u shading waves, lds %zu B, leaf rows %u, ring %u\n", sp.walkers, sp.shaders, sp.lds, sp.maxl, sp.ring_cap);
+        }
+    }
     int per_cu = 0;
     HIPCHK(hipOccupancyMaxActiveBlocksPerMultiprocessor(&per_cu, kern, pl.block, pl.lds));
     if (per_cu < 1) per_cu = 1;
@@ -420,6 +436,7 @@
     sc->last_engine = (uint32_t)pl.engine;
     sc->last_form = pl.expanded ? 1u : 0u;
     if ((rc = enqueue(sc, stream, kern, pl.blocks, pl.block, pl.lds, p))) return rc;
+    if (split) sc->split_pending = true;
     HIPCHK(hipEventRecord(rg->done, stream));
     if (p.stack_ovf) HIPCHK(hipEventRecord(sc->ovf_done, stream));
     sc->primary_rays += (uint64_t)p.Hs * p.W * p.upp * n;
@@ -441,6 +458,12 @@
     unsigned long long c[4] = {0, 0, 0, 0};
     HIPCHK(hipMemcpy(c, sc->d_counters, sizeof c, hipMemcpyDeviceToHost));
     HIPCHK(hipMemset(sc->d_counters, 0, sizeof c));
+    unsigned long long gave_up = 0;
+    if (sc->split_pending) {
+        sc->split_pending = false;
+        HIPCHK(hipMemcpy(&gave_up, sc->d_counters + GIVEUP_WORD, sizeof gave_up, hipMemcpyDeviceToHost));
+        if (gave_up) HIPCHK(hipMemset(sc->d_counters + GIVEUP_WORD, 0, sizeof gave_up));
+    }
     if (st) {
         st->ray_segments = c[0];
         st->broad_candidates = c[1];
@@ -456,6 +479,7 @@
     }
     sc->primary_rays = 0;
     sc->h2d_ms = 0.f;
+    if (gave_up) return fail(RT_ERR_HIP, "LDS-tree kernel (split form): " + std::to_string(gave_up) + " wait(s) between walker and shading waves ran out; the launch is void");
     return RT_OK;
 }
 
@@ -682,6 +706,8 @@
         for (int alt = 0; alt < 2; alt++)
             HIPCHK(hipFuncSetAttribute((const void*)(isect < 2 ? rtk::kernel_linear(isect, alt != 0) : rtk::kernel_traverse(isect, alt != 0)),
                                        hipFuncAttributeMaxDynamicSharedMemorySize, (int)rtplan::LDS_LIMIT));
+    for (int alt = 0; alt < 2; alt++)
+        HIPCHK(hipFuncSetAttribute((const void*)rtk::kernel_ltree_split(alt != 0), hipFuncAttributeMaxDynamicSharedMemorySize, (int)rtplan::LDS_LIMIT));
     hipStream_t st = nullptr, cs = nullptr;
     HIPCHK(hipStreamCreateWithFlags(&st, hipStreamNonBlocking));
     HIPCHK(hipStreamCreateWithFlags(&cs, hipStreamNonBlocking));
diff --git a/ray_tracer_s8_amd/csrc/rt_consts.h b/ray_tracer_s8_amd/csrc/rt_consts.h
--- a/ray_tracer_s8_amd/csrc/rt_consts.h
+++ b/ray_tracer_s8_amd/csrc/rt_consts.h
@@ -19,6 +19,12 @@
 #ifndef RT_MAXL_LTREE
 #define RT_MAXL_LTREE 12
 #endif
+#ifndef RT_LT_SPLIT_W
+#define RT_LT_SPLIT_W 8
+#endif
+#ifndef RT_LT_SPLIT_STEPS
+#define RT_LT_SPLIT_STEPS 8
+#endif
 
 namespace rtk {
 
@@ -36,6 +42,19 @@
 RT_HOST_DEVICE uint32_t lt_r0(uint32_t n_internal) { return 0x8000u - (n_internal + 1u) * (uint32_t)LNODE_DW; }
 constexpr int MAXL_LTREE = RT_MAXL_LTREE;
 constexpr int MAXL_LTREE_MAX = 16;
+constexpr int LT_SPLIT_W = RT_LT_SPLIT_W;
+constexpr int LT_SPLIT_STEPS = RT_LT_SPLIT_STEPS;
+static_assert(LT_SPLIT_W >= 1 && LT_SPLIT_W <= LTREE_BLOCK / 64 - 1, "walker and shading waves: at least one of each");
+constexpr uint32_t lt_split_stride(uint32_t walkers) {
+    uint32_t s = 128;
+    while (s < walkers * 128u) s <<= 1;
+    return s;
+}
+constexpr uint32_t lt_split_shift(uint32_t walkers) {
+    uint32_t sh = 0;
+    while ((0x8000u >> sh) != lt_split_stride(walkers)) sh++;
+    return sh;
+}
 constexpr uint32_t LEAF_BIT = 0x80000000u;
 constexpr uint32_t STAGE_TILE_BYTES = 192;
 constexpr uint32_t STAGE_TILES = 3;
diff --git a/ray_tracer_s8_amd/csrc/rt_handoff.h b/ray_tracer_s8_amd/csrc/rt_handoff.h
--- /dev/null
+++ b/ray_tracer_s8_amd/csrc/rt_handoff.h
@@ -0,0 +1,62 @@
+#pragma once
+#include <stdint.h>
+
+#include "rt_consts.h"
+
+namespace rthand {
+
+constexpr uint32_t RING_EMPTY_BIT = 0x8000u;
+constexpr uint32_t RING_ID_BITS = 10;
+constexpr uint32_t RING_TAG_MASK = 31u;
+constexpr uint32_t RESULT_PENDING = 0x80000000u;
+constexpr uint32_t MBOX_WORDS = 8;
+constexpr uint32_t CAS_TRIES = 8;
+
+inline constexpr uint32_t ring_capacity(uint32_t lanes) {
+    uint32_t c = 64;
+    while (c <= lanes) c <<= 1;
+    return c;
+}
+inline constexpr uint32_t ring_slot(uint32_t pos, uint32_t cap) { return pos & (cap - 1u); }
+inline constexpr uint32_t ring_tag(uint32_t pos, uint32_t cap) { return (pos / cap) & RING_TAG_MASK; }
+inline constexpr uint32_t ring_empty_for(uint32_t pos, uint32_t cap) { return RING_EMPTY_BIT | ring_tag(pos, cap); }
+inline constexpr uint32_t ring_full_of(uint32_t pos, uint32_t cap, uint32_t id) { return (ring_tag(pos, cap) << RING_ID_BITS) | id; }
+inline constexpr uint32_t ring_empty_after(uint32_t pos, uint32_t cap) { return RING_EMPTY_BIT | ((ring_tag(pos, cap) + 1u) & RING_TAG_MASK); }
+inline constexpr bool ring_is_full_of(uint32_t word, uint32_t pos, uint32_t cap) {
+    return (word & RING_EMPTY_BIT) == 0u && (word >> RING_ID_BITS) == ring_tag(pos, cap);
+}
+inline constexpr uint32_t ring_id(uint32_t word) { return word & ((1u << RING_ID_BITS) - 1u); }
+inline constexpr uint32_t ring_published(uint32_t head, uint32_t tail) { return tail - head; }
+inline constexpr uint32_t ring_take(uint32_t free, uint32_t head, uint32_t tail) {
+    const uint32_t pub = ring_published(head, tail);
+    return free < pub ? free : pub;
+}
+inline constexpr bool ring_finished(uint32_t alive, uint32_t head, uint32_t tail) { return alive == 0u && head == tail; }
+
+
+template <class A>
+RT_HOST_DEVICE __attribute__((always_inline)) uint32_t reserve_push(A& a, uint32_t n) { return a.add_tail(n); }
+
+template <class A>
+RT_HOST_DEVICE __attribute__((always_inline)) bool reserve_pop(A& a, uint32_t free, uint32_t& base, uint32_t& take) {
+    for (uint32_t i = 0; i < CAS_TRIES; i++) {
+        const uint32_t h = a.load_head(), t = a.load_tail();
+        take = ring_take(free, h, t);
+        if (take == 0u) return false;
+        if (a.cas_head(h, h + take)) {
+            base = h;
+            return true;
+        }
+    }
+    take = 0u;
+    return false;
+}
+
+template <class A>
+RT_HOST_DEVICE __attribute__((always_inline)) bool finished(A& a) {
+    const uint32_t alive = a.load_alive();
+    const uint32_t h = a.load_head(), t = a.load_tail();
+    return ring_finished(alive, h, t);
+}
+
+}
diff --git a/ray_tracer_s8_amd/csrc/rt_kernel.hip.h b/ray_tracer_s8_amd/csrc/rt_kernel.hip.h
--- a/ray_tracer_s8_amd/csrc/rt_kernel.hip.h
+++ b/ray_tracer_s8_amd/csrc/rt_kernel.hip.h
@@ -5,6 +5,7 @@
 
 #include "rt_consts.h"
 #include "rt_cull.h"
+#include "rt_handoff.h"
 
 namespace rtk {
 
@@ -46,6 +47,12 @@
 #endif
 #ifndef RT_LT_PARTIAL
 #define RT_LT_PARTIAL 40
+#endif
+#ifndef RT_LT_SPLIT_READY
+#define RT_LT_SPLIT_READY 32
+#endif
+#ifndef RT_LT_SPLIT_PRIO
+#define RT_LT_SPLIT_PRIO 0
 #endif
 #ifndef RT_LT_EAGER
 #define RT_LT_EAGER 12
@@ -141,6 +148,8 @@
     unsigned long long* strip_cost;
     unsigned long long* counters;
     unsigned long long* queue;
+    uint32_t sp_cand_off, sp_stack_off, sp_path_off, sp_mbox_off, sp_ring_off, sp_ring_cap, sp_maxl;
+    unsigned long long* giveup;
     StripDesc strips[MAX_BATCH];
 };
 
@@ -496,7 +505,19 @@
     return cull_bound_tri(best, o.x, o.y, o.z, k, diag, es, e);
 }
 
-template <int ISECT, bool EXPANDED, int BS = BLOCK, bool STATS = false>
+struct HandLds {
+    unsigned int *head, *tail, *alive;
+    __device__ __forceinline__ uint32_t load_head() { return __hip_atomic_load(head, __ATOMIC_ACQUIRE, __HIP_MEMORY_SCOPE_WORKGROUP); }
+    __device__ __forceinline__ uint32_t load_tail() { return __hip_atomic_load(tail, __ATOMIC_RELAXED, __HIP_MEMORY_SCOPE_WORKGROUP); }
+    __device__ __forceinline__ uint32_t load_alive() { return __hip_atomic_load(alive, __ATOMIC_ACQUIRE, __HIP_MEMORY_SCOPE_WORKGROUP); }
+    __device__ __forceinline__ uint32_t add_tail(uint32_t n) { return __hip_atomic_fetch_add(tail, n, __ATOMIC_RELAXED, __HIP_MEMORY_SCOPE_WORKGROUP); }
+    __device__ __forceinline__ bool cas_head(uint32_t expected, uint32_t desired) {
+        return __hip_atomic_compare_exchange_strong(head, &expected, desired, __ATOMIC_RELAXED, __ATOMIC_RELAXED, __HIP_MEMORY_SCOPE_WORKGROUP);
+    }
+};
+constexpr unsigned long long HAND_WAIT_TICKS = 5000000ull;
+
+template <int ISECT, bool EXPANDED, int BS = BLOCK, bool STATS = false, bool SPLIT = false>
 __global__ __launch_bounds__(BS, (ISECT == 5 || ISECT == 6) ? RT_MINWAVES_LTREE : ISECT == 9 ? RT_MINWAVES_TRAV : ISECT >= 7 ? RT_MINWAVES_CULL : ISECT >= 3 ? RT_MINWAVES_QTRAV : ISECT == 2 ? RT_MINWAVES_TRAV : RT_MINWAVES) void rt_tile_kernel(const KParams p) {
     constexpr int BLOCK = BS;
     constexpr bool STREAMED = (ISECT == 1);
@@ -508,10 +529,13 @@
     constexpr bool LTREE = (ISECT == 5 || ISECT == 6);
     constexpr uint32_t LB = LTREE ? 0x8000u : LEAF_BIT;
     constexpr bool BFSTEP = LTREE;
+    static_assert(!SPLIT || ISECT == 5, "the split form is the plain LDS-tree walk's");
+    constexpr uint32_t NW = SPLIT ? (uint32_t)LT_SPLIT_W : 0u, NS = (uint32_t)BS / 64u - NW;
     const uint32_t ML = QNODES ? p.maxl : (uint32_t)MAXL_EXACT;
     extern __shared__ __attribute__((aligned(16))) unsigned char lds_raw[];
     __shared__ unsigned long long wg_tiles;
     __shared__ unsigned int wg_lock, wg_drained;
+    __shared__ unsigned int hq_head, hq_tail, hq_alive, hq_abort;
     __shared__ WaveQ wave_q[BS / 64];
     constexpr bool CAN_STAGE = (ISECT >= 1 && ISECT <= 4) || ISECT >= 7;
     __shared__ WaveStage wave_st[CAN_STAGE ? BS / 64 : 1];
@@ -529,18 +553,26 @@
         wg_tiles = 0ull;
         wg_lock = 0u;
         wg_drained = 0u;
+        hq_head = hq_tail = hq_abort = 0u;
+        hq_alive = NS;
     }
     __syncthreads();
     float4* lgeom = reinterpret_cast<float4*>(lds_raw);
     const float* lgeomf = reinterpret_cast<const float*>(lds_raw);
     float* lrr = reinterpret_cast<float*>(lds_raw + p.lds_rr_off);
     const float4* __restrict__ gsrc = EXPANDED ? p.geom_px : p.geom_pk;
-    uint16_t* lcand = reinterpret_cast<uint16_t*>(lds_raw + p.lds_cand_off);
-    unsigned char* lpath = lds_raw + p.lds_path_off;
+    const uint32_t cand_off = SPLIT ? p.sp_cand_off : p.lds_cand_off, stack_off = SPLIT ? p.sp_stack_off : p.lds_stack_off;
+    uint16_t* lcand = reinterpret_cast<uint16_t*>(lds_raw + cand_off);
+    unsigned char* lpath = lds_raw + (SPLIT ? p.sp_path_off : p.lds_path_off);
 
     const int tid = threadIdx.x;
     const int lane = tid & 63;
     const int tid16 = (tid & ~63) | ((tid & 31) << 1) | ((tid >> 5) & 1);
+    const bool walker = SPLIT && uni((uint32_t)tid >> 6) < NW;
+    constexpr int LCOLS = SPLIT ? (int)(lt_split_stride(NW ? NW : 1u) / 2u) : BS, PCOLS = SPLIT ? (int)(NS * 64u) : BS;
+    const int lcol = tid16;
+    const int pcol = SPLIT ? tid16 - (int)(NW * 64u) : tid16;
+    const uint32_t sid = (uint32_t)tid - NW * 64u;
 
     if (ISECT == 0) {
         for (uint32_t i = tid; i < p.n_sph_pad; i += BLOCK) lgeom[i] = gsrc[i];
@@ -570,6 +602,8 @@
         }
         float* nanf_ = ln + LNODE_DW * (p.n_internal + 1u);
         for (uint32_t i = tid; i < p.n_sph + p.n_tri + (uint32_t)LNODE_DW; i += BLOCK) nanf_[i] = __builtin_nanf("");
+        if (SPLIT)
+            for (uint32_t i = tid; i < p.sp_ring_cap; i += BLOCK) reinterpret_cast<uint16_t*>(lds_raw + p.sp_ring_off)[i] = (uint16_t)rthand::ring_empty_for(0u, p.sp_ring_cap);
         __syncthreads();
     }
     const float* const lnodes = reinterpret_cast<const float*>(lds_raw + p.lds_node_off) - (LTREE ? (int)lt_r0(p.n_internal) : 0);
@@ -623,13 +657,13 @@
     V3 ig = mk(0, 0, 0), cq = mk(0, 0, 0);
     bool qfin = false;
     float t_far = __builtin_inff();
-    uint32_t* lc32 = reinterpret_cast<uint32_t*>(lds_raw + p.lds_cand_off);
-    uint32_t* lstack = reinterpret_cast<uint32_t*>(lds_raw + p.lds_stack_off);
+    uint32_t* lc32 = reinterpret_cast<uint32_t*>(lds_raw + cand_off);
+    uint32_t* lstack = reinterpret_cast<uint32_t*>(lds_raw + stack_off);
     uint32_t sgx = 0, sgy = 0, sgz = 0;
-    uint16_t* lc16 = reinterpret_cast<uint16_t*>(lds_raw + p.lds_cand_off);
-    uint16_t* lstack16 = reinterpret_cast<uint16_t*>(lds_raw + p.lds_stack_off);
-
-    if (BFSTEP) lstack16[tid16] = (uint16_t)(lt_r0(p.n_internal) + p.n_internal * (uint32_t)LNODE_DW);
+    uint16_t* lc16 = reinterpret_cast<uint16_t*>(lds_raw + cand_off);
+    uint16_t* lstack16 = reinterpret_cast<uint16_t*>(lds_raw + stack_off);
+
+    if (BFSTEP && (!SPLIT || walker)) lstack16[lcol] = (uint16_t)(lt_r0(p.n_internal) + p.n_internal * (uint32_t)LNODE_DW);
 
     auto drain_counters = [&]() {
         const unsigned long long ws = wave_sum(n_seg), wc = wave_sum(n_cand), wf = wave_sum(n_fall);
@@ -653,9 +687,34 @@
     };
     auto div_spp = [&](uint32_t q) -> uint32_t { return p.spp_magic ? __umulhi(q, p.spp_magic) : q; };
 
+    uint32_t* const mbox = reinterpret_cast<uint32_t*>(lds_raw + (SPLIT ? p.sp_mbox_off : 0u));
+    uint16_t* const hring = reinterpret_cast<uint16_t*>(lds_raw + (SPLIT ? p.sp_ring_off : 0u));
+    constexpr uint32_t MB = NS * 64u;
+    HandLds hq{&hq_head, &hq_tail, &hq_alive};
+    uint32_t qid = 0;
+    bool gave_up = false;
+    auto wait_turn = [&](unsigned long long t0) -> bool {
+        if (__hip_atomic_load(&hq_abort, __ATOMIC_RELAXED, __HIP_MEMORY_SCOPE_WORKGROUP) != 0u) {
+            gave_up = true;
+            return false;
+        }
+        if (__builtin_amdgcn_s_memrealtime() - t0 > HAND_WAIT_TICKS) {
+            if (lane == (int)__builtin_ctzll(__ballot(true))) {
+                atomicAdd(p.giveup, 1ull);
+                __hip_atomic_store(&hq_abort, 1u, __ATOMIC_RELAXED, __HIP_MEMORY_SCOPE_WORKGROUP);
+            }
+            gave_up = true;
+            return false;
+        }
+        __builtin_amdgcn_s_sleep(1);
+        return true;
+    };
+    if (SPLIT && walker && RT_LT_SPLIT_PRIO) __builtin_amdgcn_s_setprio(RT_LT_SPLIT_PRIO);
+
     TDECL;
     for (;;) {
         WCOUNT(0);
+        if (SPLIT && (__ballot(gave_up) != 0ull || __hip_atomic_load(&hq_abort, __ATOMIC_RELAXED, __HIP_MEMORY_SCOPE_WORKGROUP) != 0u)) break;
         TSTAMP(5);
         TROUND;
         uint32_t px = 0, pyg = 0;
@@ -797,7 +856,7 @@
         TSTAMP(6);
         if (TRAVERSE && __ballot(((n_seg | n_cand | n_fall | n_int) & 0x80000000u) != 0)) drain_counters();
         {
-            bool need = !have_unit;
+            bool need = !have_unit && !(SPLIT && walker);
             for (;;) {
                 if (__ballot(need) == 0ull) break;
                 if (tile_u == tile_units) {
@@ -944,7 +1003,7 @@
                 if (stall) { LCOUNT(14); break; }
             }
         }
-        const bool active = have_unit;
+        bool active = have_unit;
         if (!active) { LCOUNT(13); }
         TSTAMP(0);
         if (active && need_ray) {
@@ -991,15 +1050,118 @@
         const bool wave_busy = __ballot(active) != 0ull || freem != all_free || !q_drained || tile_u != tile_units;
         if (STREAMED) {
             if (!__syncthreads_or(wave_busy ? 1 : 0)) break;
+        } else if (SPLIT && walker) {
+            bool leave = false, timing = false;
+            unsigned long long t_idle = 0;
+            for (;;) {
+                const unsigned long long fm = __ballot(!have_unit);
+                uint32_t base = 0, take = 0;
+                if (fm != 0ull && lane == 0) rthand::reserve_pop(hq, (uint32_t)__builtin_popcountll(fm), base, take);
+                base = uni(base);
+                take = uni(take);
+                if (take) {
+                    const uint32_t rank = __builtin_amdgcn_mbcnt_hi((uint32_t)(fm >> 32), __builtin_amdgcn_mbcnt_lo((uint32_t)fm, 0u));
+                    const bool mine = !have_unit && rank < take;
+                    const uint32_t pos = base + rank;
+                    uint16_t* const e = hring + rthand::ring_slot(pos, p.sp_ring_cap);
+                    uint32_t word = rthand::RING_EMPTY_BIT;
+                    bool full = false;
+                    const unsigned long long t0 = __builtin_amdgcn_s_memrealtime();
+                    for (;;) {
+                        if (mine && !full) {
+                            word = __hip_atomic_load(e, __ATOMIC_ACQUIRE, __HIP_MEMORY_SCOPE_WORKGROUP);
+                            full = rthand::ring_is_full_of(word, pos, p.sp_ring_cap);
+                        }
+                        if (__ballot(mine && !full) == 0ull) break;
+                        if (!wait_turn(t0)) break;
+                    }
+                    if (mine && full) {
+                        __hip_atomic_store(e, (uint16_t)rthand::ring_empty_after(pos, p.sp_ring_cap), __ATOMIC_RELAXED, __HIP_MEMORY_SCOPE_WORKGROUP);
+                        const uint32_t id = rthand::ring_id(word);
+                        qid = id;
+                        o = mk(__uint_as_float(mbox[0u * MB + id]), __uint_as_float(mbox[1u * MB + id]), __uint_as_float(mbox[2u * MB + id]));
+                        d = mk(__uint_as_float(mbox[3u * MB + id]), __uint_as_float(mbox[4u * MB + id]), __uint_as_float(mbox[5u * MB + id]));
+                        have_unit = true;
+                    }
+                }
+                if (__ballot(gave_up) != 0ull) {
+                    leave = true;
+                    break;
+                }
+                if (__ballot(have_unit) != 0ull) break;
+                if (rthand::finished(hq)) {
+                    leave = true;
+                    break;
+                }
+                if (!timing) {
+                    t_idle = __builtin_amdgcn_s_memrealtime();
+                    timing = true;
+                }
+                if (!wait_turn(t_idle)) {
+                    leave = true;
+                    break;
+                }
+            }
+            if (leave) break;
+            active = have_unit;
         } else {
-            if (!wave_busy) break;
+            if (!wave_busy) {
+                if (SPLIT && lane == 0) (void)__hip_atomic_fetch_sub(&hq_alive, 1u, __ATOMIC_RELEASE, __HIP_MEMORY_SCOPE_WORKGROUP);
+                break;
+            }
         }
-
-        if (active && !in_trav) {
+        if (SPLIT && !walker) {
+            const bool fresh = active && !in_trav;
+            const unsigned long long fm = __ballot(fresh);
+            if (fm != 0ull) {
+                if (fresh) {
+                    mbox[0u * MB + sid] = __float_as_uint(o.x);
+                    mbox[1u * MB + sid] = __float_as_uint(o.y);
+                    mbox[2u * MB + sid] = __float_as_uint(o.z);
+                    mbox[3u * MB + sid] = __float_as_uint(d.x);
+                    mbox[4u * MB + sid] = __float_as_uint(d.y);
+                    mbox[5u * MB + sid] = __float_as_uint(d.z);
+                    mbox[6u * MB + sid] = rthand::RESULT_PENDING;
+                    n_seg++;
+                    in_trav = true;
+                }
+                const int first = (int)__builtin_ctzll(fm);
+                uint32_t base = 0;
+                if (lane == first) base = rthand::reserve_push(hq, (uint32_t)__builtin_popcountll(fm));
+                base = (uint32_t)__builtin_amdgcn_readlane((int)base, first);
+                const uint32_t rank = __builtin_amdgcn_mbcnt_hi((uint32_t)(fm >> 32), __builtin_amdgcn_mbcnt_lo((uint32_t)fm, 0u));
+                const uint32_t pos = base + rank;
+                uint16_t* const e = hring + rthand::ring_slot(pos, p.sp_ring_cap);
+                const unsigned long long t0 = __builtin_amdgcn_s_memrealtime();
+                for (;;) {
+                    const bool busy = fresh && __hip_atomic_load(e, __ATOMIC_RELAXED, __HIP_MEMORY_SCOPE_WORKGROUP) != (uint16_t)rthand::ring_empty_for(pos, p.sp_ring_cap);
+                    if (__ballot(busy) == 0ull) break;
+                    if (!wait_turn(t0)) break;
+                }
+                if (fresh && __ballot(gave_up) == 0ull)
+                    __hip_atomic_store(e, (uint16_t)rthand::ring_full_of(pos, p.sp_ring_cap, sid), __ATOMIC_RELEASE, __HIP_MEMORY_SCOPE_WORKGROUP);
+            }
+            bool ready = false;
+            const unsigned long long t0 = __builtin_amdgcn_s_memrealtime();
+            for (;;) {
+                ready = in_trav && __hip_atomic_load(&mbox[6u * MB + sid], __ATOMIC_ACQUIRE, __HIP_MEMORY_SCOPE_WORKGROUP) != rthand::RESULT_PENDING;
+                const uint32_t n_ready = (uint32_t)__builtin_popcountll(__ballot(ready)), n_out = (uint32_t)__builtin_popcountll(__ballot(in_trav));
+                if (n_ready >= min(n_out, (uint32_t)RT_LT_SPLIT_READY)) break;
+                if (!wait_turn(t0)) break;
+            }
+            if (__ballot(gave_up) != 0ull) break;
+            if (ready) {
+                h.idx = (int)mbox[6u * MB + sid];
+                h.t = __uint_as_float(mbox[7u * MB + sid]);
+                in_trav = false;
+            }
+        }
+
+        if ((!SPLIT || walker) && active && !in_trav) {
             h.idx = -1;
             aux = ray_aux(d, (p.flags & 8u) != 0);
             if (!TRAVERSE) td = 2.0f * d;
-            n_seg++;
+            if (!SPLIT) n_seg++;
             if (QNODES) {
                 const V3 og = mk((o.x - p.q_base[0]) * p.q_rstep[0], (o.y - p.q_base[1]) * p.q_rstep[1], (o.z - p.q_base[2]) * p.q_rstep[2]);
                 ig = mk(p.q_step[0] * aux.inv.x, p.q_step[1] * aux.inv.y, p.q_step[2] * aux.inv.z);
@@ -1043,7 +1205,7 @@
         if constexpr (TRAVERSE) {
             auto root_test = [&](uint32_t i) {
                     LCOUNT(6);
-                    const uint32_t prim = LTREE ? (uint32_t)lc16[i * BLOCK + tid16] & 0x7fffu
+                    const uint32_t prim = LTREE ? (uint32_t)lc16[i * LCOLS + lcol] & 0x7fffu
                                           : p.list16 ? (uint32_t)lc16[i * BLOCK + tid16] : lc32[i * BLOCK + tid];
                     float t;
                     if (prim < p.n_sph) {
@@ -1193,20 +1355,22 @@
             };
             if constexpr (BFSTEP) {
             const uint32_t DONE = lt_r0(p.n_internal) + p.n_internal * (uint32_t)LNODE_DW;
-            constexpr int STEPS = RT_STEPS_PER_CHECK_LTREE;
-            static_assert(MAXL_LTREE > STEPS, "the leaf list must take a block of appends");
-            constexpr uint32_t SLOT = (uint32_t)BLOCK * 2u;
+            constexpr int STEPS = SPLIT ? LT_SPLIT_STEPS : RT_STEPS_PER_CHECK_LTREE;
+            static_assert(SPLIT || MAXL_LTREE > STEPS, "the leaf list must take a block of appends");
+            const uint32_t maxl_k = SPLIT ? p.sp_maxl : p.maxl;
+            constexpr uint32_t SLOT = (uint32_t)LCOLS * 2u;
+            constexpr uint32_t LEAF_SHIFT = SPLIT ? lt_split_shift(NW ? NW : 1u) : 4u;
             typedef __attribute__((address_space(3))) unsigned char lds_byte;
             typedef __attribute__((address_space(3))) uint16_t lds_u16;
             const uint32_t lds0 = (uint32_t)(uintptr_t)(lds_byte*)lds_raw;
-            const uint32_t stack0_a = lds0 + p.lds_stack_off + (uint32_t)tid16 * 2u;
-            const uint32_t list0_m = lds0 + p.lds_cand_off + (uint32_t)tid16 * 2u - SLOT;
+            const uint32_t stack0_a = lds0 + stack_off + (uint32_t)lcol * 2u;
+            const uint32_t list0_m = lds0 + cand_off + (uint32_t)lcol * 2u - SLOT;
             uint32_t top_a = 0, cnt_m = 0;
             auto lds16 = [&](uint32_t a) -> lds_u16& { return *(lds_u16*)(uintptr_t)a; };
             auto step = [&](auto slow_tag) {
                 constexpr bool SLOW = decltype(slow_tag)::value;
-                static_assert(SLOT == 0x800u, "leaf flag 0x8000 >> 4 must be one slot");
-                const uint32_t leaf_slot = (t_ref >> 4) & SLOT;
+                static_assert((0x8000u >> LEAF_SHIFT) == SLOT, "the shifted leaf flag must be one slot");
+                const uint32_t leaf_slot = (t_ref >> LEAF_SHIFT) & SLOT;
                 const uint32_t ni = t_ref;
                 if (STATS) n_int += (ni < DONE) ? 1u : 0u;
                 const uint32_t top = (uint32_t)lds16(top_a);
@@ -1262,11 +1426,17 @@
                 cnt_m += leaf_slot;
                 RT_HOOK_LT_STEP_END;
             };
+            bool first_block = true;
+            if (!SPLIT || walker)
             for (;;) {
                 const uint32_t walking = (uint32_t)__builtin_popcountll(__ballot(in_trav));
                 const uint32_t live = (uint32_t)__builtin_popcountll(__ballot(active));
+                if (SPLIT) {
+                    if (walking == 0 || (!first_block && 64u - walking >= 4u * p.refill_eighths)) break;
+                    first_block = false;
+                } else
                 if (walking == 0 || (walking * 8 <= live * p.refill_eighths && walking < live)) break;
-                if (in_trav && t_cnt > p.maxl - (uint32_t)STEPS) flush();
+                if (in_trav && t_cnt > maxl_k - (uint32_t)STEPS) flush();
                 if (RT_LT_PARTIAL < 64) {
                     const bool pend = t_cnt > t_head;
                     if ((int)__builtin_popcountll(__ballot(pend)) >= RT_LT_PARTIAL ||
@@ -1457,7 +1627,7 @@
                 const bool want = active && !in_trav && t_cnt > 0;
                 if (__ballot(want)) flush_c(want);
             } else
-            if (active && !in_trav) flush();
+            if ((!SPLIT || walker) && active && !in_trav) flush();
             TSTAMP(3);
         } else {
             bool seg_active = active;
@@ -1600,6 +1770,13 @@
                 inline_chain = true;
             }
         }
+        if (SPLIT && walker) {
+            if (active && !in_trav) {
+                mbox[7u * MB + qid] = __float_as_uint(h.t);
+                __hip_atomic_store(&mbox[6u * MB + qid], (uint32_t)h.idx, __ATOMIC_RELEASE, __HIP_MEMORY_SCOPE_WORKGROUP);
+                have_unit = false;
+            }
+        } else
         if (active && !in_trav) {
             float term_r, term_g, term_b;
             bool finished;
@@ -1637,7 +1814,7 @@
                     if (p.path32)
                         reinterpret_cast<uint32_t*>(lpath)[k * BLOCK + cold<QNODES>(tid)] = (uint32_t)h.idx;
                     else
-                        reinterpret_cast<uint16_t*>(lpath)[k * BLOCK + cold<QNODES>(tid16)] = (uint16_t)h.idx;
+                        reinterpret_cast<uint16_t*>(lpath)[k * PCOLS + cold<QNODES>(pcol)] = (uint16_t)h.idx;
                     k++;
                     depth_left--;
                     if (depth_left == 0) {
@@ -1674,7 +1851,7 @@
                 {
                     auto path_idx = [&](uint32_t i) -> uint32_t {
                         return p.path32 ? reinterpret_cast<uint32_t*>(lpath)[i * BLOCK + cold<QNODES>(tid)]
-                                        : (uint32_t) reinterpret_cast<uint16_t*>(lpath)[i * BLOCK + cold<QNODES>(tid16)];
+                                        : (uint32_t) reinterpret_cast<uint16_t*>(lpath)[i * PCOLS + cold<QNODES>(pcol)];
                     };
                     uint32_t i = k;
 #pragma clang loop unroll(disable)
@@ -1722,6 +1899,7 @@
 using KernelFn = void (*)(const KParams);
 KernelFn kernel_linear(int isect, bool expanded);
 KernelFn kernel_traverse(int isect, bool stats);
+KernelFn kernel_ltree_split(bool stats);
 void sqrt_selftest_launch(uint32_t from, unsigned long long n, unsigned long long* d_bad, hipStream_t st);
 
 }
diff --git a/ray_tracer_s8_amd/csrc/rt_kernels_trav.hip b/ray_tracer_s8_amd/csrc/rt_kernels_trav.hip
--- a/ray_tracer_s8_amd/csrc/rt_kernels_trav.hip
+++ b/ray_tracer_s8_amd/csrc/rt_kernels_trav.hip
@@ -16,6 +16,9 @@
     }
 }
 KernelFn kernel_traverse(int isect, bool stats) { return stats ? traverse_kernel<true>(isect) : traverse_kernel<false>(isect); }
+KernelFn kernel_ltree_split(bool stats) {
+    return stats ? rt_tile_kernel<5, false, LTREE_BLOCK, true, true> : rt_tile_kernel<5, false, LTREE_BLOCK, false, true>;
+}
 
 __global__ void sqrt_selftest_kernel(uint32_t from, unsigned long long n, unsigned long long* bad) {
     unsigned long long mine = 0;
diff --git a/ray_tracer_s8_amd/csrc/rt_plan.h b/ray_tracer_s8_amd/csrc/rt_plan.h
--- a/ray_tracer_s8_amd/csrc/rt_plan.h
+++ b/ray_tracer_s8_amd/csrc/rt_plan.h
@@ -5,6 +5,7 @@
 #include <cstdint>
 
 #include "rt_consts.h"
+#include "rt_handoff.h"
 #include "rt_tile.h"
 
 namespace rtplan {
@@ -48,6 +49,7 @@
     int compact = 1;
     int refill_eighths = 0;
     int tail_tiles = -1;
+    int lt_split = -1;
 };
 
 struct Engine {
@@ -351,6 +353,63 @@
     return pl;
 }
 
+constexpr uint32_t LT_SPLIT_MIN_INTERNAL = 64;
+struct SplitPlan {
+    bool ok = false;
+    uint32_t walkers = 0, shaders = 0;
+    uint32_t stride = 0, shift = 0;
+    uint32_t maxl = 0, stack_rows = 0;
+    uint32_t cand_off = 0, stack_off = 0, path_off = 0, mbox_off = 0, ring_off = 0;
+    uint32_t ring_cap = 0;
+    size_t lds = 0;
+};
+
+inline bool split_wanted(const Plan& pl, const SceneShape& sh, const Knobs& kn) {
+    return pl.status == RT_OK && pl.engine == 4 && (kn.lt_split >= 0 ? kn.lt_split != 0 : sh.n_internal >= LT_SPLIT_MIN_INTERNAL);
+}
+
+template <class KP>
+SplitPlan plan_split(const SceneShape& sh, uint32_t walkers, uint32_t steps, KP& p) {
+    using namespace rtk;
+    SplitPlan s;
+    s.walkers = walkers;
+    s.shaders = (uint32_t)LTREE_BLOCK / 64u - walkers;
+    s.stride = lt_split_stride(walkers);
+    s.shift = lt_split_shift(walkers);
+    s.stack_rows = sh.bvh_depth + 2u;
+    const size_t shader_lanes = (size_t)s.shaders * 64u;
+    s.ring_cap = rthand::ring_capacity((uint32_t)shader_lanes);
+    const size_t tree_end = p.lds_cand_off;
+    const size_t rest = (size_t)s.stack_rows * s.stride + (size_t)p.depth * shader_lanes * sizeof(uint16_t) +
+                        (size_t)rthand::MBOX_WORDS * shader_lanes * sizeof(uint32_t) + (size_t)s.ring_cap * sizeof(uint16_t);
+    uint32_t maxl = steps + 1u > (uint32_t)MAXL_LTREE ? steps + 1u : (uint32_t)MAXL_LTREE;
+    if (tree_end + rest + (size_t)maxl * s.stride > LDS_LIMIT) maxl = steps + 1u;
+    if (tree_end + rest + (size_t)maxl * s.stride > LDS_LIMIT) return s;
+    while (maxl < (uint32_t)MAXL_LTREE_MAX && tree_end + rest + (size_t)(maxl + 1u) * s.stride <= LDS_LIMIT) maxl++;
+    s.maxl = maxl;
+    size_t off = tree_end;
+    s.cand_off = (uint32_t)off;
+    off += (size_t)maxl * s.stride;
+    s.stack_off = (uint32_t)off;
+    off += (size_t)s.stack_rows * s.stride;
+    s.path_off = (uint32_t)off;
+    off += (size_t)p.depth * shader_lanes * sizeof(uint16_t);
+    s.mbox_off = (uint32_t)off;
+    off += (size_t)rthand::MBOX_WORDS * shader_lanes * sizeof(uint32_t);
+    s.ring_off = (uint32_t)off;
+    off += (size_t)s.ring_cap * sizeof(uint16_t);
+    s.lds = off;
+    s.ok = true;
+    p.sp_cand_off = s.cand_off;
+    p.sp_stack_off = s.stack_off;
+    p.sp_path_off = s.path_off;
+    p.sp_mbox_off = s.mbox_off;
+    p.sp_ring_off = s.ring_off;
+    p.sp_ring_cap = s.ring_cap;
+    p.sp_maxl = s.maxl;
+    return s;
+}
+
 template <class KP>
 void plan_queue(Plan& pl, uint32_t blocks, const Knobs& kn, KP& p) {
     const uint32_t waves_per_wg = (uint32_t)pl.block / 64u;
```

New measurement: 6080. 61.4% lower.
